# facebookresearch/DLRM-FlexFlow

Measured on AMD Instinct MI355X. Metric: dlrm_training_samples_per_sec, higher is better.
Workload: dtype f32; 1 GPU; criteo-terabyte-shape: 26 tables (rows 39884406-39043-17289-7420-20263-3-7120-1543-63-38532951-2953546-403346-10-2208-11938-155-4-976-14-39979771-25641295-39664984-585935-12972-108-36), emb_dim 128, bag 1, bot 13-512-256-128, top 3456-1024-1024-512-256-1, cat interaction, SGD lr 0.01, MSE loss; global_batch=32768, per_gpu_batch=32768, parallelism=single GPU, hipGraph-replayed step, step_graph=True

## Files before the change

dlrm_flexflow_amd/capi.py:

```python
from __future__ import annotations

import ctypes as C
import os
import re

_HERE = os.path.dirname(os.path.abspath(__file__))
REPO_ROOT = os.path.dirname(_HERE)
HIP_LIB_PATH = os.path.join(_HERE, "csrc", "libffhip.so")
HEADER_PATH = os.path.join(REPO_ROOT, "include", "ff_hip.h")

FFH_OK = 0
FFH_ERR_BAD_ARG, FFH_ERR_HIP, FFH_ERR_UNSUPPORTED, FFH_ERR_WORKSPACE, FFH_ERR_NOMEM = -1, -2, -3, -4, -5
AC_MODE_NONE, AC_MODE_RELU, AC_MODE_SIGMOID, AC_MODE_TANH, AC_MODE_GELU = 10, 11, 12, 13, 14
AGGR_MODE_NONE, AGGR_MODE_SUM, AGGR_MODE_AVG = 20, 21, 22
MAX_TABLES = 64
EMB_CHUNK, EMB_CHUNK1 = 32, 1024
OPT_ZERO_GRAD = 1
CONCAT_BWD_OVERWRITE = 1
LINEAR_DX_OVERWRITE, LINEAR_ONLY_DW, LINEAR_ONLY_DX, LINEAR_DY_PREMASKED, LINEAR_DX_MASK_BY_X = 1, 2, 4, 8, 16
METRIC_ACCURACY, METRIC_MSE, METRIC_RMSE, METRIC_MAE = 1, 2, 4, 8

P = C.c_void_p
I = C.c_int
L = C.c_int64
# ... 618 lines not shown

DIGEST_HEADER_PATH = os.path.join(REPO_ROOT, "include", "ff_hip_digest.h")

_SIGS_DIGEST = {
    "ffh_digest_abi_version": (I, []),
    "ffh_state_digest": (I, [P, P, L, L, L, C.c_uint64, C.c_uint64, P, P]),
}


def digest_header_symbols(header_path: str = DIGEST_HEADER_PATH) -> list[str]:
    text = open(header_path).read()
    m = re.search(r"#define FFH_DIGEST_API_LIST\(X\)(.*?)\n\n", text, re.S)
    if not m:
        raise RuntimeError("FFH_DIGEST_API_LIST not found in " + header_path)
    return re.findall(r"X\((ffh_[a-z0-9_]+)\)", m.group(1))


def digest_header_abi_version(header_path: str = DIGEST_HEADER_PATH) -> int:
    m = re.search(r"#define\s+FFH_DIGEST_ABI_VERSION\s+(\d+)", open(header_path).read())
    if not m:
        raise RuntimeError("FFH_DIGEST_ABI_VERSION not found in " + header_path)
    return int(m.group(1))


class DigestApi:

    def __init__(self, lib: FFHLib):
        self.base = lib
        for name, (res, args) in _SIGS_DIGEST.items():
            fn = getattr(lib.lib, name, None)
            if fn is None:
                raise FFHError(f"{lib.path}: no digest extension ({name} missing; include/ff_hip_digest.h)")
            fn.restype = res
            fn.argtypes = args
        got = lib.lib.ffh_digest_abi_version()
        if got != digest_header_abi_version():
            raise FFHError(f"{lib.path}: digest ABI version {got}, include/ff_hip_digest.h says {digest_header_abi_version()} (rebuild)")
        self.lib = lib.lib
        self.ctx = lib.ctx

    def state_digest_rc(self, base, rows, row_bytes, ld_bytes, seed, index_base, acc, stream=None) -> int:
        m64 = 2 ** 64 - 1
        return self.lib.ffh_state_digest(self.ctx, ptr(base), int(rows), int(row_bytes), int(ld_bytes), int(seed) & m64, int(index_base) & m64, ptr(acc),
                                         ptr(stream))

    def state_digest(self, base, rows, row_bytes, ld_bytes, seed, index_base, acc, stream=None):
        self.base.check(self.state_digest_rc(base, rows, row_bytes, ld_bytes, seed, index_base, acc, stream), "ffh_state_digest")


def digest_api(lib: FFHLib) -> DigestApi:
    return DigestApi(lib)


class CrossApi:

    def __init__(self, lib: FFHLib):
        self.base = lib
        for name, (res, args) in _SIGS_CROSS.items():
            fn = getattr(lib.lib, name, None)
            if fn is None:
                raise FFHError(f"{lib.path}: no cross extension ({name} missing; include/ff_hip_cross.h)")
            fn.restype = res
            fn.argtypes = args
        got = lib.lib.ffh_cross_abi_version()
        if got != cross_header_abi_version():
            raise FFHError(f"{lib.path}: cross ABI version {got}, include/ff_hip_cross.h says {cross_header_abi_version()} (rebuild)")
        self.lib = lib.lib
        self.ctx = lib.ctx

    def rc(self, name: str, *args) -> int:
        sig = _SIGS_CROSS[name][1][1:]
        if len(args) != len(sig):
            raise TypeError(f"{name}: expected {len(sig)} args, got {len(args)}")
        conv = [ptr(a) if t is P else a for a, t in zip(args, sig)]
        return getattr(self.lib, name)(self.ctx, *conv)

    def call(self, name: str, *args):
        self.base.check(self.rc(name, *args), name)


def cross_api(lib: FFHLib) -> CrossApi:
    return CrossApi(lib)


class AdagradApi:

    def __init__(self, lib: FFHLib):
        self.base = lib
        for name, (res, args) in _SIGS_ADAGRAD.items():
            fn = getattr(lib.lib, name, None)
            if fn is None:
                raise FFHError(f"{lib.path}: no Adagrad extension ({name} missing; include/ff_hip_adagrad.h)")
            fn.restype = res
            fn.argtypes = args
        got = lib.lib.ffh_adagrad_abi_version()
        if got != adagrad_header_abi_version():
            raise FFHError(f"{lib.path}: Adagrad ABI version {got}, include/ff_hip_adagrad.h says {adagrad_header_abi_version()} (rebuild)")
        self.lib = lib.lib
        self.ctx = lib.ctx

    def rc(self, name: str, *args) -> int:
        sig = _SIGS_ADAGRAD[name][1][1:]
        if len(args) != len(sig):
            raise TypeError(f"{name}: expected {len(sig)} args, got {len(args)}")
        conv = [ptr(a) if t is P else a for a, t in zip(args, sig)]
        return getattr(self.lib, name)(self.ctx, *conv)

    def call(self, name: str, *args):
        self.base.check(self.rc(name, *args), name)


def adagrad_api(lib: FFHLib) -> AdagradApi:
    return AdagradApi(lib)


class RowwiseApi:

    def __init__(self, lib: FFHLib):
        self.base = lib
        for name, (res, args) in _SIGS_ROWWISE.items():
            fn = getattr(lib.lib, name, None)
            if fn is None:
                raise FFHError(f"{lib.path}: no row-wise Adagrad extension ({name} missing; include/ff_hip_rowwise.h)")
            fn.restype = res
            fn.argtypes = args
        got = lib.lib.ffh_rowwise_abi_version()
        if got != rowwise_header_abi_version():
            raise FFHError(f"{lib.path}: row-wise Adagrad ABI version {got}, include/ff_hip_rowwise.h says {rowwise_header_abi_version()} (rebuild)")
        self.lib = lib.lib
        self.ctx = lib.ctx


def rowwise_api(lib: FFHLib) -> RowwiseApi:
    return RowwiseApi(lib)


FOLD_HEADER_PATH = os.path.join(REPO_ROOT, "include", "ff_hip_fold.h")


class FoldGroup(C.Structure):
    _fields_ = [("e", P), ("lde", L), ("col0", L), ("p", P), ("rows", L)]


class FoldSeg(C.Structure):
    _fields_ = [("k0", C.c_int32), ("len", C.c_int32)]


_SIGS_FOLD = {
    "ffh_fold_abi_version": (I, []),
    "ffh_fold_product": (I, [P, C.POINTER(FoldGroup), I, P, L, I, I, P]),
    "ffh_fold_gather_add": (I, [P, C.POINTER(EmbTable), I, I, I, L, I, P, L, P]),
    "ffh_fold_linear_fwd": (I, [P, P, L, P, L, P, P, I, I, L, I, C.POINTER(FoldSeg), I, P, L, P]),
    "ffh_fold_linear_fwd_plan": (I, [P, P, L, P, L, P, P, I, I, L, C.POINTER(FoldSeg), I, P, L]),
}


def fold_header_symbols(header_path: str = FOLD_HEADER_PATH) -> list[str]:
    m = re.search(r"#define FFH_FOLD_API_LIST\(X\)(.*?)\n\n", open(header_path).read(), re.S)
    if not m:
        raise RuntimeError("FFH_FOLD_API_LIST not found in " + header_path)
    return re.findall(r"X\((\w+)\)", m.group(1))


def fold_header_abi_version(header_path: str = FOLD_HEADER_PATH) -> int:
    m = re.search(r"#define\s+FFH_FOLD_ABI_VERSION\s+(\d+)", open(header_path).read())
    if not m:
        raise RuntimeError("FFH_FOLD_ABI_VERSION not found in " + header_path)
    return int(m.group(1))


class FoldApi:

    def __init__(self, lib: "FFHLib"):
        self.base = lib
        for name, (res, args) in _SIGS_FOLD.items():
            fn = getattr(lib.lib, name, None)
            if fn is None:
                raise FFHError(f"{lib.path}: no fold extension ({name} missing; include/ff_hip_fold.h)")
            fn.restype = res
            fn.argtypes = args
        got = lib.lib.ffh_fold_abi_version()
        if got != fold_header_abi_version():
            raise FFHError(f"{lib.path}: fold ABI version {got}, include/ff_hip_fold.h says {fold_header_abi_version()} (rebuild)")
        self.lib = lib.lib
        self.ctx = lib.ctx

    @staticmethod
    def groups(entries) -> "C.Array":
        entries = list(entries)
        arr = (FoldGroup * len(entries))()
        for k, (e, lde, col0, p, rows) in enumerate(entries):
            arr[k] = FoldGroup(ptr(e), int(lde), int(col0), ptr(p), int(rows))
        return arr

    @staticmethod
    def segs(entries) -> "C.Array":
        entries = list(entries)
        arr = (FoldSeg * max(1, len(entries)))()
        for k, (k0, n) in enumerate(entries):
            arr[k] = FoldSeg(int(k0), int(n))
        return arr

    def rc(self, name: str, *args) -> int:
        sig = _SIGS_FOLD[name][1][1:]
        if len(args) != len(sig):
            raise TypeError(f"{name}: expected {len(sig)} args, got {len(args)}")
        conv = [ptr(a) if t is P else a for a, t in zip(args, sig)]
        return getattr(self.lib, name)(self.ctx, *conv)

    def call(self, name: str, *args):
        self.base.check(self.rc(name, *args), name)


def fold_api(lib: "FFHLib") -> FoldApi:
    return FoldApi(lib)


_hip_singleton: FFHLib | None = None


def load_hip(device: int = 0) -> FFHLib:
    global _hip_singleton
    if _hip_singleton is None:
        import torch
        _hip_singleton = FFHLib(HIP_LIB_PATH, device)
        if not _hip_singleton.backend.startswith("hip"):
            raise FFHError(f"{HIP_LIB_PATH} is not the HIP backend ({_hip_singleton.backend})")
    return _hip_singleton
```

dlrm_flexflow_amd/csrc/fold.hip:

```cpp
#include "linear_gemm.h"

#include "../../include/ff_hip_fold.h"

using namespace ffh_gemm;

namespace {

typedef float f32x4 __attribute__((ext_vector_type(4)));

struct FoldGemmGroup { const float* a; int64_t lda; int64_t wcol0; float* c; int64_t ldc; int rows; int tile0; };
struct FoldGemmArgs {
  FoldGemmGroup grp[FFH_FOLD_MAX_GROUPS];
  ffh_fold_seg  seg[FFH_FOLD_MAX_SEGS];
  const float*  w; int64_t ldw;
  const float*  bias;
  const float*  addend; int64_t ldadd;
  int ngroups, nseg, N, act, ntiles;
};
static_assert(sizeof(FoldGemmArgs) <= 4096, "kernel arguments");

template <bool EPI>
__global__ __launch_bounds__(256) void fold_gemm_kernel(const FoldGemmArgs g) {
  ffh_kernel_prio();
  const int lane = threadIdx.x & 63;
  const int wave = __builtin_amdgcn_readfirstlane((int)(threadIdx.x >> 6));
  const int c = lane & 15, q = lane >> 4;
  const int wt = (int)blockIdx.x * 4 + wave;
  if (wt >= g.ntiles) return;
  int gi = 0;
  while (gi + 1 < g.ngroups && g.grp[gi + 1].tile0 <= wt) gi++;
  const FoldGemmGroup G = g.grp[gi];
  const int ct = g.N / 64, local = wt - G.tile0;
  const int r0 = (local / ct) * 32, n0 = (local % ct) * 64;
  const float* ap[2];
  const float* wp[4];
#pragma unroll
  for (int mt = 0; mt < 2; mt++) {
    int r = r0 + 16 * mt + c;
    if (r > G.rows - 1) r = G.rows - 1;
    ap[mt] = G.a + (int64_t)r * G.lda + 4 * q;
  }
#pragma unroll
  for (int nt = 0; nt < 4; nt++) wp[nt] = g.w + (int64_t)(n0 + 16 * nt + c) * g.ldw + G.wcol0 + 4 * q;
  f32x4 acc[4][2];
#pragma unroll
  for (int nt = 0; nt < 4; nt++)
#pragma unroll
    for (int mt = 0; mt < 2; mt++) acc[nt][mt] = f32x4{0.f, 0.f, 0.f, 0.f};
  for (int si = 0; si < g.nseg; si++) {
    const int k0 = g.seg[si].k0, k1 = k0 + g.seg[si].len;
    for (int k = k0; k < k1; k += 16) {
      f32x4 a[2], b[4];
#pragma unroll
      for (int mt = 0; mt < 2; mt++) a[mt] = *reinterpret_cast<const f32x4*>(ap[mt] + k);
#pragma unroll
      for (int nt = 0; nt < 4; nt++) b[nt] = *reinterpret_cast<const f32x4*>(wp[nt] + k);
#pragma unroll
      for (int e = 0; e < 4; e++)
#pragma unroll
        for (int nt = 0; nt < 4; nt++)
#pragma unroll
          for (int mt = 0; mt < 2; mt++) acc[nt][mt] = __builtin_amdgcn_mfma_f32_16x16x4f32(b[nt][e], a[mt][e], acc[nt][mt], 0, 0, 0);
    }
  }
#pragma unroll
  for (int mt = 0; mt < 2; mt++) {
    const int r = r0 + 16 * mt + c;
    if (r >= G.rows) continue;
#pragma unroll
    for (int nt = 0; nt < 4; nt++) {
      const int n = n0 + 16 * nt + 4 * q;
      f32x4 v = acc[nt][mt];
      if constexpr (EPI) {
        if (g.addend) v += *reinterpret_cast<const f32x4*>(g.addend + (int64_t)r * g.ldadd + n);
        if (g.bias) v += f32x4{g.bias[n], g.bias[n + 1], g.bias[n + 2], g.bias[n + 3]};
        if (g.act != FFH_AC_MODE_NONE) { v.x = act_apply(v.x, g.act); v.y = act_apply(v.y, g.act); v.z = act_apply(v.z, g.act); v.w = act_apply(v.w, g.act); }
      }
      *reinterpret_cast<f32x4*>(G.c + (int64_t)r * G.ldc + n) = v;
    }
  }
}

struct FoldGatherTable { const int64_t* idx; const float* p; };
struct FoldGatherArgs {
  FoldGatherTable t[FFH_MAX_TABLES];
  float* S; int64_t ldS;
  int64_t batch;
  int ntables, L, out;
};

__global__ __launch_bounds__(256) void fold_gather_add_kernel(const FoldGatherArgs g) {
  ffh_kernel_prio();
  const int nvec = g.out / 4;
  const int64_t total = g.batch * nvec;
  const int n = g.ntables * g.L;
  for (int64_t i = (int64_t)blockIdx.x * 256 + threadIdx.x; i < total; i += (int64_t)gridDim.x * 256) {
    const int64_t b = i / nvec;
    const int cv = (int)(i - b * nvec) * 4;
    f32x4 acc = f32x4{0.f, 0.f, 0.f, 0.f};
    for (int j0 = 0; j0 < n; j0 += 4) {
      f32x4 v[4];
#pragma unroll
      for (int u = 0; u < 4; u++) {
        const int j = j0 + u;
        if (j < n) {
          const int t = j / g.L, l = j - t * g.L;
          const int64_t id = g.t[t].idx[b * g.L + l];
          v[u] = *reinterpret_cast<const f32x4*>(g.t[t].p + id * g.out + cv);
        }
      }
#pragma unroll
      for (int u = 0; u < 4; u++)
        if (j0 + u < n) acc = (j0 + u == 0) ? v[u] : acc + v[u];
    }
    *reinterpret_cast<f32x4*>(g.S + b * g.ldS + cv) = acc;
  }
}

inline bool al16(const void* p) { return ((uintptr_t)p & 15) == 0; }

int fold_fwd_check(ffh_ctx* c, const float* x, int64_t ldx, const float* y, int64_t ldy, const float* w, int in, int out, int64_t batch,
                   const ffh_fold_seg* keep, int nkeep, const float* addend, int64_t ldadd) {
  FFH_REQUIRE(c, in > 0 && out > 0 && batch >= 0 && ldx >= in && ldy >= out, "fold_linear_fwd: bad dims");
  FFH_REQUIRE(c, batch == 0 || (x && y && w), "fold_linear_fwd: null pointer");
  FFH_REQUIRE(c, batch < (1LL << 31), "fold_linear_fwd: batch too large");
  FFH_REQUIRE(c, nkeep >= 0 && (nkeep == 0 || keep), "fold_linear_fwd: bad segment list");
  FFH_REQUIRE(c, !addend || ldadd >= out, "fold_linear_fwd: bad addend");
  int prev = 0;
  for (int i = 0; i < nkeep; i++) {
    FFH_REQUIRE(c, keep[i].k0 >= prev && keep[i].len > 0 && (int64_t)keep[i].k0 + keep[i].len <= in, "fold_linear_fwd: segments must ascend inside [0, in_dim)");
    prev = keep[i].k0 + keep[i].len;
  }
  return FFH_OK;
}
bool fold_fwd_served(const ffh_ctx* c, const float* x, int64_t ldx, const float* y, int64_t ldy, const float* w, int in, int out,
                     const ffh_fold_seg* keep, int nkeep, const float* addend, int64_t ldadd) {
  if (c->math_mode != FFH_MATH_DEFAULT) return false;
  if (in % FFH_FOLD_KTILE || out % FFH_FOLD_NTILE || nkeep > FFH_FOLD_MAX_SEGS) return false;
  if (!al16(x) || !al16(y) || !al16(w) || ldx % 4 || ldy % 4 || (addend && (!al16(addend) || ldadd % 4))) return false;
  for (int i = 0; i < nkeep; i++)
    if (keep[i].k0 % FFH_FOLD_KTILE || keep[i].len % FFH_FOLD_KTILE) return false;
  return true;
}
bool fold_keep_mask(int in, const ffh_fold_seg* keep, int nkeep, unsigned long long mask[2], int* nk_kept) {
  mask[0] = mask[1] = 0;
  *nk_kept = 0;
  if (in % 64 || in > 128 * 64) return false;
  const ffh_fold_seg all{0, in};
  if (nkeep == 0) { keep = &all; nkeep = 1; }
  for (int i = 0; i < nkeep; i++) {
    if (keep[i].k0 % 64 || keep[i].len % 64) return false;
    for (int kt = keep[i].k0 / 64; kt < (keep[i].k0 + keep[i].len) / 64; kt++) { mask[kt >> 6] |= 1ull << (kt & 63); (*nk_kept)++; }
  }
  return *nk_kept > 0;
}
GemmArgs fold_fwd_gemm(const float* x, int64_t ldx, float* y, int64_t ldy, const float* w, const float* bias, int in, int out, int64_t batch, int act) {
  GemmArgs g{};
  g.A = x; g.sAm = ldx; g.sAk = 1;
  g.B = w; g.sBn = in; g.sBk = 1;
  g.C = y; g.ldc = ldy; g.bias = bias;
  g.M = (int)batch; g.N = out; g.K = in;
  g.epi = EPI_STORE; g.act = act;
  return g;
}

}

extern "C" {

int ffh_fold_abi_version(void) { return FFH_FOLD_ABI_VERSION; }

int ffh_fold_product(ffh_ctx* c, const ffh_fold_group* groups, int ngroups, const float* w, int64_t ldw, int d, int out, ffh_stream s) {
  FFH_REQUIRE(c, groups && w && ngroups >= 1 && d > 0 && out > 0 && ldw >= d, "fold_product: bad arguments");
  if (ngroups > FFH_FOLD_MAX_GROUPS || d % FFH_FOLD_KTILE || out % FFH_FOLD_NTILE || !al16(w) || ldw % 4)
    return ffh_fail(c, FFH_ERR_UNSUPPORTED, "fold_product: d a multiple of 16, out_dim a multiple of 64, at most 64 tables, aligned weight");
  FoldGemmArgs a{};
  int64_t tiles = 0;
  for (int i = 0; i < ngroups; i++) {
    const ffh_fold_group& gr = groups[i];
    FFH_REQUIRE(c, gr.e && gr.p && gr.rows >= 1 && gr.rows < (1LL << 31) && gr.lde >= d && gr.col0 >= 0 && gr.col0 + d <= ldw, "fold_product: bad group");
    if (!al16(gr.e) || !al16(gr.p) || gr.lde % 4 || gr.col0 % FFH_FOLD_KTILE) return ffh_fail(c, FFH_ERR_UNSUPPORTED, "fold_product: group not aligned");
    a.grp[i] = FoldGemmGroup{gr.e, gr.lde, gr.col0, gr.p, (int64_t)out, (int)gr.rows, (int)tiles};
    tiles += ((gr.rows + 31) / 32) * (out / 64);
    FFH_REQUIRE(c, tiles < (1LL << 30), "fold_product: too many rows");
  }
  a.seg[0] = ffh_fold_seg{0, d};
  a.w = w; a.ldw = ldw; a.ngroups = ngroups; a.nseg = 1; a.N = out; a.act = FFH_AC_MODE_NONE; a.ntiles = (int)tiles;
  hipLaunchKernelGGL(fold_gemm_kernel<false>, dim3((unsigned)((tiles + 3) / 4)), dim3(256), 0, as_stream(s), a);
  FFH_LAUNCH_CHECK(c, "fold_gemm_kernel (products)");
  return FFH_OK;
}

int ffh_fold_gather_add(ffh_ctx* c, const ffh_emb_table* tables, int ntables, int in_dim, int out, int64_t batch, int aggr, float* S, int64_t ldS,
                        ffh_stream s) {
  FFH_REQUIRE(c, tables && ntables >= 1 && in_dim >= 1 && out > 0 && batch >= 0 && S && ldS >= out, "fold_gather_add: bad arguments");
  if (aggr != FFH_AGGR_MODE_SUM) return ffh_fail(c, FFH_ERR_UNSUPPORTED, "fold_gather_add: sum aggregation only");
  if (ntables > FFH_MAX_TABLES || out % 4 || ldS % 4 || !al16(S)) return ffh_fail(c, FFH_ERR_UNSUPPORTED, "fold_gather_add: out_dim and ldS multiples of 4, aligned S, at most 64 tables");
  FoldGatherArgs a{};
  for (int t = 0; t < ntables; t++) {
    FFH_REQUIRE(c, tables[t].idx && tables[t].weight && tables[t].num_entries >= 1, "fold_gather_add: bad table");
    if (!al16(tables[t].weight)) return ffh_fail(c, FFH_ERR_UNSUPPORTED, "fold_gather_add: product not aligned");
    a.t[t] = FoldGatherTable{tables[t].idx, tables[t].weight};
  }
  if (batch == 0) return FFH_OK;
  a.S = S; a.ldS = ldS; a.batch = batch; a.ntables = ntables; a.L = in_dim; a.out = out;
  hipLaunchKernelGGL(fold_gather_add_kernel, dim3(ffh_grid(batch * (out / 4), 256, 4096)), dim3(256), 0, as_stream(s), a);
  FFH_LAUNCH_CHECK(c, "fold_gather_add_kernel");
  return FFH_OK;
}

int ffh_fold_linear_fwd_plan(ffh_ctx* c, const float* x, int64_t ldx, const float* y, int64_t ldy, const float* w, const float* bias, int in, int out,
                             int64_t batch, const ffh_fold_seg* keep, int nkeep, const float* addend, int64_t ldadd) {
  const int rc = fold_fwd_check(c, x, ldx, y, ldy, w, in, out, batch, keep, nkeep, addend, ldadd);
  if (rc != FFH_OK) return rc;
  if (!fold_fwd_served(c, x, ldx, y, ldy, w, in, out, keep, nkeep, addend, ldadd)) return ffh_fail(c, FFH_ERR_UNSUPPORTED, "fold_linear_fwd: shape / alignment / math mode not served");
  const GemmArgs g = fold_fwd_gemm(x, ldx, const_cast<float*>(y), ldy, w, bias, in, out, batch, FFH_AC_MODE_NONE);
  unsigned long long mask[2]; int nk = 0;
  if (batch > 0 && fold_keep_mask(in, keep, nkeep, mask, &nk) && launch_gemm_sk_fold(c, g, mask, nk, addend, ldadd, true, nullptr, "") == 1) return 2;
  return (batch > 0 && gemm_sk_serves(c, g, SK_FORM_FWD)) ? 0 : 1;
}

int ffh_fold_linear_fwd(ffh_ctx* c, const float* x, int64_t ldx, float* y, int64_t ldy, const float* w, const float* bias, int in, int out, int64_t batch,
                        int act, const ffh_fold_seg* keep, int nkeep, const float* addend, int64_t ldadd, ffh_stream s) {
  if (nkeep == 0 && !addend) return ffh_linear_fwd(c, x, ldx, y, ldy, w, bias, in, out, batch, act, s);
  const int rc = fold_fwd_check(c, x, ldx, y, ldy, w, in, out, batch, keep, nkeep, addend, ldadd);
  if (rc != FFH_OK) return rc;
  if (act != FFH_AC_MODE_NONE && act != FFH_AC_MODE_RELU && act != FFH_AC_MODE_SIGMOID && act != FFH_AC_MODE_GELU)
    return ffh_fail(c, FFH_ERR_UNSUPPORTED, "fold_linear_fwd: activation not supported (NONE, RELU, SIGMOID, GELU)");
  if (!fold_fwd_served(c, x, ldx, y, ldy, w, in, out, keep, nkeep, addend, ldadd)) return ffh_fail(c, FFH_ERR_UNSUPPORTED, "fold_linear_fwd: shape / alignment / math mode not served");
  ffh_route_clear(c);
  if (batch == 0) return FFH_OK;
  const GemmArgs g = fold_fwd_gemm(x, ldx, y, ldy, w, bias, in, out, batch, act);
  unsigned long long mask[2]; int nk = 0;
  if (fold_keep_mask(in, keep, nkeep, mask, &nk) && (!bias || al16(bias))) {
    const int r = launch_gemm_sk_fold(c, g, mask, nk, addend, ldadd, false, s, "fold_linear_fwd gemm");
    if (r != 0) return r < 0 ? r : FFH_OK;
  }
  FoldGemmArgs a{};
  a.grp[0] = FoldGemmGroup{x, ldx, 0, y, ldy, (int)batch, 0};
  if (nkeep == 0) { a.seg[0] = ffh_fold_seg{0, in}; a.nseg = 1; }
  else { for (int i = 0; i < nkeep; i++) a.seg[i] = keep[i]; a.nseg = nkeep; }
  const int64_t tiles = ((batch + 31) / 32) * (out / 64);
  FFH_REQUIRE(c, tiles < (1LL << 30), "fold_linear_fwd: too many tiles");
  a.w = w; a.ldw = in; a.bias = bias; a.addend = addend; a.ldadd = ldadd; a.ngroups = 1; a.N = out; a.act = act; a.ntiles = (int)tiles;
  hipLaunchKernelGGL(fold_gemm_kernel<true>, dim3((unsigned)((tiles + 3) / 4)), dim3(256), 0, as_stream(s), a);
  FFH_LAUNCH_CHECK(c, "fold_gemm_kernel (forward)");
  ffh_route_add(c, "fold_linear_fwd gemm|mfma_32x64x16");
  return FFH_OK;
}

}
```

dlrm_flexflow_amd/csrc/linear_gemm.h:

```cpp
#pragma once
#include "ffh_common.h"

#include <hip/hip_runtime.h>

namespace ffh_gemm {

typedef float f32x16 __attribute__((ext_vector_type(16)));

enum { EPI_STORE = 0, EPI_ADD = 1, EPI_ATOMIC = 2 };

struct GemmArgs {
  const float* A;
  const float* B;
  float*       C;
  const float* bias;
  int64_t sAm, sAk, sBn, sBk, ldc;
  int64_t bsA, bsB, bsC;
  int M, N, K;
  int k_per_split;
  int splitk;
  int epi;
  int act;
  const float* act_y;
  int64_t      ld_act_y;
  float*       db;
  int          fuse;
  const float* mask;
  int64_t      ldmask;
  const ffh_col_dest* colmap;
  float* colsum;
  const unsigned short* A16;
  const unsigned short* B16;
  unsigned short*       C16;
  int                   a_not_twinned;
  int                   db_done;
};

constexpr int kSplitGran = 32;

__device__ __forceinline__ float act_apply(float v, int act) {
  if (act == FFH_AC_MODE_RELU) return v > 0.0f ? v : 0.0f;
  if (act == FFH_AC_MODE_SIGMOID) return 1.0f / (1.0f + expf(-v));
  if (act == FFH_AC_MODE_GELU) {
    constexpr float B = 0.7978845608028654f, C = 0.035677408136300125f;
    return v * (0.5f + 0.5f * tanhf(v * (C * v * v + B)));
  }
  return v;
}

__device__ __forceinline__ float4 load4_guard(const float* p, bool row_ok, int c0, int climit, bool vec_ok) {
  float4 v = make_float4(0.f, 0.f, 0.f, 0.f);
  if (!row_ok) return v;
  if (vec_ok && c0 + 3 < climit) return ld4u(p);
  if (c0 + 0 < climit) v.x = p[0];
  if (c0 + 1 < climit) v.y = p[1];
  if (c0 + 2 < climit) v.z = p[2];
  if (c0 + 3 < climit) v.w = p[3];
  return v;
}

template <typename K>
bool glds_set_lds(K kern, int bytes) {
  if (hipFuncSetAttribute((const void*)kern, hipFuncAttributeMaxDynamicSharedMemorySize, bytes) != hipSuccess) { (void)hipGetLastError(); return false; }
  return true;
}

inline bool use_bf16(const ffh_ctx* c, int in, int out, int64_t batch) {
  if (in < FFH_BF16_MIN_DIM || out < FFH_BF16_MIN_DIM) return false;
  if (c->math_mode == FFH_MATH_TENSOR_OP_BF16) return true;
  return c->math_mode == FFH_MATH_FP32_SPLIT_BF16X3_ALL || (c->math_mode == FFH_MATH_FP32_SPLIT_BF16X3 && 2.0 * (double)batch * (double)in * (double)out >= FFH_BF16X3_MIN_FLOP);
}

enum { BF16_FORM_FWD = 0,
       BF16_FORM_DW = 1,
       BF16_FORM_DX = 2,
       BF16_FORM_DX_MASK = 3 };
int launch_gemm_bf16_form(ffh_ctx* c, GemmArgs& g, int form, ffh_stream s, const char* name);
int launch_gemm_bf16_dma(ffh_ctx* c, const GemmArgs& g, int form, ffh_stream s, const char* name);
int launch_gemm_x3_dma(ffh_ctx* c, const GemmArgs& g, int form, ffh_stream s, const char* name);
float* dw_tile_slots(const ffh_ctx* c, ffh_stream s, int64_t tiles, int splitk, int64_t ldc);
void launch_dw_tile_reduce(const float* slots, float* C, int64_t ldc, int M, int N, int64_t tiles, int splitk, ffh_stream s);

enum { SK_FORM_FWD = 0, SK_FORM_DX = 1, SK_FORM_DW = 2 };
bool gemm_sk_serves(const ffh_ctx* c, const GemmArgs& g, int form);
int launch_gemm_sk(ffh_ctx* c, const GemmArgs& g, int form, ffh_stream s, const char* name);
int launch_gemm_sk_fold(ffh_ctx* c, const GemmArgs& g, const unsigned long long keep[2], int nk_kept, const float* addend, int64_t ldadd, bool dry,
                        ffh_stream s, const char* name);

}
```

dlrm_flexflow_amd/csrc/linear_sk.hip:

```cpp
#include "linear_gemm.h"

#include <stdlib.h>
#include <atomic>
#include <type_traits>
#include <utility>

using namespace ffh_gemm;

namespace {

typedef float f32x4 __attribute__((ext_vector_type(4)));
typedef unsigned u32x4 __attribute__((ext_vector_type(4)));

constexpr int SK_BM = 128, SK_BN = 128, SK_BK = 64;
constexpr int SK_LDS_KC = 128 * 256 + 32 * 32;
constexpr int SK_LDS_KR = 64 * 512;
constexpr int sk_lds_kc_a(int TMW) { return 32 * TMW * 256 + 32 * 32; }

enum { SK_EPI_FWD = 0, SK_EPI_DX_STORE = 1, SK_EPI_DX_ADD = 2, SK_EPI_DW_ATOMIC = 3, SK_EPI_DX_CMAP = 4 };

struct SkArgs {
  const float* A; const float* B; float* C;
  const float* bias;
  float*       db;
  const float* mask;
  const ffh_col_dest* colmap;
  float*       colsum;
  int64_t lda, ldb, ldc, ldmask;
  int M, N, K;
  int act;
  unsigned a_bytes, b_bytes, bias_bytes, mask_bytes;
  float*    sk_slots;
  unsigned* sk_cnt;
};

struct SkArgsFold : SkArgs {
  unsigned long long keep[2];
  unsigned           nk_kept;
  const float*       addend;
  int64_t            ldadd;
};

template <int... I, class F>
__device__ __forceinline__ void sk_static_for_impl(std::integer_sequence<int, I...>, F&& f) { (f(std::integral_constant<int, I>{}), ...); }
template <int N_, class F>
__device__ __forceinline__ void sk_static_for(F&& f) { sk_static_for_impl(std::make_integer_sequence<int, N_>{}, static_cast<F&&>(f)); }

#define SK_PIN() __builtin_amdgcn_sched_barrier(0)

constexpr int SK_EP_LD = 68;
constexpr int SK_EP_ROWS = 16;
constexpr int SK_EP_WAVE = SK_EP_ROWS * SK_EP_LD * 4;

template <bool AKR, bool BKR, int EPI, bool DB = false, bool SPLIT = false, int TMW = 4, bool FOLD = false>
__global__ __launch_bounds__(256, 1) void gemm_sk_kernel(const std::conditional_t<FOLD, SkArgsFold, SkArgs> g) {
  static_assert(!FOLD || (EPI == SK_EPI_FWD && !SPLIT && !DB && TMW == 4), "kept k-tiles + addend: the whole-tile forward form");
  static_assert(!DB || (EPI == SK_EPI_DW_ATOMIC && AKR), "the bias gradient rides on the weight-gradient form");
  static_assert(!SPLIT || EPI != SK_EPI_DW_ATOMIC, "the weight gradient meets by atomics");
  static_assert(TMW == 4 || (TMW == 2 && !AKR && EPI != SK_EPI_DW_ATOMIC), "64-row tiles: forward and data gradient (A k-contiguous)");
  extern __shared__ __attribute__((aligned(16))) char sk_lds[];
  constexpr bool ATOMIC = EPI == SK_EPI_DW_ATOMIC;
  constexpr bool STREAMK = ATOMIC || SPLIT;
  constexpr int BM = 32 * TMW;
  constexpr int NM = 64 * TMW;
  constexpr int NPA = 2 * TMW, NP = NPA + 8;
  constexpr int LDS_A = AKR ? SK_LDS_KR : sk_lds_kc_a(TMW);
  char* const ldsA = sk_lds;
  char* const ldsB = sk_lds + LDS_A;
  const int tid = threadIdx.x, lane = tid & 63;
  const int wave = __builtin_amdgcn_readfirstlane(tid >> 6);
  const int wy = wave >> 1, wx = wave & 1;
  const int c16 = lane & 15, q = lane >> 4;

  const int fra = AKR ? (q * 2048 + wy * 256 + c16 * 16) : ((16 * TMW * wy + TMW * c16) * 256 + (16 * wy + c16) * 32 + q * 16);
  const int frb = BKR ? (q * 2048 + wx * 256 + c16 * 16) : ((64 * wx + 4 * c16) * 256 + (16 * wx + c16) * 32 + q * 16);
  const int srowA = AKR ? (tid >> 5) : (tid >> 4), schA = AKR ? (tid & 31) : (tid & 15);
  const int srowB = BKR ? (tid >> 5) : (tid >> 4), schB = BKR ? (tid & 31) : (tid & 15);
  const unsigned voffA = (unsigned)((srowA * g.lda + schA * 4) * 4);
  const unsigned voffB = (unsigned)((srowB * g.ldb + schB * 4) * 4);
  const int swA = AKR ? (srowA * 512 + schA * 16) : (srowA * 256 + (srowA / TMW) * 32 + schA * 16);
  const int swB = BKR ? (srowB * 512 + schB * 16) : (srowB * 256 + (srowB >> 2) * 32 + schB * 16);
  constexpr int SW_STEP_A = AKR ? 4096 : (4096 + (16 / TMW) * 32), SW_STEP_B = BKR ? 4096 : 4224;
  const unsigned ioffA = (unsigned)((AKR ? 8 : 16) * g.lda * 4), ioffB = (unsigned)((BKR ? 8 : 16) * g.ldb * 4);
  const unsigned kadvA = AKR ? (unsigned)(SK_BK * g.lda * 4) : (unsigned)(SK_BK * 4), kadvB = BKR ? (unsigned)(SK_BK * g.ldb * 4) : (unsigned)(SK_BK * 4);

  const __amdgpu_buffer_rsrc_t rsA = __builtin_amdgcn_make_buffer_rsrc(const_cast<float*>(g.A), 0, g.a_bytes, 0x00020000);
  const __amdgpu_buffer_rsrc_t rsB = __builtin_amdgcn_make_buffer_rsrc(const_cast<float*>(g.B), 0, g.b_bytes, 0x00020000);

  const unsigned nbx = (unsigned)(g.N / SK_BN), nby = (unsigned)(g.M / BM), ntiles = nbx * nby;
  unsigned nk = (unsigned)(g.K / SK_BK);
  if constexpr (FOLD) nk = g.nk_kept;
  auto first_kept = [&]() -> unsigned {
    if constexpr (FOLD) return g.keep[0] ? (unsigned)__builtin_ctzll(g.keep[0]) : 64u + (unsigned)__builtin_ctzll(g.keep[1]);
    else return 0u;
  };
  auto next_kept = [&](unsigned p) -> unsigned {
    if constexpr (FOLD) {
      p++;
      if (p < 64u) {
        const unsigned long long m = g.keep[0] >> p;
        if (m) return p + (unsigned)__builtin_ctzll(m);
        p = 64u;
      }
      const unsigned long long m = p < 128u ? g.keep[1] >> (p - 64u) : 0ull;
      return m ? p + (unsigned)__builtin_ctzll(m) : p;
    } else return p + 1u;
  };
  const unsigned G = gridDim.x, w = blockIdx.x;
  const unsigned total_it = ntiles * nk;
  const unsigned wperm = (w & 7u) * (G >> 3) + (w >> 3);
  unsigned it_b, it_e;
  const unsigned ipw = (total_it + G - 1) / G;
  const unsigned rng = SPLIT ? wperm : w;
  if (STREAMK) {
    it_b = rng * ipw; it_e = it_b + ipw < total_it ? it_b + ipw : total_it;
    if (it_b > total_it) it_b = total_it;
  } else {
    const unsigned mine = ntiles / G + (wperm < ntiles % G ? 1u : 0u);
    it_b = 0; it_e = mine * nk;
  }
  const unsigned n_it = it_e - it_b;
  if (n_it == 0) return;

  struct Cursor { unsigned seq, kt, m0, n0, offA, offB, kp; };
  auto place = [&](Cursor& c) {
    unsigned lin;
    if (STREAMK) lin = it_b / nk + c.seq;
    else lin = c.seq * G + wperm;
    if (lin >= ntiles) lin = ntiles - 1;
    const unsigned by = lin / nbx, bx = lin - by * nbx;
    c.m0 = by * BM; c.n0 = bx * SK_BN;
    c.kp = FOLD ? first_kept() : c.kt;
    c.offA = (AKR ? c.m0 * 4u : (unsigned)(c.m0 * g.lda * 4)) + c.kp * kadvA;
    c.offB = (BKR ? c.n0 * 4u : (unsigned)(c.n0 * g.ldb * 4)) + c.kp * kadvB;
  };
  auto advance = [&](Cursor& c) {
    c.kt++;
    if (c.kt == nk) { c.kt = 0; c.seq++; place(c); }
    else if constexpr (FOLD) { const unsigned np = next_kept(c.kp), d = np - c.kp; c.offA += d * kadvA; c.offB += d * kadvB; c.kp = np; }
    else { c.offA += kadvA; c.offB += kadvB; }
  };
  Cursor ld{0, STREAMK ? it_b % nk : 0u, 0, 0, 0, 0, 0}, cp = ld;
  place(ld); place(cp);

  u32x4 P[NP];
  auto gload_one = [&](int i, const Cursor& c) {
    if (i < NPA) P[i] = __builtin_amdgcn_raw_buffer_load_b128(rsA, voffA, c.offA + (unsigned)i * ioffA, 0);
    else P[i] = __builtin_amdgcn_raw_buffer_load_b128(rsB, voffB, c.offB + (unsigned)(i - NPA) * ioffB, 0);
  };
  auto lwrite_one = [&](int i) {
    if (i < NPA) *reinterpret_cast<u32x4*>(ldsA + swA + i * SW_STEP_A) = P[i];
    else *reinterpret_cast<u32x4*>(ldsB + swB + (i - NPA) * SW_STEP_B) = P[i];
  };
  f32x4 fa[4][4], fb[4][4];
  auto fread = [&](int j, int r, bool isB) {
    if (!isB) fa[j][r] = *reinterpret_cast<const f32x4*>(ldsA + fra + (AKR ? (j * 8192 + r * 512) : (r * 256 + j * 64)));
    else fb[j][r] = *reinterpret_cast<const f32x4*>(ldsB + frb + (BKR ? (j * 8192 + r * 512) : (r * 256 + j * 64)));
  };
  f32x4 acc[TMW][4];
  f32x4 bsum = f32x4{0.f, 0.f, 0.f, 0.f};

#pragma unroll
  for (int i = 0; i < NP; i++) gload_one(i, ld);
  advance(ld);
#pragma unroll
  for (int i = 0; i < NP; i++) lwrite_one(i);
#pragma unroll
  for (int i = 0; i < NP; i++) gload_one(i, ld);
  advance(ld);
  __builtin_amdgcn_s_waitcnt(0xC07F);
  __builtin_amdgcn_s_barrier();
  SK_PIN();
#pragma unroll
  for (int r = 0; r < 4; r++) { if (r < TMW) fread(0, r, false); fread(0, r, true); }
  SK_PIN();

  for (unsigned it = 0; it < n_it;) {
    const unsigned seg = (nk - cp.kt) < (n_it - it) ? (nk - cp.kt) : (n_it - it);
#pragma unroll
    for (int i = 0; i < TMW; i++)
#pragma unroll
      for (int j = 0; j < 4; j++) acc[i][j] = f32x4{0.f, 0.f, 0.f, 0.f};
    asm volatile("s_nop 7" ::: "memory");
    for (unsigned kk = 0; kk < seg; kk++) {
      sk_static_for<NM>([&](auto sc) {
        constexpr int s = decltype(sc)::value;
        constexpr int tn = s & 3, tm = (s >> 2) % TMW, e = (s / (4 * TMW)) & 3, j = s / (16 * TMW);
        const float av = AKR ? fa[j][e][tm] : fa[j][tm][e];
        const float bv = BKR ? fb[j][e][tn] : fb[j][tn][e];
        asm volatile("v_mfma_f32_16x16x4_f32 %0, %1, %2, %0" : "+a"(acc[tm][tn]) : "v"(av), "v"(bv));
        if constexpr (DB && (s & 15) == 1) {
          asm volatile("v_add_f32 %0, %4, %0\n\tv_add_f32 %1, %5, %1\n\tv_add_f32 %2, %6, %2\n\tv_add_f32 %3, %7, %3"
                       : "+v"(bsum.x), "+v"(bsum.y), "+v"(bsum.z), "+v"(bsum.w)
                       : "v"(fa[j][e].x), "v"(fa[j][e].y), "v"(fa[j][e].z), "v"(fa[j][e].w));
        }
        constexpr int RPG = TMW + 4;
        constexpr int NRD = 3 * RPG;
        constexpr int BAR1 = TMW == 4 ? 53 : 30;
        constexpr int PSTEP = TMW == 4 ? 11 : 7;
        constexpr int BAR2 = NM - 13;
        if constexpr (s < NRD) {
          constexpr int jj = 1 + s / RPG, gi = s % RPG;
          if constexpr (gi < 2 * TMW) fread(jj, gi >> 1, (gi & 1) != 0);
          else fread(jj, gi - TMW, true);
        }
        if constexpr (s == BAR1) {
          __builtin_amdgcn_s_waitcnt(0xC07F);
          __builtin_amdgcn_s_barrier();
        }
        if constexpr (s > BAR1 && s <= BAR1 + 1 + (NP - 1) * PSTEP && (s - BAR1 - 1) % PSTEP == 0) {
          constexpr int i = (s - BAR1 - 1) / PSTEP;
          lwrite_one(i);
          gload_one(i, ld);
        }
        if constexpr (s == BAR2) {
          __builtin_amdgcn_s_waitcnt(0xC07F);
          __builtin_amdgcn_s_barrier();
        }
        if constexpr (s > BAR2 && s <= BAR2 + RPG) {
          constexpr int o = s - BAR2 - 1;
          if constexpr (o == 0) fread(0, 0, false);
          else if constexpr (o <= 4) fread(0, o - 1, true);
          else fread(0, o - 4, false);
        }
        SK_PIN();
      });
      advance(ld);
    }
    it += seg;
    asm volatile("s_nop 15\n\ts_nop 15" ::: "memory");
    bool store_tile = true;
    if constexpr (SPLIT) {
      const bool head = cp.kt == 0;
      if (!(head && seg == nk)) {
        typedef unsigned long long u64;
        const unsigned it0 = (it_b / nk + cp.seq) * nk;
        const unsigned r0 = it0 / ipw, r1 = (it0 + nk - 1) / ipw;
        const unsigned nparts = r1 - r0 + 1;
        u64* slot = reinterpret_cast<u64*>(g.sk_slots + (size_t)(head ? 2u * rng + 1u : 2u * rng) * (SK_BM * SK_BN));
#pragma unroll
        for (int tm = 0; tm < TMW; tm++)
#pragma unroll
          for (int tn = 0; tn < 4; tn++) {
            const f32x4 v = acc[tm][tn];
            u64* q2 = slot + ((tm * 4 + tn) * 256 + tid) * 2;
            __hip_atomic_store(q2, ((u64)__float_as_uint(v.y) << 32) | __float_as_uint(v.x), __ATOMIC_RELAXED, __HIP_MEMORY_SCOPE_AGENT);
            __hip_atomic_store(q2 + 1, ((u64)__float_as_uint(v.w) << 32) | __float_as_uint(v.z), __ATOMIC_RELAXED, __HIP_MEMORY_SCOPE_AGENT);
          }
        asm volatile("s_waitcnt vmcnt(0)" ::: "memory");
        __syncthreads();
        unsigned* const bc = reinterpret_cast<unsigned*>(sk_lds + LDS_A + (BKR ? SK_LDS_KR : SK_LDS_KC));
        if (tid == 0) *bc = __hip_atomic_fetch_add(g.sk_cnt + r0, 1u, __ATOMIC_RELAXED, __HIP_MEMORY_SCOPE_AGENT);
        __syncthreads();
        const bool last = *bc == nparts - 1;
        __syncthreads();
        if (!last) {
          store_tile = false;
        } else {
          if (tid == 0) __hip_atomic_store(g.sk_cnt + r0, 0u, __ATOMIC_RELAXED, __HIP_MEMORY_SCOPE_AGENT);
          for (unsigned p = head ? 1u : 0u; p < nparts; p++) {
            const u64* sl = reinterpret_cast<const u64*>(g.sk_slots + (size_t)(p == 0 ? 2u * r0 + 1u : 2u * (r0 + p)) * (SK_BM * SK_BN));
#pragma unroll
            for (int tm = 0; tm < TMW; tm++)
#pragma unroll
              for (int tn = 0; tn < 4; tn++) {
                const u64* q2 = sl + ((tm * 4 + tn) * 256 + tid) * 2;
                const u64 lo = __hip_atomic_load(q2, __ATOMIC_RELAXED, __HIP_MEMORY_SCOPE_AGENT);
                const u64 hi = __hip_atomic_load(q2 + 1, __ATOMIC_RELAXED, __HIP_MEMORY_SCOPE_AGENT);
                const f32x4 v = f32x4{__uint_as_float((unsigned)lo), __uint_as_float((unsigned)(lo >> 32)), __uint_as_float((unsigned)hi), __uint_as_float((unsigned)(hi >> 32))};
                if (p == 0) acc[tm][tn] = v; else acc[tm][tn] += v;
              }
          }
        }
      }
    }
    if (store_tile) {
      const int nn = (int)cp.n0 + 64 * wx + 4 * c16;
      const bool relu_fast = g.act == FFH_AC_MODE_RELU, none_fast = g.act == FFH_AC_MODE_NONE;
      (void)relu_fast; (void)none_fast;
      f32x4 bv = f32x4{0.f, 0.f, 0.f, 0.f};
      if constexpr (EPI == SK_EPI_FWD) {
        const __amdgpu_buffer_rsrc_t rsBias = __builtin_amdgcn_make_buffer_rsrc(const_cast<float*>(g.bias), 0, g.bias_bytes, 0x00020000);
        const u32x4 t = __builtin_amdgcn_raw_buffer_load_b128(rsBias, (unsigned)nn * 4u, 0, 0);
        bv = __builtin_bit_cast(f32x4, t);
// ... 121 lines not shown

namespace ffh_gemm {

namespace {
struct SkPlan { int64_t lda, ldb, a_bytes, b_bytes; int G; bool split; int tmw; };
bool sk_plan(const ffh_ctx* c, const GemmArgs& g, int form, SkPlan& p) {
  static const int off = FFH_LAB_INT("FFH_GEMM_NO_SK", 0);
  if (off) return false;
  {
    static const int64_t min_w = FFH_LAB_I64("FFH_SK_MIN_WEIGHTS", 0);
    static const int64_t min_wb = FFH_LAB_I64("FFH_SK_MIN_WEIGHTS_BWD", 65536);
    const int64_t nw = form == SK_FORM_DW ? (int64_t)g.M * g.N : (int64_t)g.N * g.K;
    if (nw < min_w || (form != SK_FORM_FWD && nw < min_wb)) return false;
  }
  if (g.M % SK_BM || g.N % SK_BN || g.K % SK_BK || g.M <= 0 || g.N <= 0 || g.K <= 0) return false;
  const bool akr = form == SK_FORM_DW, bkr = form != SK_FORM_FWD;
  p.lda = akr ? g.sAk : g.sAm; p.ldb = bkr ? g.sBk : g.sBn;
  if ((akr ? g.sAm : g.sAk) != 1 || (bkr ? g.sBn : g.sBk) != 1) return false;
  if (!sk_aligned(g.A, p.lda) || !sk_aligned(g.B, p.ldb) || (!g.colmap && !sk_aligned(g.C, g.ldc))) return false;
  if (g.mask && !sk_aligned(g.mask, g.ldmask)) return false;
  if (g.bias && ((uintptr_t)g.bias & 15)) return false;
  if (g.act_y || g.fuse || g.splitk > 1) return false;
  if (g.colmap && (form != SK_FORM_DX || g.epi != EPI_STORE || g.mask)) return false;
  p.a_bytes = ((akr ? (int64_t)(g.K - 1) : (int64_t)(g.M - 1)) * p.lda + (akr ? g.M : g.K)) * 4;
  p.b_bytes = ((bkr ? (int64_t)(g.K - 1) : (int64_t)(g.N - 1)) * p.ldb + (bkr ? g.N : g.K)) * 4;
  if (p.a_bytes >= (1LL << 32) || p.b_bytes >= (1LL << 32)) return false;
  p.G = c->num_cus & ~7;
  if (form == SK_FORM_DW && c->dw_cu_reserve > 0 && p.G - c->dw_cu_reserve >= 64) p.G -= c->dw_cu_reserve;
  if (p.G < 8) return false;
  const int64_t ntiles = (int64_t)(g.M / SK_BM) * (g.N / SK_BN), nk = g.K / SK_BK;
  if (ntiles * nk >= (1LL << 31)) return false;
  p.tmw = 4;
  if (form == SK_FORM_DW) {
    if (c->deterministic || g.epi != EPI_ATOMIC) return false;
    static const int dw_min_it = FFH_LAB_INT("FFH_SK_DW_MIN_IT", 8);
    if (ntiles * nk < (int64_t)dw_min_it * p.G) return false;
  } else {
    if (g.epi != EPI_STORE && g.epi != EPI_ADD) return false;
    static const int no_split = FFH_LAB_INT("FFH_SK_NO_SPLIT", 0);
    const int64_t rounds = (ntiles + p.G - 1) / p.G;
    const int64_t idle_it = (rounds * p.G - ntiles) * nk / p.G;
    static const int no_t64 = FFH_LAB_INT("FFH_SK_NO_T64", 0);
    p.tmw = 4;
    if (!no_t64 && ntiles < p.G && g.M % 64 == 0 && (g.epi == EPI_STORE || g.epi == EPI_ADD) && nk >= 8) {
      const int64_t nt64 = (int64_t)(g.M / 64) * (g.N / SK_BN);
      if (nt64 <= p.G && nt64 * 100 >= (int64_t)p.G * 80) { p.tmw = 2; p.split = false; return true; }
    }
    p.split = !no_split && idle_it >= 2 && ntiles * nk >= 8LL * p.G && g.epi == EPI_STORE;
    if (!p.split) {
      if (ntiles < p.G) return false;
      if (ntiles * 100 < rounds * p.G * 80) return false;
    }
  }
  return true;
}

bool sk_slots_for(ffh_ctx* c, hipStream_t s, float** slots, unsigned** cnt) {
  for (int i = 0; i < c->nscratch; i++)
    if (c->scratch[i].stream == (void*)s && c->scratch[i].sk_slots) { *slots = c->scratch[i].sk_slots; *cnt = c->scratch[i].sk_cnt; return true; }
  return false;
}
}

bool gemm_sk_serves(const ffh_ctx* c, const GemmArgs& g, int form) { SkPlan p; return sk_plan(c, g, form, p); }

int launch_gemm_sk(ffh_ctx* c, const GemmArgs& g, int form, ffh_stream s, const char* name) {
  SkPlan p{};
  if (!sk_plan(c, g, form, p)) return 0;
  float* slots = nullptr; unsigned* flags = nullptr;
  if (p.split && !sk_slots_for(c, as_stream(s), &slots, &flags)) {
    p.split = false;
    { char tok[96]; snprintf(tok, sizeof tok, "%s|no_scratch_on_this_stream", name); ffh_route_add(c, tok); }
    const int64_t ntiles = (int64_t)(g.M / SK_BM) * (g.N / SK_BN), rounds = (ntiles + p.G - 1) / p.G;
    if (ntiles < p.G || ntiles * 100 < rounds * p.G * 80) return 0;
  }
  const int64_t lda = p.lda, ldb = p.ldb, a_bytes = p.a_bytes, b_bytes = p.b_bytes;
  const int G = p.G;
  SkArgs a{};
  a.A = g.A; a.B = g.B; a.C = g.C; a.bias = g.bias; a.mask = g.mask; a.db = g.db; a.colmap = g.colmap; a.colsum = (form == SK_FORM_DX && g.epi == EPI_STORE && !g.colmap) ? g.colsum : nullptr;
  a.lda = lda; a.ldb = ldb; a.ldc = g.ldc; a.ldmask = g.ldmask;
  a.M = g.M; a.N = g.N; a.K = g.K; a.act = g.act;
  a.a_bytes = (unsigned)a_bytes; a.b_bytes = (unsigned)b_bytes;
  a.bias_bytes = g.bias ? (unsigned)g.N * 4u : 0u;
  a.mask_bytes = g.mask ? 1u : 0u;
  if (p.split) { a.sk_slots = slots; a.sk_cnt = flags; }
#define FFH_SK_LAUNCH(AKR, BKR, EPI, LDSB, ...)                                                                  \
  {                                                                                                              \
    auto kern = gemm_sk_kernel<AKR, BKR, EPI, ##__VA_ARGS__>;                                                    \
    static std::atomic<signed char> ok[64];                \
    const int dev = c->device & 63;                                                                              \
    if (ok[dev].load(std::memory_order_acquire) == 0) ok[dev].store(sk_set_lds(kern, LDSB) ? 1 : -1, std::memory_order_release); \
    if (ok[dev].load(std::memory_order_acquire) < 0) return 0;                                                   \
    hipLaunchKernelGGL(kern, dim3((unsigned)G), dim3(256), LDSB, as_stream(s), a);                               \
  }
  constexpr int BCW = 64;
  constexpr int KC64 = sk_lds_kc_a(2);
  if (form == SK_FORM_FWD && p.tmw == 2) FFH_SK_LAUNCH(false, false, SK_EPI_FWD, KC64 + SK_LDS_KC, false, false, 2)
  else if (form == SK_FORM_DX && p.tmw == 2 && g.colmap) FFH_SK_LAUNCH(false, true, SK_EPI_DX_CMAP, KC64 + SK_LDS_KR, false, false, 2)
  else if (form == SK_FORM_DX && p.tmw == 2 && g.epi == EPI_STORE) FFH_SK_LAUNCH(false, true, SK_EPI_DX_STORE, KC64 + SK_LDS_KR, false, false, 2)
  else if (form == SK_FORM_DX && p.tmw == 2) FFH_SK_LAUNCH(false, true, SK_EPI_DX_ADD, KC64 + SK_LDS_KR, false, false, 2)
  else if (form == SK_FORM_FWD && p.split) FFH_SK_LAUNCH(false, false, SK_EPI_FWD, 2 * SK_LDS_KC + BCW, false, true)
  else if (form == SK_FORM_DX && p.split && g.colmap) FFH_SK_LAUNCH(false, true, SK_EPI_DX_CMAP, SK_LDS_KC + SK_LDS_KR + BCW, false, true)
  else if (form == SK_FORM_DX && p.split) FFH_SK_LAUNCH(false, true, SK_EPI_DX_STORE, SK_LDS_KC + SK_LDS_KR + BCW, false, true)
  else if (form == SK_FORM_FWD) FFH_SK_LAUNCH(false, false, SK_EPI_FWD, 2 * SK_LDS_KC)
  else if (form == SK_FORM_DW && g.db) FFH_SK_LAUNCH(true, true, SK_EPI_DW_ATOMIC, 2 * SK_LDS_KR + 4 * SK_EP_WAVE, true)
  else if (form == SK_FORM_DW) FFH_SK_LAUNCH(true, true, SK_EPI_DW_ATOMIC, 2 * SK_LDS_KR + 4 * SK_EP_WAVE)
  else if (g.colmap) FFH_SK_LAUNCH(false, true, SK_EPI_DX_CMAP, SK_LDS_KC + SK_LDS_KR)
  else if (g.epi == EPI_STORE) FFH_SK_LAUNCH(false, true, SK_EPI_DX_STORE, SK_LDS_KC + SK_LDS_KR)
  else FFH_SK_LAUNCH(false, true, SK_EPI_DX_ADD, SK_LDS_KC + SK_LDS_KR)
#undef FFH_SK_LAUNCH
  {
    const hipError_t e = hipGetLastError();
    if (e == hipErrorInvalidValue || e == hipErrorInvalidConfiguration || e == hipErrorLaunchOutOfResources || e == hipErrorSharedObjectInitFailed) return 0;
    if (e != hipSuccess) return ffh_fail_hip(c, e, name);
  }
  { char tok[96]; snprintf(tok, sizeof tok, "%s|sk_%dx128x64%s%s%s|wgs=%d", name, 32 * p.tmw, g.colmap ? "|colmap" : "", p.split ? "|streamk" : "", a.colsum ? "|colsum" : "", G); ffh_route_add(c, tok); }
  return 1;
}

int launch_gemm_sk_fold(ffh_ctx* c, const GemmArgs& g, const unsigned long long keep[2], int nk_kept, const float* addend, int64_t ldadd, bool dry,
                        ffh_stream s, const char* name) {
  if (g.K % SK_BK || g.K > 128 * SK_BK || nk_kept < 1 || nk_kept > g.K / SK_BK) return 0;
  if (addend && !sk_aligned(addend, ldadd)) return 0;
  GemmArgs gk = g;
  gk.K = nk_kept * SK_BK;
  SkPlan p{};
  if (!sk_plan(c, gk, SK_FORM_FWD, p) || p.split || p.tmw != 4) return 0;
  const int64_t a_bytes = ((int64_t)(g.M - 1) * p.lda + g.K) * 4, b_bytes = ((int64_t)(g.N - 1) * p.ldb + g.K) * 4;
  if (a_bytes >= (1LL << 32) || b_bytes >= (1LL << 32)) return 0;
  if (dry) return 1;
  SkArgsFold a{};
  a.A = g.A; a.B = g.B; a.C = g.C; a.bias = g.bias;
  a.lda = p.lda; a.ldb = p.ldb; a.ldc = g.ldc;
  a.M = g.M; a.N = g.N; a.K = g.K; a.act = g.act;
  a.a_bytes = (unsigned)a_bytes; a.b_bytes = (unsigned)b_bytes;
  a.bias_bytes = g.bias ? (unsigned)g.N * 4u : 0u;
  a.keep[0] = keep[0]; a.keep[1] = keep[1]; a.nk_kept = (unsigned)nk_kept; a.addend = addend; a.ldadd = ldadd;
  {
    auto kern = gemm_sk_kernel<false, false, SK_EPI_FWD, false, false, 4, true>;
    constexpr int LDSB = 2 * SK_LDS_KC;
    static std::atomic<signed char> ok[64];
    const int dev = c->device & 63;
    if (ok[dev].load(std::memory_order_acquire) == 0) ok[dev].store(sk_set_lds(kern, LDSB) ? 1 : -1, std::memory_order_release);
    if (ok[dev].load(std::memory_order_acquire) < 0) return 0;
    hipLaunchKernelGGL(kern, dim3((unsigned)p.G), dim3(256), LDSB, as_stream(s), a);
    const hipError_t e = hipGetLastError();
    if (e == hipErrorInvalidValue || e == hipErrorInvalidConfiguration || e == hipErrorLaunchOutOfResources || e == hipErrorSharedObjectInitFailed) return 0;
    if (e != hipSuccess) return ffh_fail_hip(c, e, name);
  }
  { char tok[96]; snprintf(tok, sizeof tok, "%s|sk_128x128x64|kept=%d/%d%s|wgs=%d", name, nk_kept, g.K / SK_BK, addend ? "|addend" : "", p.G); ffh_route_add(c, tok); }
  return 1;
}

}
```

dlrm_flexflow_amd/host/ffmodel.h:

```cpp
#pragma once

#include <cstddef>
#include <cstdint>
#include <condition_variable>
#include <deque>
#include <functional>
#include <map>
#include <mutex>
#include <thread>
#include <string>
#include <vector>

#include "../../include/ff_hip.h"
#include "../../include/ff_hip_bf16.h"
#include "../../include/ff_hip_ctr.h"
#include "../../include/ff_hip_lr.h"
#include "../../include/ff_hip_cross.h"
#include "../../include/ff_hip_adagrad.h"
#include "../../include/ff_hip_rowwise.h"
#include "../../include/ff_hip_fold.h"
#include "ffcomm.h"

enum ActiMode { AC_MODE_NONE = 10, AC_MODE_RELU = 11, AC_MODE_SIGMOID = 12, AC_MODE_TANH = 13, AC_MODE_GELU = 14 };
enum AggrMode { AGGR_MODE_NONE = 20, AGGR_MODE_SUM = 21, AGGR_MODE_AVG = 22 };
enum DataType { DT_FLOAT = 40, DT_DOUBLE = 41, DT_INT32 = 42, DT_INT64 = 43, DT_BOOLEAN = 44, DT_NONE = 49,
                DT_BF16 = 140 };
enum LossType {
  LOSS_CATEGORICAL_CROSSENTROPY = 50,
  LOSS_SPARSE_CATEGORICAL_CROSSENTROPY = 51,
  LOSS_MEAN_SQUARED_ERROR_AVG_REDUCE = 52,
  LOSS_MEAN_SQUARED_ERROR_SUM_REDUCE = 53,
  LOSS_BINARY_CROSSENTROPY = 150,
};
enum CompMode { COMP_MODE_TRAINING = 70, COMP_MODE_INFERENCE = 71 };
enum ParameterSyncType { NONE = 80, PS = 81, NCCL = 82 };
enum MetricsType {
  METRICS_ACCURACY = 1001,
  METRICS_CATEGORICAL_CROSSENTROPY = 1002,
  METRICS_SPARSE_CATEGORICAL_CROSSENTROPY = 1004,
  METRICS_MEAN_SQUARED_ERROR = 1008,
  METRICS_ROOT_MEAN_SQUARED_ERROR = 1016,
  METRICS_MEAN_ABSOLUTE_ERROR = 1032,
  METRICS_BINARY_CROSSENTROPY = 2001,
  METRICS_AUC = 2002,
};
enum OperatorType { OP_INPUT, OP_LINEAR, OP_EMBEDDING, OP_CONCAT, OP_BATCHMATMUL, OP_TRANSPOSE, OP_RESHAPE, OP_FLAT, OP_TRIL, OP_DOT_INTERACTION, OP_CROSS_COMBINE };

#define MAX_TENSOR_DIM 4
#define MAX_NUM_INPUTS 256
#define MAX_OPNAME 64

class FFModel;
class Op;
struct KernelApi;

struct ParallelConfig {
  enum DeviceType { GPU = 0, CPU = 1 };
  ParallelConfig() : device_type(GPU), nDims(0) { for (int& d : dim) d = 1; }
  int num_parts() const { int n = 1; for (int i = 0; i < nDims; i++) n *= dim[i]; return n; }
  bool is_data_parallel() const;
  bool operator==(const ParallelConfig& rhs) const;
  DeviceType device_type;
  int nDims, dim[MAX_TENSOR_DIM];
  std::vector<int> device_ids;
};
typedef size_t MappingTagID;
bool load_strategies_from_file(const std::string& filename, std::map<MappingTagID, ParallelConfig>& strategies);
bool save_strategies_to_file(const std::string& filename, const std::map<std::string, ParallelConfig>& strategies);

class FFConfig {
 public:
  FFConfig();
  void parse_args(char** argv, int argc);
  int epochs, batchSize, printFreq;
  int numNodes, cpusPerNode, workersPerNode;
  float learningRate, weightDecay;
  size_t workSpaceSize;
  bool syntheticInput, profiling, perform_fusion;
  CompMode computationMode;
  std::string dataset_path;
  std::string import_strategy_file, export_strategy_file;
  std::map<MappingTagID, ParallelConfig> strategies;
  static MappingTagID get_hash_id(const std::string& pcname);
  bool find_parallel_config(int ndims, const std::string& pcname, ParallelConfig& config) const;
  std::string save_checkpoint_dir, load_checkpoint_dir;
  int checkpoint_every_epochs;
  std::string backend_lib;
  int device;
  uint64_t seed;
  bool enable_graph;
  bool overlap_embedding;
  bool dense_embedding_update;
  int64_t column_shard_rows;
  bool deterministic;
  bool fp32_split_bf16x3;
  bool allow_tensor_op_math_conversion;
  bool bf16_convert_twins;
  bool bf16_exact_small_backward;
  bool bf16_twins, force_async_launch;
  bool capture_exchange;
  bool pad_linear_k;
  bool sparse_embedding_optimizer;
  int early_sort;
  bool dx_colsum;
  bool dx_scatter;
  bool fuse_pair;
  int  bucket_allreduce;
  bool direct_allreduce;
  int64_t allreduce_bucket_floats;
  int64_t big_dw_min_weights;
  int  big_dw_chunks;
  int  trace_mode;
  bool fold_small_tables;
  int64_t fold_max_rows;
  bool mlp_chain;
  int64_t mlp_chain_max_batch;
  int64_t mlp_chain_fwd_max_batch;
  int64_t mlp_chain_fwd_min_batch;
  int64_t mlp_chain_max_weights;
  bool attach_events;
  bool timing_events;
  int driver_loss;
  int eval_batches;
  int synthetic_labels;
  bool eval_only;
  int data_randomize;
  bool fuse_loss;
  int64_t replicate_embedding_rows;
  int64_t row_shard_rows;
  bool async_launch;
  bool parallel_dw;
  bool force_exchange;
  DataType embedding_dtype;
  int embedding_rounding;
  int64_t lr_warmup_steps, lr_decay_start_step, lr_num_decay_steps;
  bool device_lr;
  bool host_lr_schedule;
  double adagrad_eps;
  double adagrad_initial_accumulator;
  bool adagrad_rowwise;
  ffcomm comm;
};

struct TensorPiece {
  float*  ptr;
  float*  grad;
  int64_t ld;
  int     cols;
};

struct TensorImpl {
  void*   ptr = nullptr;
  int64_t ld = 0;
  float*  grad = nullptr;
  int64_t grad_ld = 0;
  bool    alias = false;
  bool    grad_alias = false;
  bool    is_input = false;
  size_t  bytes = 0;
  int64_t rows_local = 0;
  int     guid = -1;
  std::vector<TensorPiece> pieces;
};

struct Tensor {
  Tensor(void);
  size_t get_volume() const;
  int64_t rows() const;
  int64_t cols() const { return adim[0]; }
  template <typename T> bool set_tensor(const FFModel* model, const std::vector<int>& dims, const T* data);
  template <typename T> bool get_tensor(const FFModel* model, T* data) const;
  template <typename T> bool get_grad(const FFModel* model, T* data) const;
  int numDim, adim[MAX_TENSOR_DIM];
  DataType data_type;
  ParameterSyncType sync_type;
  Op* owner_op;
  int owner_idx;
  TensorImpl* impl;
};

struct Parameter : Tensor {
  template <typename T> bool set_weights(const FFModel* model, const std::vector<int>& dims, const T* data);
  template <typename T> bool get_weights(const FFModel* model, T* data) const;
};

class Initializer {
 public:
  virtual ~Initializer() {}
  virtual void init(const FFModel* ff, const Parameter* p) = 0;
};
class ZeroInitializer : public Initializer {
 public:
  void init(const FFModel* ff, const Parameter* p) override;
};
class ConstantInitializer : public Initializer {
 public:
  explicit ConstantInitializer(float v) : value(v) {}
  void init(const FFModel* ff, const Parameter* p) override;
  float value;
};
class UniformInitializer : public Initializer {
 public:
  UniformInitializer(int _seed, float _min, float _max) : seed(_seed), min_val(_min), max_val(_max) {}
  void init(const FFModel* ff, const Parameter* p) override;
  int seed;
  float min_val, max_val;
};
class NormInitializer : public Initializer {
 public:
  NormInitializer(int _seed, float _mean, float _stddev) : seed(_seed), mean(_mean), stddev(_stddev) {}
  void init(const FFModel* ff, const Parameter* p) override;
  int seed;
  float mean, stddev;
};
class GlorotUniform : public Initializer {
 public:
  explicit GlorotUniform(int _seed) : seed(_seed) {}
  void init(const FFModel* ff, const Parameter* p) override;
  int seed;
};

class Optimizer {
 public:
  explicit Optimizer(const FFModel* _model) : model(_model) {}
  virtual ~Optimizer() {}
  virtual void init(void) = 0;
  virtual void next(void) = 0;
  virtual void update(const Parameter* p) = 0;
  const FFModel* model;
};
class SGDOptimizer : public Optimizer {
 public:
  SGDOptimizer(const FFModel* _model, double lr = 0.01f, double momentum = 0.0f, bool nesterov = false,
               double weight_decay = 0.0f);
  void init(void) override;
  void next(void) override;
  void update(const Parameter* p) override;
  void set_weight_decay(double wd) { weight_decay = wd; }
  double lr, momentum;
  bool nesterov;
  double weight_decay;
  std::map<const void*, float*> v_values;
};

class AdamOptimizer : public Optimizer {
 public:
  AdamOptimizer(const FFModel* _model, double _alpha = 0.001f, double _beta1 = 0.9f, double _beta2 = 0.999f,
                double _weight_decay = 0.0f, double _epsilon = 1e-8);
  void init(void) override;
  void next(void) override;
  void update(const Parameter* p) override;
  void set_weight_decay(double wd) { weight_decay = wd; }
  double alpha, beta1, beta2, weight_decay, epsilon;
  double alpha_t, beta1_t, beta2_t;
  float *mlp_m, *mlp_v;
  std::map<const void*, std::pair<float*, float*>> mv_values;
};

class AdagradOptimizer : public Optimizer {
 public:
  AdagradOptimizer(const FFModel* _model, double _lr = 0.01f, double _weight_decay = 0.0f, double _epsilon = 1e-10, double _initial_accumulator = 0.0);
  void init(void) override;
  void next(void) override;
  void update(const Parameter* p) override;
  void set_weight_decay(double wd) { weight_decay = wd; }
  double lr, weight_decay, epsilon, initial_accumulator;
  bool rowwise;
// ... 215 lines not shown
                          bool create_grad = true);

  void compile(LossType loss_type, const std::vector<MetricsType>& metrics, CompMode comp_mode = COMP_MODE_TRAINING);
  void compile(Optimizer* optimizer, LossType loss_type, const std::vector<MetricsType>& metrics,
               CompMode comp_mode = COMP_MODE_TRAINING);
  void init_layers();
  void reset_metrics();
  void forward(int seq_length = -1);
  void zero_gradients();
  void compute_metrics();
  void backward(int seq_length = -1);
  void update();
  void begin_trace(int trace_id);
  void end_trace(int trace_id);
  void sync();
  PerfMetrics get_perf_metrics();
  void eval_batch();
  void reset_eval_metrics();
  EvalMetrics get_eval_metrics(bool with_histograms = false);
  Initializer* own(Initializer* init) { owned_initializers.push_back(init); return init; }
  int next_seed();
  uint64_t seed_counter;
  void print_layers(int id);
  std::string get_operator_type_name(OperatorType type) const;

  int op_global_guid;
  FFConfig config;
  Optimizer* optimizer;
  LossType loss_type;
  int metrics_flags;
  Tensor label_tensor;
  std::vector<Op*> layers;
  std::vector<Parameter> parameters;
  int seq_length;

  const KernelApi* api;
  ffh_ctx* ctx;
  ffh_stream stream;
  ffh_stream side_stream;
  ffh_stream dw_stream;
  ffh_event ev_dw_done;
  int big_dw_layer;
  bool need_zero_gsend;
  bool need_zero_act_grads;
  mutable bool dw_forked;
  mutable bool dw1_used = false;
  mutable bool dw_stream_used_directly = false;
  struct GradBucket {
    size_t off, count;
    int lowest_layer;
    bool issued;
    ffh_event ready, ready_dw, done;
    int chunk_layer, chunk_index;
    bool inline_issued;
  };
  std::vector<GradBucket> grad_buckets;
  std::vector<std::pair<size_t, size_t>> grad_rest;
  ffh_stream ar_stream = nullptr;
  bool bucketed_now() const;
  int  allreduce_grads(float* buf, int64_t count, ffh_stream s, bool bucket) const;
  float* ar_scratch = nullptr;
  size_t ar_scratch_floats = 0;
  mutable int64_t n_direct_allreduces = 0;
  mutable std::map<int64_t, std::vector<int64_t>> direct_plans;
  bool buckets_held() const;
  void issue_grad_buckets(int next_layer);
  void issue_one_bucket(size_t k, bool wait_main);
  int  big_dw_chunks_now() const;
  mutable int64_t n_bucket_allreduces = 0;
  int64_t n_fused_loss_calls = 0;
  mutable int64_t n_chain_fwd_calls = 0, n_chain_bwd_calls = 0;
  bool mlp_chain_usable(int64_t rows, bool fwd) const;
  int run_chain_fwd(const Linear* lowest) const;
  int run_chain_bwd(Linear* top);
  mutable bool mlp_grads_clean;
  LaunchWorker *dw_worker, *side_worker;
  std::vector<ffh_event> layer_events;
  bool use_workers() const { return dw_worker != nullptr && capturing_trace < 0; }
  ffh_event ev_fork, ev_join, ev_grad_ready, ev_update_done;
  int rank, world_size;
  bool exchange;
  int64_t local_batch;
  bool compiled;

  void* dmalloc(size_t bytes) const;
  void check(int rc, const char* what) const;

  std::vector<Embedding*> embeddings;
  void embedding_group_forward(ffh_stream s, ffh_ctx* on_ctx = nullptr) const;
  void replicated_embedding_grads() const;
  void embedding_group_update(ffh_stream s, ffh_ctx* on_ctx = nullptr) const;
  void embedding_kernels_only(bool fwd, ffh_stream s, const std::vector<const int64_t*>* idx_override = nullptr) const;
  mutable bool probe_events_on = false;
  static constexpr int kProbeEvents = 30;
  mutable ffh_event probe_ev[kProbeEvents] = {};
  void probe_record(int which, ffh_stream s, ffh_ctx* cx) const;
  uint64_t* bf16_counter = nullptr;
  ffh_bf16_rounding bf16_rounding() const;
  uint64_t read_bf16_counter() const;
  void advance_bf16_counter(ffh_stream s, ffh_ctx* cx) const;
  size_t bf16_tables_per_launch() const;
  enum LrRoute { kLrOff = 0, kLrHost = 1, kLrDevice = 2 };
  int lr_route = kLrOff;
  std::string lr_route_why;
  double lr_base = 0.0;
  int64_t lr_host_steps = 0;
  ffh_lr_state* lr_block[2] = {nullptr, nullptr};
  void lr_choose_route();
  void lr_allocate();
  void lr_host_set(int64_t k);
  void advance_lr(int which, ffh_stream s, ffh_ctx* cx) const;
  double current_lr();
  int64_t lr_steps();
  std::string lr_schedule_line() const;
  struct CheckpointInfo { int64_t epochs_done = 0, steps = 0; uint64_t digest = 0; size_t bytes = 0; };
  CheckpointInfo save_checkpoint(const std::string& dir, int64_t epochs_done);
  CheckpointInfo load_checkpoint(const std::string& dir);
  uint64_t state_digest();
  int64_t n_update_calls = 0;
  uint64_t* digest_acc = nullptr;
  mutable int64_t n_graph_replays = 0;
  mutable int64_t n_early_sorts = 0;
  bool fused_embedding_update() const;
  bool sparse_rule(ffh_sparse_opt& rule) const;
  mutable bool opt_next_done = false;
  void embedding_dense_update() const;
  void issue_embedding_forward_on_side_stream() const;
  void join_embedding_forward() const;
  void issue_embedding_update_on_side_stream() const;
  void order_input_writes_behind_update() const;
  void profiled(const Op* op, bool fwd, const std::function<void()>& fn) const;
  mutable bool emb_forward_issued, emb_forward_joined, emb_update_pending;
  static constexpr int early_sort_big_batch_mode = 0;
  bool early_sort_possible(int where) const;
  mutable bool emb_sorted_early;
  int scatter_attach_layer;
  std::vector<Initializer*> owned_initializers;
  int grad_attach_layer;
  void* w_twin = nullptr; void* act_twin = nullptr; void* grad_twin = nullptr;
  mutable bool w_twin_dirty = false;
  void refresh_weight_twin() const;
  int64_t weight_mirror_stale_bytes();
  void note_weight_write(const void* p) const;
  mutable bool bwd_alltoall_issued = false;
  int n_twin_regions = 0;
  struct FoldRoute {
    Linear* layer = nullptr;
    std::vector<Embedding*> tables;
    std::vector<ffh_fold_group> groups;
    std::vector<ffh_emb_table> gather;
    std::vector<ffh_fold_seg> keep;
    float* P = nullptr;
    float* S = nullptr;
  } fold;
  ffh_event ev_fold_w = nullptr;
  ffh_event ev_fold_done = nullptr;
  mutable bool fold_w_recorded = false, fold_on_side = false;
  void plan_fold();
  void fold_products_and_sum(ffh_stream s, ffh_ctx* cx) const;
  void fold_linear_forward(const Linear* li) const;
  int z_reader_layer;
  ffh_event ev_z_free;
  mutable bool z_free_recorded;
  mutable bool grad_ready_attached;

  float *mlp_weights, *mlp_grads;  size_t mlp_count;
  char* act_slab;
  char* act_grad_slab;  size_t act_grad_bytes;
  void* workspace;  size_t workspace_bytes;
  void* repl_workspace;  size_t repl_workspace_bytes;
  ffh_perf_metrics* d_perf;
  float* d_bce_sum;
  ffh_ctr_eval* d_eval;
  bool want_eval;
  bool evaluating;
  struct EmbShard { Embedding* e; int owner; int col0; int cols; int64_t off; };
  std::vector<EmbShard> shards;
  std::vector<int64_t> rank_width;
  float *xsend, *xrecv, *gsend, *grecv;
  std::vector<int64_t> fwd_send_counts, fwd_recv_counts;
  std::vector<int> owned_tables;
  int tables_of_rank(int r) const;

  std::map<int, ffh_graph> graphs;
  int capturing_trace, replaying_trace;
  struct TraceTune { int calls = 0; int decided = 0; ffh_event ev[4] = {nullptr, nullptr, nullptr, nullptr}; float eager_ms = 0.f, graph_ms = 0.f; };
  std::map<int, TraceTune> trace_tune;
  bool trace_adaptive() const { return config.trace_mode == 0 && !exchange; }
  bool trace_replays(int trace_id) const;
  mutable bool inputs_dirty;
  mutable bool fork_recorded;

  std::vector<TensorImpl*> tensor_impls;
  std::vector<Tensor*> input_tensors;
 private:
  void allocate();
  void apply_strategies();
};
```

dlrm_flexflow_amd/host/ffmodel_c.cc:

```cpp
#include <cstring>
#include "ffmodel_c.h"
#include <string>

#include <chrono>

#include <cstdio>
#include <cstdlib>
#include <vector>

#include "backend.h"
#include "dlrm.h"
#include "ffmodel.h"

namespace {
FFConfig* C(flexflow_config_t h) { return (FFConfig*)h.impl; }
FFModel* M(flexflow_model_t h) { return (FFModel*)h.impl; }
Tensor* T(flexflow_tensor_t h) { return (Tensor*)h.impl; }
Initializer* I(flexflow_initializer_t h) { return (Initializer*)h.impl; }
DLRMApp* A(flexflow_dlrm_t h) { return (DLRMApp*)h.impl; }
flexflow_tensor_t wrap(const Tensor& t) { flexflow_tensor_t h; h.impl = new Tensor(t); return h; }
std::vector<int> dims_vec(const int* dims, int n) { return std::vector<int>(dims, dims + n); }
}

extern "C" {

flexflow_config_t flexflow_config_create(void) { flexflow_config_t h; h.impl = new FFConfig(); return h; }
void flexflow_config_destroy(flexflow_config_t h) { delete C(h); }
void flexflow_config_parse_args(flexflow_config_t h, char** argv, int argc) { C(h)->parse_args(argv, argc); }
void flexflow_config_set_comm(flexflow_config_t h, const ffcomm* comm) { if (comm) C(h)->comm = *comm; }
void flexflow_config_set_batch_size(flexflow_config_t h, int b) { C(h)->batchSize = b; }
int  flexflow_config_get_batch_size(flexflow_config_t h) { return C(h)->batchSize; }
void flexflow_config_set_backend(flexflow_config_t h, const char* p) { C(h)->backend_lib = p ? p : ""; }
void flexflow_config_set_seed(flexflow_config_t h, uint64_t s) { C(h)->seed = s; }
void flexflow_config_set_device(flexflow_config_t h, int d) { C(h)->device = d; }
void flexflow_config_set_enable_graph(flexflow_config_t h, bool v) { C(h)->enable_graph = v; }
void flexflow_config_set_overlap_embedding(flexflow_config_t h, bool v) { C(h)->overlap_embedding = v; }
void flexflow_config_set_dense_embedding_update(flexflow_config_t h, bool v) { C(h)->dense_embedding_update = v; }
void flexflow_config_set_embedding_dtype(flexflow_config_t h, int dt) {
  if (dt != DT_FLOAT && dt != DT_BF16) { fprintf(stderr, "FATAL: embedding data type %d: %d (fp32) or %d (bf16)\n", dt, (int)DT_FLOAT, (int)DT_BF16); abort(); }
  C(h)->embedding_dtype = (DataType)dt;
}
void flexflow_config_set_embedding_rounding(flexflow_config_t h, int mode) {
  if (mode != 0 && mode != 1) { fprintf(stderr, "FATAL: embedding rounding %d: 0 (stochastic) or 1 (nearest)\n", mode); abort(); }
  C(h)->embedding_rounding = mode;
}
void flexflow_config_set_lr_schedule(flexflow_config_t h, int64_t warmup_steps, int64_t decay_start_step, int64_t num_decay_steps, int device_lr) {
  C(h)->lr_warmup_steps = warmup_steps; C(h)->lr_decay_start_step = decay_start_step; C(h)->lr_num_decay_steps = num_decay_steps;
  C(h)->device_lr = device_lr == 1;
  C(h)->host_lr_schedule = device_lr == -1;
}
double flexflow_lr_schedule_value(int64_t k, double base, int64_t W, int64_t S, int64_t N) { return (double)(float)ffh_lr_schedule_value(k, base, W, S, N); }
uint64_t flexflow_shuffle_index(uint64_t seed, uint64_t epoch, uint64_t i, uint64_t n) { return ffh_perm_index(seed, epoch, i, n); }
void flexflow_shuffle_indices(uint64_t seed, uint64_t epoch, uint64_t first, uint64_t count, uint64_t n, uint64_t* out) {
  for (uint64_t j = 0; j < count; j++) out[j] = ffh_perm_index(seed, epoch, first + j, n);
}

flexflow_model_t flexflow_model_create(flexflow_config_t c) { flexflow_model_t h; h.impl = new FFModel(*C(c)); return h; }
void flexflow_model_destroy(flexflow_model_t h) { delete M(h); }

flexflow_tensor_t flexflow_tensor_create(flexflow_model_t m, int nd, const int* dims, int dt, bool cg) {
  switch (nd) {
    case 1: return wrap(M(m)->create_tensor<1>(dims, (DataType)dt, NULL, cg));
    case 2: return wrap(M(m)->create_tensor<2>(dims, (DataType)dt, NULL, cg));
    case 3: return wrap(M(m)->create_tensor<3>(dims, (DataType)dt, NULL, cg));
    case 4: return wrap(M(m)->create_tensor<4>(dims, (DataType)dt, NULL, cg));
    default: fprintf(stderr, "FATAL: tensors have 1..4 dimensions\n"); abort();
  }
}
flexflow_tensor_t flexflow_model_add_dense(flexflow_model_t m, flexflow_tensor_t in, int out_dim, int act, bool use_bias,
                                           flexflow_initializer_t ki, flexflow_initializer_t bi, const char* name) {
  return wrap(M(m)->dense(*T(in), out_dim, (ActiMode)act, use_bias, NULL, I(ki), I(bi), name));
}
flexflow_tensor_t flexflow_model_add_embedding(flexflow_model_t m, flexflow_tensor_t in, int num_entries, int out_dim, int aggr,
                                               flexflow_initializer_t ki, const char* name) {
  return wrap(M(m)->embedding(*T(in), num_entries, out_dim, (AggrMode)aggr, NULL, I(ki), name));
}
flexflow_tensor_t flexflow_model_add_concat(flexflow_model_t m, int n, const flexflow_tensor_t* ins, int axis, const char* name) {
  std::vector<Tensor> v;
  for (int i = 0; i < n; i++) v.push_back(*T(ins[i]));
  return wrap(M(m)->concat(n, v.data(), axis, name));
}
flexflow_tensor_t flexflow_model_add_flat(flexflow_model_t m, flexflow_tensor_t in, const char* name) { return wrap(M(m)->flat(*T(in), name)); }
flexflow_tensor_t flexflow_model_add_dot_interaction(flexflow_model_t m, flexflow_tensor_t in, int d, const char* name) { return wrap(M(m)->dot_interaction(*T(in), d, name)); }
flexflow_tensor_t flexflow_model_add_cross_combine(flexflow_model_t m, flexflow_tensor_t x0, flexflow_tensor_t v, flexflow_tensor_t xl, const char* name) {
  return wrap(M(m)->cross_combine(*T(x0), *T(v), *T(xl), name));
}
flexflow_tensor_t flexflow_model_add_cross_net(flexflow_model_t m, flexflow_tensor_t x0, int num_layers, int low_rank, const char* name) {
  return wrap(M(m)->cross_net(*T(x0), num_layers, low_rank, name));
}
flexflow_tensor_t flexflow_model_add_tril(flexflow_model_t m, flexflow_tensor_t in, const char* name) { return wrap(M(m)->tril(*T(in), name)); }
flexflow_tensor_t flexflow_model_add_transpose(flexflow_model_t m, flexflow_tensor_t in, int n, const int* perm, const char* name) {
  return wrap(M(m)->transpose(*T(in), dims_vec(perm, n), name));
}
flexflow_tensor_t flexflow_model_add_reshape(flexflow_model_t m, flexflow_tensor_t in, int n, const int* shape, const char* name) {
  return wrap(M(m)->reshape(*T(in), dims_vec(shape, n), name));
}
flexflow_tensor_t flexflow_model_add_batch_matmul(flexflow_model_t m, flexflow_tensor_t a, flexflow_tensor_t b, int asd, int bsd) {
  return wrap(M(m)->batch_matmul(*T(a), *T(b), asd, bsd));
}
flexflow_initializer_t flexflow_zero_initializer_create(void) { flexflow_initializer_t h; h.impl = new ZeroInitializer(); return h; }
flexflow_initializer_t flexflow_uniform_initializer_create(int seed, float lo, float hi) { flexflow_initializer_t h; h.impl = new UniformInitializer(seed, lo, hi); return h; }
flexflow_initializer_t flexflow_norm_initializer_create(int seed, float mean, float sd) { flexflow_initializer_t h; h.impl = new NormInitializer(seed, mean, sd); return h; }
flexflow_initializer_t flexflow_glorot_uniform_initializer_create(int seed) { flexflow_initializer_t h; h.impl = new GlorotUniform(seed); return h; }
flexflow_sgd_optimizer_t flexflow_sgd_optimizer_create(flexflow_model_t m, double lr, double mom, bool nest, double wd) {
  flexflow_sgd_optimizer_t h; h.impl = new SGDOptimizer(M(m), lr, mom, nest, wd); return h;
}
void flexflow_model_set_sgd_optimizer(flexflow_model_t m, flexflow_sgd_optimizer_t o) { M(m)->optimizer = (SGDOptimizer*)o.impl; }
flexflow_adam_optimizer_t flexflow_adam_optimizer_create(flexflow_model_t m, double alpha, double b1, double b2, double wd, double eps) {
  flexflow_adam_optimizer_t h; h.impl = new AdamOptimizer(M(m), alpha, b1, b2, wd, eps); return h;
}
void flexflow_adam_optimizer_set_lr(flexflow_adam_optimizer_t o, double lr) { ((AdamOptimizer*)o.impl)->alpha = lr; }
void flexflow_model_set_adam_optimizer(flexflow_model_t m, flexflow_adam_optimizer_t o) { M(m)->optimizer = (AdamOptimizer*)o.impl; }
int64_t flexflow_model_weight_mirror_stale_bytes(flexflow_model_t m) { return M(m)->weight_mirror_stale_bytes(); }
void flexflow_config_set_adagrad(flexflow_config_t h, double eps, double acc) { C(h)->adagrad_eps = eps; C(h)->adagrad_initial_accumulator = acc; }
flexflow_adagrad_optimizer_t flexflow_adagrad_optimizer_create(flexflow_model_t m, double lr, double wd, double eps, double acc) {
  flexflow_adagrad_optimizer_t h;
  h.impl = new AdagradOptimizer(M(m), lr, wd, eps != eps ? M(m)->config.adagrad_eps : eps, acc != acc ? M(m)->config.adagrad_initial_accumulator : acc);
  return h;
}
void flexflow_model_set_adagrad_optimizer(flexflow_model_t m, flexflow_adagrad_optimizer_t o) { M(m)->optimizer = (AdagradOptimizer*)o.impl; }
void flexflow_config_set_adagrad_rowwise(flexflow_config_t h, int on) { C(h)->adagrad_rowwise = on != 0; }
void flexflow_adagrad_optimizer_set_rowwise(flexflow_adagrad_optimizer_t o, int on) { ((AdagradOptimizer*)o.impl)->rowwise = on != 0; }
void flexflow_model_compile(flexflow_model_t m, int loss, const int* metrics, int nb, int comp_mode) {
  std::vector<MetricsType> v;
  for (int i = 0; i < nb; i++) v.push_back((MetricsType)metrics[i]);
  M(m)->compile((LossType)loss, v, (CompMode)comp_mode);
}
void flexflow_model_init_layers(flexflow_model_t m) { M(m)->init_layers(); }
void flexflow_model_reset_metrics(flexflow_model_t m) { M(m)->reset_metrics(); }
void flexflow_model_forward(flexflow_model_t m, int sl) { M(m)->forward(sl); }
void flexflow_model_zero_gradients(flexflow_model_t m) { M(m)->zero_gradients(); }
void flexflow_model_backward(flexflow_model_t m, int sl) { M(m)->backward(sl); }
void flexflow_model_update(flexflow_model_t m) { M(m)->update(); }
void flexflow_model_begin_trace(flexflow_model_t m, int id) { M(m)->begin_trace(id); }
void flexflow_model_end_trace(flexflow_model_t m, int id) { M(m)->end_trace(id); }
void flexflow_model_sync(flexflow_model_t m) { M(m)->sync(); }
const char* flexflow_model_get_backend_name(flexflow_model_t m) { return M(m)->api->ffh_backend_name(); }
const char* flexflow_model_get_backend_path(flexflow_model_t m) { return M(m)->api->path.c_str(); }
void flexflow_model_get_perf_metrics(flexflow_model_t m, flexflow_perf_metrics_t* out) {
  PerfMetrics p = M(m)->get_perf_metrics();
  out->train_all = p.train_all; out->train_correct = p.train_correct; out->cce_loss = p.cce_loss;
  out->sparse_cce_loss = p.sparse_cce_loss; out->mse_loss = p.mse_loss; out->rmse_loss = p.rmse_loss; out->mae_loss = p.mae_loss;
}
flexflow_tensor_t flexflow_model_get_label_tensor(flexflow_model_t m) { return wrap(M(m)->label_tensor); }
int flexflow_model_get_num_layers(flexflow_model_t m) { return (int)M(m)->layers.size(); }
const char* flexflow_model_get_layer_name(flexflow_model_t m, int l) { return M(m)->layers.at(l)->name; }
int flexflow_model_get_layer_num_weights(flexflow_model_t m, int l) { return M(m)->layers.at(l)->numWeights; }
flexflow_tensor_t flexflow_model_get_parameter(flexflow_model_t m, int l, int i) {
  Op* op = M(m)->layers.at(l);
  if (i < 0 || i >= op->numWeights) { fprintf(stderr, "FATAL: %s has %d weights\n", op->name, op->numWeights); abort(); }
  return wrap(op->weights[i]);
}
flexflow_tensor_t flexflow_model_get_layer_output(flexflow_model_t m, int l) { return wrap(M(m)->layers.at(l)->outputs[0]); }
void* flexflow_model_get_stream(flexflow_model_t m) { return M(m)->stream; }
double flexflow_model_get_current_lr(flexflow_model_t m) { return M(m)->current_lr(); }
int flexflow_model_uses_graph(flexflow_model_t m) { return M(m)->config.enable_graph ? 1 : 0; }
void flexflow_model_set_trace_mode(flexflow_model_t m, int mode) { M(m)->config.trace_mode = mode; }
int flexflow_model_trace_replays(flexflow_model_t m, int trace_id) { return M(m)->trace_replays(trace_id) ? 1 : 0; }
int64_t flexflow_model_get_counter(flexflow_model_t m, const char* name) {
  const std::string n(name ? name : "");
  if (n == "mlp_chain_fwd_calls") return M(m)->n_chain_fwd_calls;
  if (n == "mlp_chain_bwd_calls") return M(m)->n_chain_bwd_calls;
  if (n == "fused_loss_calls") return M(m)->n_fused_loss_calls;
  if (n == "allreduce_bucket_calls") return M(m)->n_bucket_allreduces;
  if (n == "allreduce_buckets") return (int64_t)M(m)->grad_buckets.size();
  if (n.rfind("allreduce_bucket_floats_", 0) == 0) {
    const size_t k = (size_t)atoi(n.c_str() + 24);
    return k < M(m)->grad_buckets.size() ? (int64_t)M(m)->grad_buckets[k].count : -1;
  }
  if (n == "allreduce_bucket_channel_own") return M(m)->config.comm.bucket_channel_own;
  if (n == "direct_allreduces") return M(m)->n_direct_allreduces;
  if (n == "bf16_updates") return (int64_t)M(m)->read_bf16_counter();
  if (n == "early_sorts") return M(m)->n_early_sorts;
  if (n == "lr_steps") return M(m)->lr_steps();
  if (n == "lr_route") return M(m)->lr_route;
  if (n == "graph_replays") return M(m)->n_graph_replays;
  if (n == "folded_tables") return (int64_t)M(m)->fold.tables.size();
  if (n == "tensor_op_exact_backward_layers") {
    int64_t k = 0;
    for (Op* op : M(m)->layers) if (op->op_type == OP_LINEAR && static_cast<Linear*>(op)->bwd_exact) k++;
    return k;
  }
  return -1;
}

int flexflow_model_save_checkpoint(flexflow_model_t m, const char* dir, int64_t epochs_done) { M(m)->save_checkpoint(dir ? dir : "", epochs_done); return 0; }
int flexflow_model_load_checkpoint(flexflow_model_t m, const char* dir, int64_t* epochs_done) {
  const FFModel::CheckpointInfo info = M(m)->load_checkpoint(dir ? dir : "");
  if (epochs_done) *epochs_done = info.epochs_done;
  return 0;
}
uint64_t flexflow_model_state_digest(flexflow_model_t m) { return M(m)->state_digest(); }
uint64_t flexflow_state_digest_host(const void* base, int64_t rows, int64_t row_bytes, int64_t ld_bytes, uint64_t seed, uint64_t index_base) {
  return ffh_state_digest_host(base, rows, row_bytes, ld_bytes, seed, index_base);
}
uint64_t flexflow_digest_record_seed(uint64_t ordinal) { return ffh_digest_record_seed(ordinal); }

int flexflow_tensor_get_num_dims(flexflow_tensor_t t) { return T(t)->numDim; }
void flexflow_tensor_get_dims(flexflow_tensor_t t, int* dims) { for (int i = 0; i < T(t)->numDim; i++) dims[i] = T(t)->adim[T(t)->numDim - 1 - i]; }
int64_t flexflow_tensor_get_local_rows(flexflow_tensor_t t) { return T(t)->impl ? T(t)->impl->rows_local : 0; }
bool flexflow_tensor_is_local(flexflow_tensor_t t) { return T(t)->impl && T(t)->impl->ptr != nullptr; }
void* flexflow_tensor_get_device_ptr(flexflow_tensor_t t) { return T(t)->impl ? T(t)->impl->ptr : nullptr; }
int64_t flexflow_tensor_get_ld(flexflow_tensor_t t) { return T(t)->impl ? T(t)->impl->ld : 0; }
void flexflow_tensor_set_float(flexflow_tensor_t t, flexflow_model_t m, const int* dims, int nd, const float* d) { T(t)->set_tensor<float>(M(m), dims_vec(dims, nd), d); }
void flexflow_tensor_set_int64(flexflow_tensor_t t, flexflow_model_t m, const int* dims, int nd, const int64_t* d) { T(t)->set_tensor<int64_t>(M(m), dims_vec(dims, nd), d); }
void flexflow_tensor_get_float(flexflow_tensor_t t, flexflow_model_t m, float* d) { T(t)->get_tensor<float>(M(m), d); }
void flexflow_tensor_get_int64(flexflow_tensor_t t, flexflow_model_t m, int64_t* d) { T(t)->get_tensor<int64_t>(M(m), d); }
void flexflow_tensor_get_grad_float(flexflow_tensor_t t, flexflow_model_t m, float* d) { T(t)->get_grad<float>(M(m), d); }
int flexflow_tensor_get_data_type(flexflow_tensor_t t) { return (int)T(t)->data_type; }
void flexflow_tensor_set_bf16(flexflow_tensor_t t, flexflow_model_t m, const int* dims, int nd, const uint16_t* d) {
  if (T(t)->data_type != DT_BF16) { fprintf(stderr, "FATAL: flexflow_tensor_set_bf16: not a bf16 tensor\n"); abort(); }
  T(t)->set_tensor<uint16_t>(M(m), dims_vec(dims, nd), d);
}
void flexflow_tensor_get_bf16(flexflow_tensor_t t, flexflow_model_t m, uint16_t* d) {
  if (T(t)->data_type != DT_BF16) { fprintf(stderr, "FATAL: flexflow_tensor_get_bf16: not a bf16 tensor\n"); abort(); }
  T(t)->get_tensor<uint16_t>(M(m), d);
}

flexflow_dlrm_t flexflow_dlrm_create(int argc, char** argv, const ffcomm* comm) { flexflow_dlrm_t h; h.impl = new DLRMApp(argc, argv, comm); return h; }
void flexflow_dlrm_destroy(flexflow_dlrm_t h) { delete A(h); }
int flexflow_dlrm_get_start_epoch(flexflow_dlrm_t h) { return A(h)->start_epoch; }
flexflow_model_t flexflow_dlrm_get_model(flexflow_dlrm_t h) { flexflow_model_t m; m.impl = A(h)->ff; return m; }
int flexflow_dlrm_get_num_samples(flexflow_dlrm_t h) { return A(h)->loader->num_samples; }
int flexflow_dlrm_get_num_tables(flexflow_dlrm_t h) { return (int)A(h)->sparse_inputs.size(); }
flexflow_tensor_t flexflow_dlrm_get_sparse_input(flexflow_dlrm_t h, int t) { return wrap(A(h)->sparse_inputs.at(t)); }
flexflow_tensor_t flexflow_dlrm_get_dense_input(flexflow_dlrm_t h) { return wrap(A(h)->dense_input); }
void flexflow_dlrm_warmup(flexflow_dlrm_t h) { A(h)->warmup(); }
static void to_c(const EvalMetrics& m, flexflow_eval_metrics_t* out) {
  out->samples = m.samples; out->positives = m.positives; out->correct = m.correct; out->nan_predictions = m.nan_predictions;
  out->logloss_sum = m.logloss_sum; out->auc = m.auc;
}
double flexflow_dlrm_evaluate(flexflow_dlrm_t h, int epoch, flexflow_eval_metrics_t* out) {
  EvalMetrics m;
  const double secs = A(h)->evaluate(epoch, &m);
  if (out) to_c(m, out);
  return secs;
}
float flexflow_perf_metrics_get_bce_loss(flexflow_model_t m) { return M(m)->get_perf_metrics().bce_loss; }
void flexflow_model_eval_batch(flexflow_model_t m) { M(m)->eval_batch(); }
void flexflow_model_reset_eval_metrics(flexflow_model_t m) { M(m)->reset_eval_metrics(); }
void flexflow_model_get_eval_metrics(flexflow_model_t m, flexflow_eval_metrics_t* out, uint64_t* hist_pos, uint64_t* hist_neg) {
  const EvalMetrics e = M(m)->get_eval_metrics(hist_pos || hist_neg);
  to_c(e, out);
  if (hist_pos) memcpy(hist_pos, e.hist_pos.data(), sizeof(uint64_t) * FFH_AUC_BINS);
  if (hist_neg) memcpy(hist_neg, e.hist_neg.data(), sizeof(uint64_t) * FFH_AUC_BINS);
}
int flexflow_auc_bins(void) { return FFH_AUC_BINS; }
double flexflow_auc_from_histograms(const uint64_t* hist_pos, const uint64_t* hist_neg, int bins) { return ffh_auc_from_histograms(hist_pos, hist_neg, bins); }
void flexflow_dlrm_train_steps(flexflow_dlrm_t h, int n, bool trace) { A(h)->train_steps(n, trace); }
double flexflow_dlrm_run_epochs(flexflow_dlrm_t h) { return A(h)->run_epochs(); }

void flexflow_dlrm_probe_step(flexflow_dlrm_t h, int iters, float* out, int nout) {
  DLRMApp* app = A(h);
  FFModel* ff = app->ff;
  for (int k = 0; k < nout; k++) out[k] = 0.0f;
  if (!app->warmed_up) app->warmup();
  ff->sync();
  ff->probe_events_on = true;
  const int npairs = FFModel::kProbeEvents / 2;
  std::vector<double> sum(npairs, 0.0);
  std::vector<int> cnt(npairs, 0);
  for (int i = 0; i < iters + 1; i++) {
    app->train_steps(1, false);
    ff->sync();
    if (i == 0) continue;
    for (int k = 0; k < npairs; k++) {
      if (!ff->probe_ev[2 * k] || !ff->probe_ev[2 * k + 1]) continue;
      float ms = 0.f;
      if (ff->api->ffh_event_elapsed_ms(ff->ctx, ff->probe_ev[2 * k], ff->probe_ev[2 * k + 1], &ms) == 0) { sum[k] += ms; cnt[k]++; }
    }
  }
  ff->probe_events_on = false;
  for (int k = 0; k < npairs && k < nout; k++) out[k] = cnt[k] ? (float)(sum[k] / cnt[k]) : 0.0f;
}

float flexflow_dlrm_time_kernel(flexflow_dlrm_t h, int which, int iters) {
  DLRMApp* app = A(h);
  FFModel* ff = app->ff;
  if (!app->warmed_up) app->warmup();
  ff->sync();
  if (which == 10 || which == 11) {
    if (ff->embeddings.empty() || !ff->config.overlap_embedding) return 0.0f;
    ff->probe_events_on = true;
    double sum = 0.0; int n = 0;
    for (int i = 0; i < iters + 1; i++) {
      app->train_steps(1, false);
      ff->sync();
      const int a = which == 10 ? 0 : 2;
      if (i == 0 || !ff->probe_ev[a] || !ff->probe_ev[a + 1]) continue;
      float ms = 0.f;
      if (ff->api->ffh_event_elapsed_ms(ff->ctx, ff->probe_ev[a], ff->probe_ev[a + 1], &ms) == 0) { sum += ms; n++; }
    }
    ff->probe_events_on = false;
    return n ? (float)(sum / n) : 0.0f;
  }
  constexpr int kProbeSets = 4;
  std::vector<std::vector<const int64_t*>> probe_ids;
  std::vector<void*> probe_bufs;
  if (which == 8 || which == 9) {
    const int L = ff->embeddings.empty() ? 1 : ff->embeddings[0]->inputs[0].adim[0];
    for (int set = 0; set < kProbeSets; set++) {
      std::vector<const int64_t*> ptrs;
      for (const FFModel::EmbShard& sh : ff->shards) {
        if (sh.owner != ff->rank) continue;
        const int64_t n = (int64_t)ff->config.batchSize * L;
        void* buf = nullptr;
        ff->check(ff->api->ffh_malloc(ff->ctx, &buf, (size_t)n * sizeof(int64_t)), "probe ids");
        ff->check(ff->api->ffh_gen_indices(ff->ctx, (int64_t*)buf, n, 0x9e3779b97f4a7c15ull * (uint64_t)(set + 1) + (uint64_t)ptrs.size(), 0, sh.e->num_entries, ff->stream), "probe ids");
        probe_bufs.push_back(buf);
        ptrs.push_back((const int64_t*)buf);
      }
      probe_ids.push_back(ptrs);
    }
  }
  int probe_turn = 0;
  ffh_event e0, e1;
  ff->check(ff->api->ffh_event_create(ff->ctx, &e0), "event");
  ff->check(ff->api->ffh_event_create(ff->ctx, &e1), "event");
  auto body = [&](int n) {
    for (int i = 0; i < n; i++) {
      if (which == 6 || which == 7) {
        Linear* big = nullptr;
        for (Op* op : ff->layers)
          if (Linear* li = dynamic_cast<Linear*>(op))
            if (!big || (double)li->in_channels * li->out_channels > (double)big->in_channels * big->out_channels) big = li;
        if (!big) continue;
        if (which == 6) big->forward(*ff); else big->backward(*ff);
        continue;
      }
      if (which == 8) ff->embedding_kernels_only(true, ff->stream, &probe_ids[probe_turn++ % kProbeSets]);
// ... 45 lines not shown
```

dlrm_flexflow_amd/host/model.cc:

```cpp
#include "ffmodel.h"
#include "model_internal.h"


LaunchWorker::LaunchWorker(const KernelApi* _api, int _device) : api(_api), device(_device), wctx(nullptr), stop(false), busy(false) {
  th = std::thread([this] { run(); });
  drain();
}
LaunchWorker::~LaunchWorker() {
  {
    std::lock_guard<std::mutex> lk(mu);
    stop = true;
  }
  cv.notify_all();
  if (th.joinable()) th.join();
  if (wctx) api->ffh_ctx_destroy(wctx);
}
void LaunchWorker::run() {
  {
    ffh_ctx* c = nullptr;
    if (api->ffh_ctx_create(&c, device) != FFH_OK) die("launch worker: ffh_ctx_create(device %d) failed", device);
    std::lock_guard<std::mutex> lk(mu);
    wctx = c;
  }
  cv_idle.notify_all();
// ... 192 lines not shown
  ff->check(ff->api->ffh_stream_sync(ff->ctx, ff->stream), "NormInitializer sync");
  ff->note_weight_write(p->impl->ptr);
}
void GlorotUniform::init(const FFModel* ff, const Parameter* p) {
  const float fan = (float)(p->adim[0] + (p->numDim > 1 ? p->adim[1] : 0));
  const float scale = std::sqrt(6.0f / fan);
  init_uniform(ff, p, ff->config.seed * 0x9E3779B1ULL + (uint64_t)(uint32_t)seed, -scale, scale, "GlorotUniform");
  ff->note_weight_write(p->impl->ptr);
}

PerfMetrics::PerfMetrics()
    : train_all(0), train_correct(0), cce_loss(0), sparse_cce_loss(0), mse_loss(0), rmse_loss(0), mae_loss(0), bce_loss(0) {
  start_time = now_us();
}
void PerfMetrics::update(const PerfMetrics& o) {
  train_all += o.train_all; train_correct += o.train_correct; cce_loss += o.cce_loss;
  sparse_cce_loss += o.sparse_cce_loss; mse_loss += o.mse_loss; rmse_loss += o.rmse_loss; mae_loss += o.mae_loss; bce_loss += o.bce_loss;
}
void PerfMetrics::print(int flags) const {
  std::string out = "[Metrics]";
  if (flags & 1) {
    const float acc = train_all ? train_correct * 100.0f / train_all : 0.0f;
    out += " accuracy: " + std::to_string(acc) + "% (" + std::to_string(train_correct) + " / " + std::to_string(train_all) + ")";
  }
  if (flags & 2) out += " mean_squared_error: " + std::to_string(train_all ? mse_loss / train_all : 0.0f);
  if (flags & 4) out += " root_mean_squared_error: " + std::to_string(train_all ? rmse_loss / train_all : 0.0f);
  if (flags & 8) out += " mean_absolute_error: " + std::to_string(train_all ? mae_loss / train_all : 0.0f);
  if (flags & 16) out += " binary_crossentropy: " + std::to_string(train_all ? bce_loss / (train_all / ((flags & 1) ? 2 : 1)) : 0.0f);
  fprintf(stderr, "%s\n", out.c_str());
}

std::string FFModel::get_operator_type_name(OperatorType type) const {
  switch (type) {
    case OP_LINEAR: return "Dense";
    case OP_EMBEDDING: return "Embedding";
    case OP_CONCAT: return "Concat";
    case OP_BATCHMATMUL: return "BatchMatmul";
    case OP_TRANSPOSE: return "Transpose";
    case OP_RESHAPE: return "Reshape";
    case OP_FLAT: return "Flat";
    case OP_TRIL: return "Tril";
    case OP_DOT_INTERACTION: return "DotInteraction";
    case OP_CROSS_COMBINE: return "CrossCombine";
    default: return "Unknown";
  }
}

Op::Op(FFModel& model, OperatorType type, const char* _name, int num_inputs, const Tensor* _inputs)
    : op_type(type), numInputs(num_inputs), numWeights(0), numOutputs(1), layer_index(-1), profiling(model.config.profiling) {
  std::string pc = (_name == nullptr ? model.get_operator_type_name(type) : std::string(_name)) + "_" +
                   std::to_string(model.op_global_guid++);
  if (pc.length() >= MAX_OPNAME) die("operator name too long: %s", pc.c_str());
  strcpy(name, pc.c_str());
  if (num_inputs > MAX_NUM_INPUTS) die("%s: more than %d inputs", name, MAX_NUM_INPUTS);
  for (int i = 0; i < num_inputs; i++) inputs[i] = _inputs[i];
  outputs[0].owner_op = this;
  outputs[0].owner_idx = 0;
  outputs[0].data_type = DT_FLOAT;
  outputs[0].impl = new TensorImpl();
  model.tensor_impls.push_back(outputs[0].impl);
  outputs[0].impl->guid = (int)model.tensor_impls.size() - 1;
}

void Op::print_layer(const FFModel&) const {
  printf("%s: inputs %d ->", name, numInputs);
  for (int d = outputs[0].numDim - 1; d >= 0; d--) printf(" %d", outputs[0].adim[d]);
  printf("\n");
}

static FFConfig& profiling_schedule(FFConfig& c) {
  if (c.profiling) {
    c.overlap_embedding = false; c.enable_graph = false; c.parallel_dw = false; c.async_launch = false;
    c.fuse_pair = false; c.mlp_chain = false; c.attach_events = false; c.dx_scatter = false; c.timing_events = true;
  }
  return c;
}

FFModel::FFModel(FFConfig& _config)
    : op_global_guid(100), config(profiling_schedule(_config)), optimizer(nullptr), loss_type(LOSS_MEAN_SQUARED_ERROR_AVG_REDUCE),
      metrics_flags(0), seq_length(-1), api(nullptr), ctx(nullptr), stream(nullptr), side_stream(nullptr),
      ev_fork(nullptr), ev_join(nullptr), ev_grad_ready(nullptr), ev_update_done(nullptr), compiled(false),
      emb_forward_issued(false), emb_forward_joined(false), emb_update_pending(false), emb_sorted_early(false), mlp_weights(nullptr), mlp_grads(nullptr), mlp_count(0),
      act_slab(nullptr), act_grad_slab(nullptr), act_grad_bytes(0), workspace(nullptr), workspace_bytes(0), repl_workspace(nullptr), repl_workspace_bytes(0), d_perf(nullptr), d_bce_sum(nullptr), d_eval(nullptr), want_eval(false), evaluating(false),
      xsend(nullptr), xrecv(nullptr), gsend(nullptr), grecv(nullptr), capturing_trace(-1), replaying_trace(-1), inputs_dirty(true), fork_recorded(false) {
  seed_counter = 0;
  dw_stream = nullptr; ev_dw_done = nullptr; big_dw_layer = -1; need_zero_act_grads = true; need_zero_gsend = true; dw_forked = false; mlp_grads_clean = false; dw_worker = side_worker = nullptr;
  rank = config.comm.world_size > 1 ? config.comm.rank : 0;
  world_size = config.comm.world_size > 1 ? config.comm.world_size : 1;
  if (world_size == 1 && config.workersPerNode > 1)
    die("-ll:gpu %d: one process per GPU and no communicator was supplied; use the `dlrm` binary (it starts its own %d ranks),\n"
        "       python dlrm_flexflow_amd/run_dlrm.py <flags>, or bench.py --gpus %d",
        config.workersPerNode, config.workersPerNode, config.workersPerNode);
  if (world_size > 1 && (!config.comm.alltoall_f32 || !config.comm.allreduce_sum_f32))
    die("world_size %d needs the ffcomm callbacks", world_size);
  if (config.batchSize % world_size != 0) die("batch size %d is not divisible by %d ranks", config.batchSize, world_size);
  local_batch = config.batchSize / world_size;
  exchange = world_size > 1 || (config.force_exchange && config.comm.alltoall_f32 && config.comm.allreduce_sum_f32);
  api = load_kernel_api(config.backend_lib);
  int rc = api->ffh_ctx_create(&ctx, config.device);
  if (rc != FFH_OK || !ctx) die("ffh_ctx_create(device %d) failed with %d on %s -- no usable GPU?", config.device, rc, api->path.c_str());
  if (config.allow_tensor_op_math_conversion) check(api->ffh_ctx_set_math_mode(ctx, FFH_MATH_TENSOR_OP_BF16), "tensor-op math mode");
  else if (config.fp32_split_bf16x3) check(api->ffh_ctx_set_math_mode(ctx, FFH_MATH_FP32_SPLIT_BF16X3), "split-bf16x3 math mode");
  if (config.deterministic) { check(api->ffh_ctx_set_deterministic(ctx, 1), "deterministic mode"); config.async_launch = false; }
  check(api->ffh_stream_create(ctx, &stream), "stream create");
  check(api->ffh_ctx_reserve_scratch(ctx, stream), "reserve scratch");
  check(api->ffh_stream_create(ctx, &side_stream), "stream create");
  check(api->ffh_stream_create(ctx, &dw_stream), "stream create");
  check(api->ffh_ctx_reserve_scratch(ctx, dw_stream), "reserve scratch");
  check(api->ffh_stream_create(ctx, &ar_stream), "stream create");
  check((config.timing_events ? api->ffh_event_create : api->ffh_event_create_sync)(ctx, &ev_dw_done), "event create");
  check((config.timing_events ? api->ffh_event_create : api->ffh_event_create_sync)(ctx, &ev_z_free), "event create");
  z_reader_layer = -1; z_free_recorded = false;
  dw_worker = side_worker = nullptr;
  if (config.async_launch && (std::string(api->ffh_backend_name()).rfind("hip", 0) == 0 || config.force_async_launch)) {
    dw_worker = new LaunchWorker(api, config.device);
    side_worker = new LaunchWorker(api, config.device);
    const int mm = config.allow_tensor_op_math_conversion ? FFH_MATH_TENSOR_OP_BF16 : (config.fp32_split_bf16x3 ? FFH_MATH_FP32_SPLIT_BF16X3 : FFH_MATH_DEFAULT);
    if (mm != FFH_MATH_DEFAULT) {
      check(api->ffh_ctx_set_math_mode(dw_worker->ctx(), mm), "math mode");
      check(api->ffh_ctx_set_math_mode(side_worker->ctx(), mm), "math mode");
    }
  }
  check((config.timing_events ? api->ffh_event_create : api->ffh_event_create_sync)(ctx, &ev_fork), "event create");
  check((config.timing_events ? api->ffh_event_create : api->ffh_event_create_sync)(ctx, &ev_join), "event create");
  check((config.timing_events ? api->ffh_event_create : api->ffh_event_create_sync)(ctx, &ev_grad_ready), "event create");
  check((config.timing_events ? api->ffh_event_create : api->ffh_event_create_sync)(ctx, &ev_update_done), "event create");
}

FFModel::~FFModel() {
  if (!ctx) return;
  delete dw_worker; delete side_worker;
  api->ffh_device_sync(ctx);
  for (ffh_event e : layer_events) api->ffh_event_destroy(ctx, e);
  for (auto& kv : graphs) api->ffh_graph_destroy(ctx, kv.second);
  for (TensorImpl* t : tensor_impls) {
    if (t->ptr && !t->alias && t->bytes) api->ffh_free(ctx, t->ptr);
    delete t;
  }
  for (void* p : {w_twin, act_twin, grad_twin, (void*)ar_scratch}) if (p) api->ffh_free(ctx, p);
  for (void* p : {(void*)mlp_weights, (void*)mlp_grads, (void*)act_slab, (void*)act_grad_slab, workspace, repl_workspace, (void*)d_perf, (void*)d_bce_sum, (void*)d_eval, (void*)digest_acc, (void*)xsend,
                  (void*)xrecv, (void*)gsend, (void*)grecv})
    if (p) api->ffh_free(ctx, p);
  for (Embedding* e : embeddings)
    for (void* p : {(void*)e->local_idx, (void*)e->partial, (void*)e->gfull, (void*)e->opt_state[0], (void*)e->opt_state[1]})
      if (p) api->ffh_free(ctx, p);
  for (Op* op : layers)
    if (op->op_type == OP_LINEAR && static_cast<Linear*>(op)->dx_map) api->ffh_free(ctx, static_cast<Linear*>(op)->dx_map);
  api->ffh_event_destroy(ctx, ev_fork); api->ffh_event_destroy(ctx, ev_join);
  api->ffh_event_destroy(ctx, ev_grad_ready); api->ffh_event_destroy(ctx, ev_update_done);
  api->ffh_event_destroy(ctx, ev_dw_done);
  api->ffh_event_destroy(ctx, ev_z_free);
  if (ev_fold_w) api->ffh_event_destroy(ctx, ev_fold_w);
  if (ev_fold_done) api->ffh_event_destroy(ctx, ev_fold_done);
  for (void* p : {(void*)fold.P, (void*)fold.S}) if (p) api->ffh_free(ctx, p);
  for (auto& kv : trace_tune) for (ffh_event& e : kv.second.ev) if (e) { api->ffh_event_destroy(ctx, e); e = nullptr; }
  for (ffh_event& e : probe_ev) if (e) { api->ffh_event_destroy(ctx, e); e = nullptr; }
  api->ffh_stream_destroy(ctx, stream); api->ffh_stream_destroy(ctx, side_stream); api->ffh_stream_destroy(ctx, dw_stream); api->ffh_stream_destroy(ctx, ar_stream);
  for (GradBucket& b : grad_buckets) { api->ffh_event_destroy(ctx, b.ready); api->ffh_event_destroy(ctx, b.ready_dw); api->ffh_event_destroy(ctx, b.done); }
  api->ffh_ctx_destroy(ctx);
  for (Op* op : layers) delete op;
  for (Initializer* i : owned_initializers) delete i;
  for (Tensor* t : input_tensors) delete t;
}

void FFModel::check(int rc, const char* what) const {
  if (rc != FFH_OK) die("%s failed (%d): %s", what, rc, api->ffh_last_error_string(ctx));
}

void* FFModel::dmalloc(size_t bytes) const {
  void* p = nullptr;
  int rc = api->ffh_malloc(ctx, &p, bytes);
  if (rc != FFH_OK || !p) die("device allocation of %zu bytes failed: %s", bytes, api->ffh_last_error_string(ctx));
  return p;
}

template <int NDIM>
Tensor FFModel::create_tensor(const int dims[], DataType data_type, const Op* owner_op, bool create_grad) {
  (void)create_grad;
  Tensor t;
  t.numDim = NDIM;
  t.data_type = data_type;
  t.owner_op = const_cast<Op*>(owner_op);
  for (int i = 0; i < NDIM; i++) t.adim[i] = dims[NDIM - 1 - i];
  t.impl = new TensorImpl();
  tensor_impls.push_back(t.impl);
  t.impl->guid = (int)tensor_impls.size() - 1;
  t.impl->is_input = owner_op == nullptr;
  if (owner_op == nullptr) {
    Tensor* keep = new Tensor(t);
    input_tensors.push_back(keep);
  }
  return t;
}
template Tensor FFModel::create_tensor<1>(const int[], DataType, const Op*, bool);
template Tensor FFModel::create_tensor<2>(const int[], DataType, const Op*, bool);
template Tensor FFModel::create_tensor<3>(const int[], DataType, const Op*, bool);
template Tensor FFModel::create_tensor<4>(const int[], DataType, const Op*, bool);

template <int NDIM>
Parameter FFModel::create_weight(const int dims[], const Op* op, DataType data_type, Initializer* initializer, bool) {
  Parameter p;
  p.numDim = NDIM;
  p.data_type = data_type;
  p.owner_op = const_cast<Op*>(op);
  p.sync_type = world_size > 1 ? NCCL : PS;
  for (int i = 0; i < NDIM; i++) p.adim[i] = dims[NDIM - 1 - i];
  p.impl = new TensorImpl();
  tensor_impls.push_back(p.impl);
  p.impl->guid = (int)tensor_impls.size() - 1;
  (void)initializer;
  return p;
}
template Parameter FFModel::create_weight<1>(const int[], const Op*, DataType, Initializer*, bool);
template Parameter FFModel::create_weight<2>(const int[], const Op*, DataType, Initializer*, bool);

Tensor FFModel::dense(const Tensor& input, int outDim, ActiMode activation, bool use_bias, const Op* shared_op,
                      Initializer* kernel_initializer, Initializer* bias_initializer, const char* name) {
  if (kernel_initializer == nullptr) kernel_initializer = new GlorotUniform(next_seed());
  if (bias_initializer == nullptr) bias_initializer = new ZeroInitializer();
  Linear* li = new Linear(*this, input, outDim, activation, use_bias, shared_op, kernel_initializer, bias_initializer, name);
  li->layer_index = (int)layers.size();
  layers.push_back(li);
  return li->outputs[0];
}

Tensor FFModel::embedding(const Tensor& input, int num_entries, int outDim, AggrMode aggr, const Op* shared_op,
                          Initializer* kernel_initializer, const char* name) {
  if (kernel_initializer == nullptr) kernel_initializer = new GlorotUniform(next_seed());
  Embedding* e = new Embedding(*this, input, num_entries, outDim, aggr, shared_op, kernel_initializer, name);
  e->layer_index = (int)layers.size();
  layers.push_back(e);
  return e->outputs[0];
}

Tensor FFModel::concat(int n, const Tensor* tensors, int axis, const char* name) {
  Concat* c = new Concat(*this, n, tensors, axis, name);
  c->layer_index = (int)layers.size();
  layers.push_back(c);
  return c->outputs[0];
}

Tensor FFModel::batch_matmul(const Tensor& A, const Tensor& B, int a_seq_length_dim, int b_seq_length_dim) {
  BatchMatmul* b = new BatchMatmul(*this, A, B, a_seq_length_dim, b_seq_length_dim);
  b->layer_index = (int)layers.size();
  layers.push_back(b);
  return b->outputs[0];
}

Linear::Linear(FFModel& model, const Tensor& input, int out_dim, ActiMode _activation, bool _use_bias, const Op* shared_op,
               Initializer* ki, Initializer* bi, const char* name)
    : Op(model, OP_LINEAR, name, 1, &input), in_channels(input.adim[0]), out_channels(out_dim), in_padded(input.adim[0]), activation(_activation),
      use_bias(_use_bias), discard_input_grad(input.owner_op == nullptr), dx_overwrite(false), dx_map(nullptr), dx_map_concat(nullptr), pair_upper(nullptr), fwd_done_by_pair(false), pair_lower(nullptr), dx_mask_by_x(false), dy_premasked(false), colsum_lower(nullptr), db_from_upper(false), fwd_done_by_chain(false),
      kernel_initializer(ki), bias_initializer(bi) {
  if (shared_op) die("%s: weight sharing is not supported on this path", this->name);
  if (input.data_type != DT_FLOAT) die("%s: input must be DT_FLOAT", this->name);
  if (activation != AC_MODE_NONE && activation != AC_MODE_RELU && activation != AC_MODE_SIGMOID && activation != AC_MODE_GELU)
    die("%s: activation %d not supported (NONE, RELU, SIGMOID, GELU)", this->name, (int)activation);
  outputs[0].numDim = input.numDim;
  for (int i = 1; i < input.numDim; i++) outputs[0].adim[i] = input.adim[i];
  outputs[0].adim[0] = out_dim;
  numWeights = use_bias ? 2 : 1;
}
void Linear::create_output_and_partition(FFModel&) {}
void Linear::create_weights(FFModel& model) {
  const int kdims[2] = {out_channels, in_channels};
  weights[0] = model.create_weight<2>(kdims, this, DT_FLOAT, kernel_initializer);
  if (use_bias) {
    const int bdims[1] = {out_channels};
    weights[1] = model.create_weight<1>(bdims, this, DT_FLOAT, bias_initializer);
  }
}
void Linear::forward(const FFModel& ff) {
  const Tensor& x = inputs[0];
  const Tensor& y = outputs[0];
  const int64_t b = local_rows(y, &ff);
  if (fwd_done_by_pair) { fwd_done_by_pair = false; return; }
  if (fwd_done_by_chain) { fwd_done_by_chain = false; return; }
  if (!chain_fwd.empty() && ff.mlp_chain_usable(b, true)) {
    const int rc = ff.run_chain_fwd(this);
    if (rc == FFH_OK) { for (size_t i = 1; i < chain_fwd.size(); i++) chain_fwd[i]->fwd_done_by_chain = true; return; }
    if (rc != FFH_ERR_UNSUPPORTED) ff.check(rc, name);
    chain_fwd.clear();
  }
  if (pair_upper) {
    Linear* up = pair_upper;
    const Tensor& yu = up->outputs[0];
    const int rc = ff.api->ffh_linear_pair_fwd(ff.ctx, (const float*)x.impl->ptr, x.impl->ld, (const float*)weights[0].impl->ptr,
                                               use_bias ? (const float*)weights[1].impl->ptr : nullptr, in_channels, (int)activation, (float*)y.impl->ptr,
                                               y.impl->ld, out_channels, (const float*)up->weights[0].impl->ptr,
                                               up->use_bias ? (const float*)up->weights[1].impl->ptr : nullptr, up->out_channels, (int)up->activation,
                                               (float*)yu.impl->ptr, yu.impl->ld, b, ff.stream);
    if (rc == FFH_OK) { up->fwd_done_by_pair = true; return; }
    if (rc != FFH_ERR_UNSUPPORTED) ff.check(rc, name);
    pair_upper = nullptr;
  }
  if (ff.fold.layer == this) { ff.fold_linear_forward(this); return; }
  ff.check(ff.api->ffh_linear_fwd(ff.ctx, (const float*)x.impl->ptr, x.impl->ld, (float*)y.impl->ptr, y.impl->ld,
                                  (const float*)weights[0].impl->ptr, use_bias ? (const float*)weights[1].impl->ptr : nullptr,
                                  in_padded, out_channels, b, (int)activation, ff.stream), name);
  if (out_twin && out_twin_x3) ff.check(ff.api->ffh_convert_f32_to_bf16x3(ff.ctx, (const float*)y.impl->ptr, b, out_channels, y.impl->ld, ff.stream), name);
  else if (out_twin) ff.check(ff.api->ffh_convert_f32_to_bf16(ff.ctx, out_twin, (const float*)y.impl->ptr, b * (int64_t)y.impl->ld, ff.stream), name);
}
int Linear::backward_pair(const FFModel& ff) {
  Linear* lo = pair_lower;
  const Tensor &xu = inputs[0], &yu = outputs[0], &xl = lo->inputs[0];
  const int64_t b = local_rows(yu, &ff);
  const int flags_u = dy_premasked ? FFH_LINEAR_DY_PREMASKED : 0;
  const int flags_l = (lo->dx_overwrite ? FFH_LINEAR_DX_OVERWRITE : 0) | (lo->dx_mask_by_x ? FFH_LINEAR_DX_MASK_BY_X : 0);
  const int rc = ff.api->ffh_linear_pair_bwd(
      ff.ctx, (const float*)xu.impl->ptr, xu.impl->ld, (const float*)yu.impl->ptr, yu.impl->ld, yu.impl->grad, yu.impl->grad_ld,
      (const float*)weights[0].impl->ptr, weights[0].impl->grad, (use_bias && !db_from_upper) ? weights[1].impl->grad : nullptr, in_channels, out_channels,
      (int)activation, flags_u, (const float*)xl.impl->ptr, xl.impl->ld, xl.impl->grad, xl.impl->grad_ld, xu.impl->grad, xu.impl->grad_ld,
      (const float*)lo->weights[0].impl->ptr, lo->in_channels, (int)lo->activation, flags_l, b, ff.stream);
  if (rc != FFH_OK) return rc;
  db_from_upper = false;
  ff.check(ff.api->ffh_linear_bwd_ex(ff.ctx, (const float*)xl.impl->ptr, xl.impl->ld, nullptr, xl.impl->grad_ld, (const float*)xu.impl->ptr, xu.impl->ld,
                                     xu.impl->grad, xu.impl->grad_ld, (const float*)lo->weights[0].impl->ptr, lo->weights[0].impl->grad,
                                     lo->use_bias ? lo->weights[1].impl->grad : nullptr, lo->in_channels, lo->out_channels, b, (int)lo->activation,
                                     FFH_LINEAR_ONLY_DW | FFH_LINEAR_DY_PREMASKED, ff.stream, nullptr), lo->name);
  return FFH_OK;
}
void Linear::backward(const FFModel& ff) { backward_part(ff, 0); }

void Linear::backward_part(const FFModel& ff, int part) {
  if (activation == AC_MODE_GELU) die("%s: GELU has no backward (forward / inference only, as in the reference)", name);
  const Tensor& x = inputs[0];
  const Tensor& y = outputs[0];
  const int64_t b = local_rows(y, &ff);
  float* dx = discard_input_grad ? nullptr : x.impl->grad;
  const double macs = (double)in_channels * out_channels * (double)b;
  const bool fork = ff.config.parallel_dw && macs >= 1.0e8;
  const int flags = (dx_overwrite ? FFH_LINEAR_DX_OVERWRITE : 0) | (dx_mask_by_x ? FFH_LINEAR_DX_MASK_BY_X : 0) | (dy_premasked ? FFH_LINEAR_DY_PREMASKED : 0);
  const float *xp = (const float*)x.impl->ptr, *yp = (const float*)y.impl->ptr, *wp = (const float*)weights[0].impl->ptr;
  float *dyp = y.impl->grad, *dwp = weights[0].impl->grad, *dbp = (use_bias && !db_from_upper) ? weights[1].impl->grad : nullptr;
  const int64_t ldx = x.impl->ld, lddx = x.impl->grad_ld, ldy = y.impl->ld, lddy = y.impl->grad_ld;
  if (part != 1) db_from_upper = false;
  struct ColsumScope {
    const FFModel& ff; Linear* lo;
    ColsumScope(const FFModel& f, Linear* l, bool produces_dx) : ff(f), lo(produces_dx ? l : nullptr) {
      if (lo) ff.check(ff.api->ffh_linear_bwd_set_dx_colsum(ff.ctx, lo->weights[1].impl->grad, lo->out_channels), "dx colsum");
    }
    ~ColsumScope() { if (lo) lo->db_from_upper = ff.api->ffh_linear_dx_colsum_used(ff.ctx) != 0; }
  } colsum_scope(ff, colsum_lower, dx != nullptr && (part == 0 || part == 1) && !ff.use_workers() && !ff.config.profiling);
  auto image_dx = [&] {
    if (dx_image && dx) ff.check(ff.api->ffh_convert_f32_to_bf16x3(ff.ctx, dx, b, in_channels, lddx, ff.stream), name);
    if (bwd_exact && dx && dx_twin) ff.check(ff.api->ffh_convert_f32_to_bf16(ff.ctx, dx_twin, dx, b * (int64_t)in_channels, ff.stream), name);
  };
  struct ExactScope {
    const FFModel& ff; bool on;
    ExactScope(const FFModel& f, bool o) : ff(f), on(o) { if (on) ff.check(ff.api->ffh_ctx_set_math_mode(ff.ctx, FFH_MATH_DEFAULT), "math mode"); }
    ~ExactScope() { if (on) ff.check(ff.api->ffh_ctx_set_math_mode(ff.ctx, FFH_MATH_TENSOR_OP_BF16), "math mode"); }
  } exact_scope(ff, bwd_exact && !ff.use_workers());
  if (part == 1) {
    ff.check(ff.api->ffh_linear_bwd_ex(ff.ctx, xp, ldx, dx, lddx, yp, ldy, dyp, lddy, wp, dwp, dbp, in_padded, out_channels, b, (int)activation,
                                       flags | FFH_LINEAR_ONLY_DX, ff.stream, nullptr), name);
    image_dx();
    return;
  }
  if (fork && ff.use_workers()) {
    const KernelApi* api = ff.api;
    ffh_stream dws = ff.dw_stream;
    ffh_event ev = ff.layer_events[layer_index];
    const int in = in_padded, out = out_channels, act = (int)activation;
    const char* nm = name;
    auto dw_call = [=](ffh_ctx* wc) {
      int rc = api->ffh_stream_wait_event(wc, dws, ev);
      if (rc == FFH_OK) rc = api->ffh_linear_bwd_ex(wc, xp, ldx, nullptr, lddx, yp, ldy, dyp, lddy, wp, dwp, dbp, in, out, b, act, flags | FFH_LINEAR_ONLY_DW, dws, nullptr);
      if (rc != FFH_OK) die("%s (weight gradient) failed (%d): %s", nm, rc, api->ffh_last_error_string(wc));
    };
    const bool sig = activation == AC_MODE_SIGMOID;
    if (!sig) { ff.check(api->ffh_event_record(ff.ctx, ev, ff.stream), "event"); ff.dw_worker->post(dw_call); }
    ff.check(api->ffh_linear_bwd_ex(ff.ctx, xp, ldx, dx, lddx, yp, ldy, dyp, lddy, wp, dwp, dbp, in, out, b, act, flags | FFH_LINEAR_ONLY_DX, ff.stream, nullptr), name);
    if (sig) { ff.check(api->ffh_event_record(ff.ctx, ev, ff.stream), "event"); ff.dw_worker->post(dw_call); }
    ff.dw_forked = true;
    return;
  }
  ffh_stream dws = ff.dw_stream;
  ff.check(ff.api->ffh_linear_bwd_ex(ff.ctx, xp, ldx, dx, lddx, yp, ldy, dyp, lddy, wp, dwp, dbp, in_padded, out_channels, b, (int)activation,
                                     flags, ff.stream, fork ? dws : nullptr), name);
  image_dx();
  if (fork) { ff.dw_forked = true; ff.dw1_used = true; }
}

void Linear::backward_dw_rows(const FFModel& ff, int row0, int nrows) {
  const Tensor& x = inputs[0];
  const Tensor& y = outputs[0];
  const int64_t b = local_rows(y, &ff);
  const float *xp = (const float*)x.impl->ptr, *yp = (const float*)y.impl->ptr + row0;
  float *dyp = y.impl->grad + row0, *dwp = weights[0].impl->grad + (size_t)row0 * (size_t)weights[0].impl->ld;
  const float* wp = (const float*)weights[0].impl->ptr + (size_t)row0 * (size_t)weights[0].impl->ld;
  float* dbp = (use_bias && !db_from_upper) ? weights[1].impl->grad + row0 : nullptr;
  const int flags = FFH_LINEAR_ONLY_DW | FFH_LINEAR_DY_PREMASKED;
  ff.check(ff.api->ffh_linear_bwd_ex(ff.ctx, xp, x.impl->ld, nullptr, x.impl->grad_ld, yp, y.impl->ld, dyp, y.impl->grad_ld, wp, dwp, dbp, in_padded, nrows, b,
                                     (int)activation, flags, ff.dw_stream, nullptr), name);
  ff.dw_forked = true;
  ff.dw1_used = true;
  ff.dw_stream_used_directly = true;
}

bool FFModel::mlp_chain_usable(int64_t rows, bool fwd) const {
  return config.mlp_chain && !config.profiling && !use_workers() && !config.allow_tensor_op_math_conversion && rows <= config.mlp_chain_max_batch && (!fwd || (rows >= config.mlp_chain_fwd_min_batch && rows <= config.mlp_chain_fwd_max_batch));
}
static void fill_chain(const std::vector<Linear*>& ch, ffh_chain_layer* out) {
  for (size_t i = 0; i < ch.size(); i++) {
    const Linear* li = ch[i];
    ffh_chain_layer& d = out[i];
    d.w = (const float*)li->weights[0].impl->ptr;
    d.bias = li->use_bias ? (const float*)li->weights[1].impl->ptr : nullptr;
    d.y = (float*)li->outputs[0].impl->ptr; d.ldy = li->outputs[0].impl->ld;
    d.dy = li->outputs[0].impl->grad; d.lddy = li->outputs[0].impl->grad_ld;
    d.dw = li->weights[0].impl->grad;
    d.db = (li->use_bias && !li->db_from_upper) ? li->weights[1].impl->grad : nullptr;
    d.ldw = (int)li->weights[0].impl->ld; d.in_dim = li->in_padded; d.out_dim = li->out_channels; d.activation = (int)li->activation;
  }
}
int FFModel::run_chain_fwd(const Linear* lowest) const {
  const std::vector<Linear*>& ch = lowest->chain_fwd;
  ffh_chain_layer ls[FFH_CHAIN_MAX_LAYERS];
  fill_chain(ch, ls);
  const Tensor& x = lowest->inputs[0];
  const int rc = api->ffh_mlp_chain_fwd(ctx, (const float*)x.impl->ptr, x.impl->ld, ls, (int)ch.size(), local_rows(lowest->outputs[0], this), stream);
  if (rc == FFH_OK) n_chain_fwd_calls++;
  return rc;
}
int FFModel::run_chain_bwd(Linear* top) {
  const std::vector<Linear*>& ch = top->chain_bwd;
  ffh_chain_layer ls[FFH_CHAIN_MAX_LAYERS];
  fill_chain(ch, ls);
  Linear* lo = ch.front();
  const Tensor& x = lo->inputs[0];
  const int flags = (top->dy_premasked ? FFH_LINEAR_DY_PREMASKED : 0) | (lo->dx_overwrite ? FFH_LINEAR_DX_OVERWRITE : 0) |
                    (lo->dx_mask_by_x ? FFH_LINEAR_DX_MASK_BY_X : 0);
  const int rc = api->ffh_mlp_chain_bwd(ctx, (const float*)x.impl->ptr, x.impl->ld, lo->discard_input_grad ? nullptr : x.impl->grad, x.impl->grad_ld, ls,
                                        (int)ch.size(), local_rows(top->outputs[0], this), flags, stream);
  if (rc == FFH_OK) { n_chain_bwd_calls++; for (Linear* li : ch) li->db_from_upper = false; }
  return rc;
}

Embedding::Embedding(FFModel& model, const Tensor& input, int _num_entries, int outDim, AggrMode _aggr, const Op* shared_op,
                     Initializer* ki, const char* name)
    : Op(model, OP_EMBEDDING, name, 1, &input), num_entries(_num_entries), out_channels(outDim), aggr(_aggr),
      kernel_initializer(ki) {
  if (shared_op) die("%s: weight sharing is not supported on this path", this->name);
  if (input.data_type != DT_INT64) die("%s: input must be DT_INT64", this->name);
  if (input.numDim != 2) die("%s: input must be [batch][bag]", this->name);
  if (input.owner_op != nullptr) die("%s: input must be a model input tensor", this->name);
  if (aggr != AGGR_MODE_SUM && aggr != AGGR_MODE_AVG) die("%s: aggr must be SUM or AVG", this->name);
  outputs[0].numDim = 2;
  outputs[0].adim[0] = outDim;
  outputs[0].adim[1] = input.adim[1];
  numWeights = 1;
  table_index = (int)model.embeddings.size();
  owner_rank = table_index % model.world_size;
  column_sharded = model.world_size > 1 && model.config.column_shard_rows > 0 && num_entries >= model.config.column_shard_rows;
  if (column_sharded && outDim % model.world_size != 0) die("%s: out_dim %d is not divisible by %d ranks", this->name, outDim, model.world_size);
  local_cols = column_sharded ? outDim / model.world_size : outDim;
  local_idx = nullptr; partial = gfull = nullptr;
  row_sharded = false; row_begin = 0; rows_local = num_entries;
  set_row_sharding(model, model.exchange && model.config.row_shard_rows > 0 && num_entries >= model.config.row_shard_rows);
  replicated = false;
  set_replicated(model, model.exchange && model.world_size > 1 && !row_sharded && !column_sharded && model.config.replicate_embedding_rows > 0 &&
                            num_entries <= model.config.replicate_embedding_rows);
  model.embeddings.push_back(this);
}
void Embedding::set_replicated(const FFModel& model, bool on) {
  if (on && !model.config.comm.allreduce_sum_f32) die("%s: a data-parallel table needs the allreduce callback of ffcomm", this->name);
  replicated = on;
  if (on) {
    set_row_sharding(model, false);
    column_sharded = false;
    local_cols = out_channels;
    owner_rank = -1;
  } else if (owner_rank < 0 && !row_sharded) {
    owner_rank = table_index % model.world_size;
  }
}
void Embedding::set_row_sharding(const FFModel& model, bool on) {
  if (on && (!model.config.comm.reduce_scatter_sum_f32 || !model.config.comm.allgather_f32))
    die("%s: --row-shard-rows needs the reduce_scatter / allgather callbacks of ffcomm", this->name);
  if (on && num_entries < model.world_size) die("%s: %d rows cannot be split over %d ranks", this->name, num_entries, model.world_size);
  row_sharded = on;
  if (on) {
    column_sharded = false;
    local_cols = out_channels;
    owner_rank = -1;
    row_begin = (int64_t)num_entries * model.rank / model.world_size;
    rows_local = (int64_t)num_entries * (model.rank + 1) / model.world_size - row_begin;
  } else {
    row_begin = 0;
    rows_local = num_entries;
    if (owner_rank < 0) owner_rank = table_index % model.world_size;
  }
}
void Embedding::create_output_and_partition(FFModel&) {}
void Embedding::create_weights(FFModel& model) {
  const int dims[2] = {row_sharded ? (int)rows_local : num_entries, local_cols};
  const DataType dt = model.config.embedding_dtype == DT_BF16 && !replicated ? DT_BF16 : DT_FLOAT;
  weights[0] = model.create_weight<2>(dims, this, dt, kernel_initializer);
}
void Embedding::forward(const FFModel& ff) {
  if (ff.emb_forward_issued) return;
  if (ff.config.overlap_embedding) {
    ff.issue_embedding_forward_on_side_stream();
  } else {
    ff.embedding_group_forward(ff.stream);
    ff.emb_forward_issued = true;
    ff.emb_forward_joined = true;
  }
}
void Embedding::backward(const FFModel& ff) {
  if (table_index != (int)ff.embeddings.size() - 1) return;
  ff.replicated_embedding_grads();
  if (ff.fused_embedding_update()) {
    if (ff.config.overlap_embedding) {
      if (!ff.grad_ready_attached) ff.check(ff.api->ffh_event_record(ff.ctx, ff.ev_grad_ready, ff.stream), "event");
      if (ff.exchange && !ff.config.comm.nonblocking && !ff.use_workers()) {
        ff.emb_update_pending = true;
      } else {
        ff.issue_embedding_update_on_side_stream();
      }
    }
    return;
  }
  if (ff.exchange) return;
  for (Embedding* e : ff.embeddings) {
    if (e->owner_rank != ff.rank || e->replicated) continue;
    const Tensor& in = e->inputs[0];
    const Tensor& out = e->outputs[0];
    const float* g = out.impl->grad;
    int64_t gld = out.impl->grad_ld, batch = ff.local_batch;
// ... 413 lines not shown
```

dlrm_flexflow_amd/host/model_allocate.cc:

```cpp
#include "model_internal.h"

int FFModel::tables_of_rank(int r) const {
  int n = 0;
  for (const Embedding* e : embeddings) n += e->owner_rank == r;
  return n;
}

int FFModel::next_seed() {
  return (int)(ffh_hash(config.seed * 0x9E3779B97F4A7C15ULL + 0x5EED, seed_counter++) & 0x7fffffffULL);
}

bool FFModel::fused_embedding_update() const {
  if (config.dense_embedding_update) return false;
  const SGDOptimizer* sgd = dynamic_cast<const SGDOptimizer*>(optimizer);
  if (sgd && sgd->momentum == 0.0 && sgd->weight_decay == 0.0) return true;
  const AdagradOptimizer* adagrad = dynamic_cast<const AdagradOptimizer*>(optimizer);
  if (adagrad && adagrad->weight_decay == 0.0) return true;
  return config.sparse_embedding_optimizer && (sgd || adagrad || dynamic_cast<const AdamOptimizer*>(optimizer));
}

bool FFModel::sparse_rule(ffh_sparse_opt& o) const {
  memset(&o, 0, sizeof o);
  if (const SGDOptimizer* sgd = dynamic_cast<const SGDOptimizer*>(optimizer)) {
    o.lr = (float)sgd->lr;
// ... 749 lines not shown
    auto twin_linear = [&](const Op* op) {
      const Linear* l = op && op->op_type == OP_LINEAR ? static_cast<const Linear*>(op) : nullptr;
      return l && l->in_channels >= FFH_BF16_MIN_DIM && l->out_channels >= FFH_BF16_MIN_DIM &&
             (!x3_images || 2.0 * (double)local_rows(l->outputs[0], this) * (double)l->in_padded * (double)l->out_channels >= FFH_BF16X3_MIN_FLOP);
    };
    auto in_slab = [&](const void* q) { return (const char*)q >= act_slab && (const char*)q < act_slab + act_bytes; };
    for (Op* op : layers) {
      TensorImpl* im = op->outputs[0].impl;
      if (!im || !im->ptr || alias_of.count(im) || !in_slab(im->ptr) || !im->pieces.empty()) continue;
      bool act_ok = false;
      if (twin_linear(op)) {
        act_ok = true;
        if (x3_images) {
          act_ok = false;
          for (Op* q : layers)
            for (int i = 0; i < q->numInputs; i++)
              if (q->inputs[i].impl == im && twin_linear(q)) act_ok = true;
        }
      }
      else if (Concat* c = dynamic_cast<Concat*>(op)) {
        act_ok = !exchange && c->numInputs > 0 && (!x3_images || im->ld % 32 == 0);
        std::vector<int> x3_convert;
        c->image_inputs.clear();
        for (int i = 0; i < c->numInputs && act_ok; i++) {
          const Tensor& in = c->inputs[i];
          auto it = alias_of.find(in.impl);
          if (it == alias_of.end() || it->second.first != c || !in.owner_op) { act_ok = false; break; }
          if (in.owner_op->op_type == OP_EMBEDDING) act_ok = static_cast<const Embedding*>(in.owner_op)->out_channels % 4 == 0 && !static_cast<const Embedding*>(in.owner_op)->replicated;
          else if (x3_images && in.owner_op->op_type == OP_LINEAR && !twin_linear(in.owner_op) && !use_workers()) x3_convert.push_back(i);
          else act_ok = twin_linear(in.owner_op);
        }
        if (act_ok) c->image_inputs = x3_convert;
      }
      const Linear* only = nullptr; int ncons = 0;
      for (Op* q : layers)
        for (int i = 0; i < q->numInputs; i++)
          if (q->inputs[i].impl == im) { ncons++; only = q->op_type == OP_LINEAR ? static_cast<const Linear*>(q) : nullptr; }
      if (!act_ok && config.bf16_convert_twins && op->op_type == OP_LINEAR && ncons == 1 && only && twin_linear(only) && !use_workers() && im->ld % 8 == 0) {
        Linear* li = static_cast<Linear*>(op);
        if (!li->pair_upper && !li->pair_lower) {
          li->out_twin = twin_at(act_twin, (size_t)((const char*)im->ptr - act_slab));
          li->out_twin_x3 = x3_images;
          act_ok = li->out_twin != nullptr;
        }
      }
      if (act_ok && !reg(im->ptr, im->bytes, twin_at(act_twin, (size_t)((const char*)im->ptr - act_slab)))) {
        if (op->op_type == OP_LINEAR) { static_cast<Linear*>(op)->out_twin = nullptr; static_cast<Linear*>(op)->out_twin_x3 = false; }
        if (Concat* c = dynamic_cast<Concat*>(op)) c->image_inputs.clear();
      }
      auto skinny_twin = [&](const Linear* l) {
        return l && l->out_channels <= 4 && l->in_channels >= FFH_BF16_MIN_DIM && l->in_channels <= 1024 && l->in_channels % 4 == 0 && !config.deterministic;
      };
      const Linear* prod = op->op_type == OP_LINEAR ? static_cast<const Linear*>(op) : nullptr;
      const bool twin_read = prod && twin_linear(prod) && (prod->dy_premasked || prod->activation == AC_MODE_NONE);
      if (ncons == 1 && twin_read && only && (twin_linear(only) || skinny_twin(only)) && only->dx_overwrite && !only->discard_input_grad && im->grad && !exchange) {
        const bool registered = reg(im->grad, im->bytes, twin_at(grad_twin, (size_t)((const char*)im->grad - act_grad_slab)));
        if (!x3_images && registered) {
          Linear* o = const_cast<Linear*>(only);
          o->dx_twin_registered = true;
          if (im->grad_ld == op->outputs[0].adim[0]) o->dx_twin = twin_at(grad_twin, (size_t)((const char*)im->grad - act_grad_slab));
        }
      }
      else if (x3_images && ncons == 1 && twin_read && only && only->dx_overwrite && !only->discard_input_grad && im->grad && !exchange && !use_workers() &&
               !only->pair_upper && !only->pair_lower && twin_at(grad_twin, (size_t)((const char*)im->grad - act_grad_slab))) {
        if (reg(im->grad, im->bytes, twin_at(grad_twin, (size_t)((const char*)im->grad - act_grad_slab)))) const_cast<Linear*>(only)->dx_image = true;
      }
    }
  }
  if (config.allow_tensor_op_math_conversion && !x3_images && config.bf16_exact_small_backward && !use_workers())
    for (Op* op : layers) {
      if (op->op_type != OP_LINEAR) continue;
      Linear* li = static_cast<Linear*>(op);
      const double flop = 2.0 * (double)local_rows(li->outputs[0], this) * (double)li->in_padded * (double)li->out_channels;
      if (li->in_channels < FFH_BF16_MIN_DIM || li->out_channels < FFH_BF16_MIN_DIM || flop >= 4.0e9) continue;
      if (li->dy_premasked || (li->activation != AC_MODE_RELU && li->activation != AC_MODE_SIGMOID)) continue;
      if (li->pair_upper || li->pair_lower || (li->dx_twin_registered && !li->dx_twin)) continue;
      li->bwd_exact = true;
    }
  if (x3_images)
    for (Op* op : layers) {
      if (op->op_type != OP_LINEAR) continue;
      Linear* li = static_cast<Linear*>(op);
      auto converts = [](const std::vector<Linear*>& ch) { for (const Linear* m : ch) if (m->out_twin || m->dx_image) return true; return false; };
      if (converts(li->chain_fwd)) li->chain_fwd.clear();
      if (converts(li->chain_bwd)) li->chain_bwd.clear();
    }
  plan_fold();
  check(api->ffh_stream_sync(ctx, stream), "allocate sync");
}

void FFModel::plan_fold() {
  fold = FoldRoute();
  if (!config.fold_small_tables || !api->fold || exchange || world_size != 1 || embeddings.empty()) return;
  if (config.allow_tensor_op_math_conversion || config.fp32_split_bf16x3) return;
  for (Op* op : layers) {
    Linear* li = dynamic_cast<Linear*>(op);
    if (!li) continue;
    const Tensor& x = li->inputs[0];
    Concat* c = x.owner_op ? dynamic_cast<Concat*>(const_cast<Op*>(x.owner_op)) : nullptr;
    if (!c || c->axis != 0 || !x.impl->pieces.empty() || !x.impl->ptr) continue;
    if (li->in_padded != li->in_channels || li->pair_upper || li->out_channels % FFH_FOLD_NTILE || li->in_channels % FFH_FOLD_KTILE) continue;
    if (!li->chain_fwd.empty() && mlp_chain_usable(local_rows(li->outputs[0], this), true)) continue;
    FoldRoute r;
    int64_t off = 0, prows = 0;
    int32_t kept_from = 0;
    for (int i = 0; i < c->numInputs; i++) {
      const Tensor& in = c->inputs[i];
      const int64_t w = in.adim[0];
      Embedding* e = in.owner_op && in.owner_op->op_type == OP_EMBEDDING ? static_cast<Embedding*>(const_cast<Op*>(in.owner_op)) : nullptr;
      const bool in_place = in.impl->pieces.empty() && in.impl->ptr == (float*)x.impl->ptr + off && in.impl->ld == x.impl->ld;
      const bool ok = e && in_place && e->aggr == AGGR_MODE_SUM && !e->replicated && !e->row_sharded && !e->column_sharded && !e->bf16_weights() &&
                      e->held_here(rank) && e->out_channels == w && w % FFH_FOLD_KTILE == 0 && off % FFH_FOLD_KTILE == 0 &&
                      e->num_entries <= config.fold_max_rows && 4 * (int64_t)e->num_entries <= 3 * local_batch &&
                      (r.tables.empty() || (e->out_channels == r.tables[0]->out_channels && e->inputs[0].adim[0] == r.tables[0]->inputs[0].adim[0])) &&
                      (int)r.tables.size() < FFH_FOLD_MAX_GROUPS;
      if (ok) {
        if (off > kept_from) r.keep.push_back(ffh_fold_seg{kept_from, (int32_t)(off - kept_from)});
        kept_from = (int32_t)(off + w);
        r.tables.push_back(e);
        prows += e->num_entries;
      }
      off += w;
    }
    if (off != li->in_channels || r.tables.empty()) continue;
    if (off > kept_from) r.keep.push_back(ffh_fold_seg{kept_from, (int32_t)(off - kept_from)});
    if (r.keep.empty() || r.keep.size() > (size_t)FFH_FOLD_MAX_SEGS) continue;
    const int out = li->out_channels;
    r.P = (float*)dmalloc((size_t)prows * out * 4);
    r.S = (float*)dmalloc((size_t)local_batch * out * 4);
    const int plan = api->fold->ffh_fold_linear_fwd_plan(ctx, (const float*)x.impl->ptr, x.impl->ld, (const float*)li->outputs[0].impl->ptr, li->outputs[0].impl->ld,
                                                         (const float*)li->weights[0].impl->ptr, li->use_bias ? (const float*)li->weights[1].impl->ptr : nullptr,
                                                         li->in_padded, out, local_rows(li->outputs[0], this), r.keep.data(), (int)r.keep.size(), r.S, out);
    if (plan < 1) { api->ffh_free(ctx, r.P); api->ffh_free(ctx, r.S); continue; }
    int64_t prow = 0, col = 0;
    size_t k = 0;
    for (int i = 0; i < c->numInputs; i++) {
      const Tensor& in = c->inputs[i];
      if (k < r.tables.size() && in.owner_op == r.tables[k]) {
        Embedding* e = r.tables[k++];
        float* p = r.P + (size_t)prow * out;
        r.groups.push_back(ffh_fold_group{(const float*)e->weights[0].impl->ptr, (int64_t)e->out_channels, col, p, (int64_t)e->num_entries});
        ffh_emb_table t;
        t.idx = (const int64_t*)e->inputs[0].impl->ptr;
        t.weight = p;
        t.num_entries = e->num_entries;
        t.io = nullptr;
        t.ld = out;
        r.gather.push_back(t);
        prow += e->num_entries;
      }
      col += in.adim[0];
    }
    r.layer = li;
    fold = r;
    if (!ev_fold_w) check((config.timing_events ? api->ffh_event_create : api->ffh_event_create_sync)(ctx, &ev_fold_w), "event create");
    if (!ev_fold_done) check((config.timing_events ? api->ffh_event_create : api->ffh_event_create_sync)(ctx, &ev_fold_done), "event create");
    return;
  }
}

void FFModel::init_layers() {
  if (!compiled) die("init_layers() before compile()");
  for (Op* op : layers) op->init(*this);
}

void FFModel::print_layers(int id) {
  if (id == -1) for (Op* op : layers) op->print_layer(*this);
  else layers.at(id)->print_layer(*this);
}
```

dlrm_flexflow_amd/host/model_flags.cc:

```cpp
#include "model_internal.h"

FFConfig::FFConfig() {
  epochs = 1;
  batchSize = 64;
  printFreq = 10;
  numNodes = 1;
  cpusPerNode = 0;
  workersPerNode = 0;
  learningRate = 0.01f;
  weightDecay = 0.0001f;
  workSpaceSize = (size_t)1 << 30;
  syntheticInput = false;
  profiling = false;
  perform_fusion = false;
  computationMode = COMP_MODE_TRAINING;
  device = 0;
  seed = 0;
  enable_graph = true;
  overlap_embedding = true;
  dense_embedding_update = false;
  force_exchange = false;
  parallel_dw = true;
  async_launch = false;
  column_shard_rows = 0;
  row_shard_rows = 0;
  replicate_embedding_rows = 0;
  fuse_loss = true;
  driver_loss = LOSS_MEAN_SQUARED_ERROR_AVG_REDUCE;
  eval_batches = 0;
  eval_only = false;
  synthetic_labels = 0;
  data_randomize = 0;
  timing_events = false;
  attach_events = true;
  fuse_pair = true;
  mlp_chain = true;
  fold_small_tables = true;
  fold_max_rows = 7420;
  trace_mode = -1;
  bucket_allreduce = -1;
  allreduce_bucket_floats = 1 << 20;
  direct_allreduce = false;
  big_dw_chunks = 0;
  big_dw_min_weights = 2 << 20;
  mlp_chain_max_batch = 8192;
  mlp_chain_fwd_max_batch = 4096;
  mlp_chain_fwd_min_batch = 4096;
  mlp_chain_max_weights = 200000;
  dx_scatter = true;
  dx_colsum = true;
  early_sort = -1;
  pad_linear_k = true;
  capture_exchange = false;
  bf16_twins = true;
  bf16_convert_twins = true;
  bf16_exact_small_backward = true;
  force_async_launch = false;
  sparse_embedding_optimizer = false;
  allow_tensor_op_math_conversion = false;
  fp32_split_bf16x3 = false;
  deterministic = false;
  embedding_dtype = DT_FLOAT;
  embedding_rounding = FFH_BF16_ROUND_STOCHASTIC;
  lr_warmup_steps = lr_decay_start_step = lr_num_decay_steps = 0;
  device_lr = false;
  host_lr_schedule = false;
  checkpoint_every_epochs = 0;
  adagrad_eps = 1e-10;
  adagrad_initial_accumulator = 0.0;
  adagrad_rowwise = false;
  memset(&comm, 0, sizeof comm);
  comm.rank = 0;
  comm.world_size = 1;
}

void FFConfig::parse_args(char** argv, int argc) {
  for (int i = 1; i < argc; i++) {
    const char* eq = strncmp(argv[i], "--", 2) == 0 ? strchr(argv[i], '=') : nullptr;
    auto is = [&](const char* a) { return eq ? (strlen(a) == (size_t)(eq - argv[i]) && !strncmp(argv[i], a, (size_t)(eq - argv[i]))) : !strcmp(argv[i], a); };
    auto next = [&]() -> const char* {
      if (eq) return eq + 1;
      if (i + 1 >= argc) die("flag %s needs a value", argv[i]);
      return argv[++i];
    };
    if (is("-e") || is("--epochs")) { epochs = atoi(next()); continue; }
    if (is("-b") || is("--batch-size")) { batchSize = atoi(next()); continue; }
    if (is("--lr") || is("--learning-rate")) { learningRate = (float)atof(next()); continue; }
    if (is("--wd") || is("--weight-decay")) { weightDecay = (float)atof(next()); continue; }
    if (is("-p") || is("--print-freq")) { printFreq = atoi(next()); continue; }
    if (is("-d") || is("--dataset")) { dataset_path = next(); continue; }
    if (is("--import") || is("--import-strategy")) { import_strategy_file = next(); continue; }
    if (is("--export") || is("--export-strategy")) { export_strategy_file = next(); continue; }
    if (is("-ll:gpu")) { workersPerNode = atoi(next()); continue; }
    if (is("--nodes")) { numNodes = atoi(next()); continue; }
    if (is("-ll:cpu")) { cpusPerNode = atoi(next()); continue; }
    if (is("--profiling")) { profiling = true; continue; }
    if (is("--fusion")) { perform_fusion = true; continue; }
    if (is("-ll:fsize") || is("-ll:zsize") || is("-ll:util") || is("-ll:csize") || is("--budget") || is("--search-budget") ||
        is("--alpha") || is("--search-alpha") || is("--simulator-workspace-size") || is("--strategy") ||
        is("--machine-model-version") || is("--machine-model-file") || is("--simulator-segment-size") ||
        is("--simulator-max-num-segments") || is("--taskgraph")) { next(); continue; }
    if (is("--allow-tensor-op-math-conversion")) { allow_tensor_op_math_conversion = true; continue; }
    if (is("--fp32-split-bf16x3")) { fp32_split_bf16x3 = true; continue; }
    if (is("-dm:memoize") || is("-dm:memorize") || is("--overlap") || is("--enable-parameter-parallel") ||
        is("--enable-attribute-parallel") || is("--enable-propagation")) continue;
    if (is("--seed")) { seed = strtoull(next(), nullptr, 10); continue; }
    if (is("--deterministic")) { deterministic = true; continue; }
    if (is("--backend")) { backend_lib = next(); continue; }
    if (is("--device")) { device = atoi(next()); continue; }
    if (is("--no-trace")) { enable_graph = false; continue; }
    if (is("--no-overlap")) { overlap_embedding = false; continue; }
    if (is("--dense-embedding-update")) { dense_embedding_update = true; continue; }
    if (is("--force-exchange")) { force_exchange = true; continue; }
    if (is("--serial-dw")) { parallel_dw = false; continue; }
    if (is("--inline-launch")) { async_launch = false; continue; }
    if (is("--async-launch")) { async_launch = true; continue; }
    if (is("--column-shard-rows")) { column_shard_rows = atoll(next()); continue; }
    if (is("--row-shard-rows")) { row_shard_rows = atoll(next()); continue; }
    if (is("--replicate-embedding-rows")) { replicate_embedding_rows = atoll(next()); continue; }
    if (is("--no-fused-loss")) { fuse_loss = false; continue; }
    if (is("--loss")) {
      const char* v = next();
      if (!strcmp(v, "mse")) driver_loss = LOSS_MEAN_SQUARED_ERROR_AVG_REDUCE;
      else if (!strcmp(v, "bce")) driver_loss = LOSS_BINARY_CROSSENTROPY;
      else die("--loss %s: 'mse' or 'bce'", v);
      continue;
    }
    if (is("--eval-batches")) { eval_batches = atoi(next()); if (eval_batches < 0) die("--eval-batches %d: must be >= 0", eval_batches); continue; }
    if (is("--eval-only")) { eval_only = true; continue; }
    if (is("--synthetic-labels")) {
      const char* v = next();
      if (!strcmp(v, "bernoulli")) synthetic_labels = 0;
      else if (!strcmp(v, "logistic")) synthetic_labels = 1;
      else die("--synthetic-labels %s: 'bernoulli' or 'logistic'", v);
      continue;
    }
    if (is("--data-randomize")) {
      const char* v = next();
      if (!strcmp(v, "none")) data_randomize = 0;
      else if (!strcmp(v, "total")) data_randomize = 1;
      else die("--data-randomize %s: 'none' or 'total'", v);
      continue;
    }
    if (is("--timing-events")) { timing_events = true; continue; }
    if (is("--no-attach-event")) { attach_events = false; continue; }
    if (is("--no-fused-pair")) { fuse_pair = false; continue; }
    if (is("--no-mlp-chain")) { mlp_chain = false; continue; }
    if (is("--no-fold-small-tables")) { fold_small_tables = false; continue; }
    if (is("--fold-max-rows")) { fold_max_rows = atoll(next()); continue; }
    if (is("--always-replay")) { trace_mode = 1; continue; }
    if (is("--adaptive-replay")) { trace_mode = 0; continue; }
    if (is("--bucket-allreduce")) { bucket_allreduce = 1; continue; }
    if (is("--no-bucket-allreduce")) { bucket_allreduce = 0; continue; }
    if (is("--allreduce-bucket-floats")) { allreduce_bucket_floats = atoll(next()); continue; }
    if (is("--direct-allreduce")) { direct_allreduce = true; continue; }
    if (is("--big-dw-chunks")) { big_dw_chunks = atoi(next()); continue; }
    if (is("--big-dw-min-weights")) { big_dw_min_weights = atoll(next()); continue; }
    if (is("--mlp-chain-max-batch")) { mlp_chain_max_batch = atoll(next()); continue; }
    if (is("--mlp-chain-fwd-min-batch")) { mlp_chain_fwd_min_batch = atoll(next()); continue; }
    if (is("--mlp-chain-fwd-max-batch")) { mlp_chain_fwd_max_batch = atoll(next()); continue; }
    if (is("--mlp-chain-max-weights")) { mlp_chain_max_weights = atoll(next()); continue; }
    if (is("--no-dx-scatter")) { dx_scatter = false; continue; }
    if (is("--no-dx-colsum")) { dx_colsum = false; continue; }
    if (is("--no-early-sort")) { early_sort = 0; continue; }
    if (is("--early-sort")) { early_sort = 1; continue; }
    if (is("--no-pad-linear-k")) { pad_linear_k = false; continue; }
    if (is("--capture-exchange")) { capture_exchange = true; continue; }
    if (is("--no-bf16-exact-small-backward")) { bf16_exact_small_backward = false; continue; }
    if (is("--no-bf16-convert-twins")) { bf16_convert_twins = false; continue; }
    if (is("--no-bf16-twins")) { bf16_twins = false; continue; }
    if (is("--force-async-launch")) { force_async_launch = true; continue; }
    if (is("--sparse-embedding-optimizer")) { sparse_embedding_optimizer = true; continue; }
    if (is("--embedding-dtype")) {
      const char* v = next();
      if (!strcmp(v, "fp32")) embedding_dtype = DT_FLOAT;
      else if (!strcmp(v, "bf16")) embedding_dtype = DT_BF16;
      else die("--embedding-dtype %s: 'fp32' or 'bf16'", v);
      continue;
    }
    if (is("--lr-num-warmup-steps")) { lr_warmup_steps = atoll(next()); continue; }
    if (is("--lr-decay-start-step")) { lr_decay_start_step = atoll(next()); continue; }
    if (is("--lr-num-decay-steps")) { lr_num_decay_steps = atoll(next()); continue; }
    if (is("--save-checkpoint")) { save_checkpoint_dir = next(); if (save_checkpoint_dir.empty()) die("--save-checkpoint: needs a directory"); continue; }
    if (is("--load-checkpoint")) { load_checkpoint_dir = next(); if (load_checkpoint_dir.empty()) die("--load-checkpoint: needs a directory"); continue; }
    if (is("--checkpoint-every-epochs")) {
      checkpoint_every_epochs = atoi(next());
      if (checkpoint_every_epochs < 1) die("--checkpoint-every-epochs %d: must be >= 1", checkpoint_every_epochs);
      continue;
    }
    if (is("--adagrad-eps")) { adagrad_eps = atof(next()); continue; }
    if (is("--adagrad-initial-accumulator")) { adagrad_initial_accumulator = atof(next()); continue; }
    if (is("--adagrad-rowwise")) { adagrad_rowwise = eq ? atoi(eq + 1) != 0 : true; continue; }
    if (is("--device-lr")) { device_lr = true; continue; }
    if (is("--host-lr-schedule")) { host_lr_schedule = true; continue; }
    if (is("--embedding-rounding")) {
      const char* v = next();
      if (!strcmp(v, "stochastic")) embedding_rounding = FFH_BF16_ROUND_STOCHASTIC;
      else if (!strcmp(v, "nearest")) embedding_rounding = FFH_BF16_ROUND_NEAREST;
      else die("--embedding-rounding %s: 'stochastic' or 'nearest'", v);
      continue;
    }
  }
}
```

dlrm_flexflow_amd/host/model_step.cc:

```cpp
#include "model_internal.h"

void FFModel::reset_metrics() {
  if (replaying_trace >= 0) return;
  check(api->ffh_zero(ctx, d_perf, sizeof(ffh_perf_metrics), stream), "reset_metrics");
  if (d_bce_sum) check(api->ffh_zero(ctx, d_bce_sum, sizeof(float), stream), "reset_metrics");
}

void FFModel::refresh_weight_twin() const {
  if (!w_twin || !w_twin_dirty) return;
  if (config.fp32_split_bf16x3 && !config.allow_tensor_op_math_conversion) check(api->ffh_convert_f32_to_bf16x3(ctx, mlp_weights, 1, (int64_t)mlp_count, (int64_t)mlp_count, stream), "weight image");
  else check(api->ffh_convert_f32_to_bf16(ctx, w_twin, mlp_weights, (int64_t)mlp_count, stream), "weight twin");
  w_twin_dirty = false;
}
int64_t FFModel::weight_mirror_stale_bytes() {
  if (!w_twin) return -1;
  if (w_twin_dirty) return -2;
  sync();
  const bool x3 = config.fp32_split_bf16x3 && !config.allow_tensor_op_math_conversion;
  const size_t bytes = x3 ? FFH_BF16X3_IMAGE_BYTES((size_t)mlp_count * 4) : (size_t)mlp_count * 2;
  std::vector<char> kept(bytes), fresh(bytes);
  check(api->ffh_memcpy_d2h(ctx, kept.data(), w_twin, bytes, stream), "weight mirror d2h");
  w_twin_dirty = true;
  refresh_weight_twin();
  check(api->ffh_memcpy_d2h(ctx, fresh.data(), w_twin, bytes, stream), "weight mirror d2h");
  check(api->ffh_stream_sync(ctx, stream), "weight mirror sync");
  int64_t n = 0;
  for (size_t i = 0; i < bytes; i++) n += kept[i] != fresh[i];
  return n;
}
void FFModel::note_weight_write(const void* p) const {
  if (w_twin && (const char*)p >= (const char*)mlp_weights && (const char*)p < (const char*)(mlp_weights + mlp_count)) w_twin_dirty = true;
}

void FFModel::forward(int _seq_length) {
  if (replaying_trace >= 0) return;
  seq_length = _seq_length;
  if (capturing_trace < 0) refresh_weight_twin();
  emb_forward_issued = emb_forward_joined = false;
  fold_w_recorded = fold_on_side = false;
  if (config.overlap_embedding && !embeddings.empty()) {
    fork_recorded = inputs_dirty || capturing_trace >= 0 || use_workers() || repl_workspace != nullptr || !fused_embedding_update();
    if (fork_recorded) check(api->ffh_event_record(ctx, ev_fork, stream), "fork");
    inputs_dirty = false;
    if (fold.layer && !use_workers()) {
      check(api->ffh_event_record(ctx, ev_fold_w, stream), "fold: weights ready");
      fold_w_recorded = true;
    }
    if (!exchange || config.comm.nonblocking || use_workers()) issue_embedding_forward_on_side_stream();
  }
  for (Op* op : layers) {
    if (!config.profiling) { op->forward(*this); continue; }
    if (op->op_type == OP_EMBEDDING && emb_forward_issued) continue;
    profiled(op, true, [&] { op->forward(*this); });
  }
  if (emb_forward_issued && !emb_forward_joined) join_embedding_forward();
}

void FFModel::profiled(const Op* op, bool fwd, const std::function<void()>& fn) const {
  ffh_event e0, e1;
  check(api->ffh_event_create(ctx, &e0), "event");
  check(api->ffh_event_create(ctx, &e1), "event");
  check(api->ffh_event_record(ctx, e0, stream), "event");
  fn();
  check(api->ffh_event_record(ctx, e1, stream), "event");
  check(api->ffh_event_sync(ctx, e1), "event");
  float ms = 0.0f;
  check(api->ffh_event_elapsed_ms(ctx, e0, e1, &ms), "event");
  api->ffh_event_destroy(ctx, e0);
  api->ffh_event_destroy(ctx, e1);
  const char* dir = fwd ? "forward" : "backward";
  switch (op->op_type) {
    case OP_LINEAR:
      if (fwd) printf("%s [Linear] forward time = %.2lfms\n", op->name, (double)ms);
      else printf("Linear backward time = %.2lfms\n", (double)ms);
      break;
    case OP_BATCHMATMUL: printf("BatchMatmul %s time = %.2lfms\n", dir, (double)ms); break;
    case OP_EMBEDDING:
      printf("[Embedding x%zu] %s time = %.4f ms\n", embeddings.size(), dir, ms);
      break;
    default: printf("[%s] %s time = %.4f ms\n", op->name, dir, ms); break;
  }
}

void FFModel::issue_embedding_forward_on_side_stream() const {
  if (use_workers()) {
    const FFModel* self = this;
    side_worker->post([self](ffh_ctx* wc) {
      self->check(self->api->ffh_stream_wait_event(wc, self->side_stream, self->ev_fork), "fork");
      self->embedding_group_forward(self->side_stream, wc);
      self->check(self->api->ffh_event_record(wc, self->ev_join, self->side_stream), "join");
    });
  } else {
    if (fork_recorded) check(api->ffh_stream_wait_event(ctx, side_stream, ev_fork), "fork");
    probe_record(0, side_stream, ctx);
    embedding_group_forward(side_stream);
    probe_record(1, side_stream, ctx);
    check(api->ffh_event_record(ctx, ev_join, side_stream), "join");
    if (fold.layer && fold_w_recorded) {
      check(api->ffh_stream_wait_event(ctx, side_stream, ev_fold_w), "fold: weights ready");
      fold_products_and_sum(side_stream, ctx);
      check(api->ffh_event_record(ctx, ev_fold_done, side_stream), "fold: sum ready");
      fold_on_side = true;
    }
    if (early_sort_possible(1)) {
      launch_shard_groups(this, kSortOnly, side_stream, ctx);
      emb_sorted_early = true;
    }
  }
  emb_forward_issued = true;
  emb_forward_joined = false;
}

void FFModel::fold_products_and_sum(ffh_stream s, ffh_ctx* cx) const {
  const Linear* li = fold.layer;
  const Embedding* e0 = fold.tables[0];
  check(api->fold->ffh_fold_product(cx, fold.groups.data(), (int)fold.groups.size(), (const float*)li->weights[0].impl->ptr, li->in_padded, e0->out_channels,
                                    li->out_channels, s), "fold_product");
  check(api->fold->ffh_fold_gather_add(cx, fold.gather.data(), (int)fold.gather.size(), e0->inputs[0].adim[0], li->out_channels, local_batch, FFH_AGGR_MODE_SUM,
                                       fold.S, li->out_channels, s), "fold_gather_add");
}

void FFModel::fold_linear_forward(const Linear* li) const {
  if (fold_on_side) check(api->ffh_stream_wait_event(ctx, stream, ev_fold_done), "fold: sum ready");
  else fold_products_and_sum(stream, ctx);
  const Tensor& x = li->inputs[0];
  const Tensor& y = li->outputs[0];
  check(api->fold->ffh_fold_linear_fwd(ctx, (const float*)x.impl->ptr, x.impl->ld, (float*)y.impl->ptr, y.impl->ld, (const float*)li->weights[0].impl->ptr,
                                       li->use_bias ? (const float*)li->weights[1].impl->ptr : nullptr, li->in_padded, li->out_channels, local_rows(y, this),
                                       (int)li->activation, fold.keep.data(), (int)fold.keep.size(), fold.S, li->out_channels, stream), li->name);
}

void FFModel::join_embedding_forward() const {
  if (side_worker) side_worker->drain();
  probe_record(10, stream, ctx);
  check(api->ffh_stream_wait_event(ctx, stream, ev_join), "join");
  probe_record(11, stream, ctx);
  emb_forward_joined = true;
}

void FFModel::issue_embedding_update_on_side_stream() const {
  if (use_workers()) {
    const FFModel* self = this;
    side_worker->post([self](ffh_ctx* wc) {
      self->check(self->api->ffh_stream_wait_event(wc, self->side_stream, self->ev_grad_ready), "event");
      self->embedding_group_update(self->side_stream, wc);
      self->check(self->api->ffh_event_record(wc, self->ev_update_done, self->side_stream), "event");
    });
  } else {
    check(api->ffh_stream_wait_event(ctx, side_stream, ev_grad_ready), "event");
    probe_record(2, side_stream, ctx);
    embedding_group_update(side_stream);
    probe_record(3, side_stream, ctx);
    check(api->ffh_event_record(ctx, ev_update_done, side_stream), "event");
  }
}

void FFModel::order_input_writes_behind_update() const {
  if (embeddings.empty() || !config.overlap_embedding || !fused_embedding_update()) return;
  if (side_worker) side_worker->drain();
  check(api->ffh_stream_wait_event(ctx, stream, ev_update_done), "inputs behind the table update");
}

void FFModel::zero_gradients() {
  if (replaying_trace >= 0) return;
  if (need_zero_act_grads) check(api->ffh_zero(ctx, act_grad_slab, act_grad_bytes, stream), "zero_gradients");
  if (!mlp_grads_clean) check(api->ffh_zero(ctx, mlp_grads, mlp_count * 4, stream), "zero_gradients");
  if (exchange && gsend && need_zero_gsend) {
    size_t n = 0;
    for (int64_t c : fwd_recv_counts) n += (size_t)c;
    check(api->ffh_zero(ctx, gsend, n * 4, stream), "zero_gradients");
  }
  if (!fused_embedding_update())
    for (Embedding* e : embeddings)
      if (e->held_here(rank) && !e->replicated)
        check(api->ffh_zero(ctx, e->weights[0].impl->grad, e->weights[0].impl->bytes + (e->row_sharded ? (size_t)e->out_channels * 4 : 0), stream), "zero_gradients");
}

void FFModel::compute_metrics() {
  if (replaying_trace >= 0) return;
  const Tensor& fin = layers.back()->outputs[0];
  check(api->ffh_metrics_update(ctx, (const float*)fin.impl->ptr, (const float*)label_tensor.impl->ptr, d_perf,
                                local_rows(fin, this), fin.adim[0], metrics_flags, stream), "compute_metrics");
}

void FFModel::backward(int _seq_length) {
  if (replaying_trace >= 0) return;
  seq_length = _seq_length;
  if (config.computationMode != COMP_MODE_TRAINING) die("backward() in inference mode");
  const Tensor& fin = layers.back()->outputs[0];
  const bool bce = loss_type == LOSS_BINARY_CROSSENTROPY;
  const float scale = (bce || loss_type == LOSS_MEAN_SQUARED_ERROR_AVG_REDUCE) ? 1.0f / (float)fin.adim[fin.numDim - 1] : 1.0f;
  if (fin.impl->grad_ld != fin.adim[0] || fin.impl->ld != fin.adim[0]) die("final layer output must be contiguous");
  dw_forked = false;
  opt_next_done = false;
  int first = (int)layers.size() - 1;
  emb_update_pending = false;
  mlp_grads_clean = false;
  Linear* last = (config.fuse_loss && !config.profiling) ? dynamic_cast<Linear*>(layers.back()) : nullptr;
  int rc = FFH_ERR_UNSUPPORTED;
  if (last) {
    const Tensor& x = last->inputs[0];
    const int flags = (last->dx_overwrite ? FFH_LINEAR_DX_OVERWRITE : 0) | (last->dx_mask_by_x ? FFH_LINEAR_DX_MASK_BY_X : 0);
    if (bce)
      rc = api->ctr->ffh_linear_bwd_bce(ctx, (const float*)x.impl->ptr, x.impl->ld, last->discard_input_grad ? nullptr : x.impl->grad, x.impl->grad_ld,
                                        (const float*)fin.impl->ptr, fin.impl->ld, fin.impl->grad, fin.impl->grad_ld,
                                        (const float*)last->weights[0].impl->ptr, last->weights[0].impl->grad,
                                        last->use_bias ? last->weights[1].impl->grad : nullptr, last->in_channels, last->out_channels,
                                        local_rows(fin, this), (int)last->activation, flags, (const float*)label_tensor.impl->ptr, scale, d_perf,
                                        d_bce_sum, metrics_flags, stream);
    else
    rc = api->ffh_linear_bwd_mse(ctx, (const float*)x.impl->ptr, x.impl->ld, last->discard_input_grad ? nullptr : x.impl->grad, x.impl->grad_ld,
                                 (const float*)fin.impl->ptr, fin.impl->ld, fin.impl->grad, fin.impl->grad_ld,
                                 (const float*)last->weights[0].impl->ptr, last->weights[0].impl->grad,
                                 last->use_bias ? last->weights[1].impl->grad : nullptr, last->in_channels, last->out_channels,
                                 local_rows(fin, this), (int)last->activation, flags, (const float*)label_tensor.impl->ptr, scale, d_perf,
                                 metrics_flags, stream);
    if (rc == FFH_OK) n_fused_loss_calls++;
    if (rc == FFH_OK) first--;
    else if (rc != FFH_ERR_UNSUPPORTED) check(rc, "loss + last layer backward");
  }
  if (rc != FFH_OK && bce)
    check(api->ctr->ffh_bce_bwd_metrics(ctx, fin.impl->grad, (const float*)fin.impl->ptr, (const float*)label_tensor.impl->ptr, d_perf, d_bce_sum,
                                        local_rows(fin, this), fin.adim[0], scale, metrics_flags, stream), "metrics + loss backward (bce)");
  else if (rc != FFH_OK)
    check(api->ffh_mse_bwd_metrics(ctx, fin.impl->grad, (const float*)fin.impl->ptr, (const float*)label_tensor.impl->ptr, d_perf,
                                   local_rows(fin, this), fin.adim[0], scale, metrics_flags, stream), "metrics + loss backward");
  grad_ready_attached = false;
  z_free_recorded = false;
  auto mark_z_free = [&](int l) {
    if (l == z_reader_layer && dw_forked && !dw_worker && capturing_trace < 0) {
      check(api->ffh_event_record(ctx, ev_z_free, dw_stream), "z free");
      z_free_recorded = true;
    }
  };
  bwd_alltoall_issued = false;
  for (GradBucket& b : grad_buckets) b.issued = b.inline_issued = false;
  const int dw_chunks = big_dw_chunks_now();
  auto chunked_big_backward = [&](Linear* up, int l) {
    ffh_event ev = layer_events[l];
    check(api->ffh_event_record(ctx, ev, stream), "event");
    check(api->ffh_stream_wait_event(ctx, dw_stream, ev), "event");
    up->backward_part(*this, 1);
    const int per = up->out_channels / dw_chunks;
    for (size_t k = 0; k < grad_buckets.size(); k++) {
      GradBucket& b = grad_buckets[k];
      if (b.chunk_layer != l) continue;
      up->backward_dw_rows(*this, b.chunk_index * per, per);
      if (!buckets_held()) issue_one_bucket(k, false);
    }
    up->db_from_upper = false;
  };
  for (int l = first; l >= 0; l--) {
    if (bucketed_now()) issue_grad_buckets(l);
    if (l == grad_attach_layer) {
      check(api->ffh_event_record_with_next_linear_bwd(ctx, ev_grad_ready), "attach event");
      grad_ready_attached = true;
    }
    Linear* up = layers[l]->op_type == OP_LINEAR ? static_cast<Linear*>(layers[l]) : nullptr;
    if (up && up->dx_map && !use_workers()) {
      const bool attach = l == scatter_attach_layer;
      check(api->ffh_linear_bwd_set_dx_scatter(ctx, up->dx_map, up->in_channels, attach ? ev_grad_ready : nullptr), "dx scatter");
      if (dw_chunks > 1 && l == big_dw_layer) { chunked_big_backward(up, l); mark_z_free(l); }
      else { up->backward(*this); mark_z_free(l); }
      if (api->ffh_linear_dx_scatter_used(ctx)) {
        up->dx_map_concat->bwd_done = true;
        if (attach) grad_ready_attached = true;
      }
      continue;
    }
    if (config.profiling) {
      if (layers[l]->op_type == OP_EMBEDDING && static_cast<Embedding*>(layers[l])->table_index != (int)embeddings.size() - 1) continue;
      profiled(layers[l], false, [&] {
        layers[l]->backward(*this);
        if (layers[l]->op_type == OP_EMBEDDING && fused_embedding_update()) embedding_group_update(stream);
      });
      continue;
    }
    if (up && !up->chain_bwd.empty() && mlp_chain_usable(local_rows(up->outputs[0], this), false)) {
      const int n = (int)up->chain_bwd.size();
      const int crc = run_chain_bwd(up);
      if (crc == FFH_OK) {
        if (grad_attach_layer > l - n && grad_attach_layer < l && !grad_ready_attached) {
          check(api->ffh_event_record(ctx, ev_grad_ready, stream), "event");
          grad_ready_attached = true;
        }
        for (int k = 0; k < n; k++) mark_z_free(l - k);
        l -= n - 1;
        continue;
      }
      if (crc != FFH_ERR_UNSUPPORTED) check(crc, up->name);
      up->chain_bwd.clear();
    }
    if (up && up->pair_lower && !use_workers() && l != grad_attach_layer && l >= 1 && layers[l - 1] == up->pair_lower) {
      const int prc = up->backward_pair(*this);
      if (prc == FFH_OK) { l--; continue; }
      if (prc != FFH_ERR_UNSUPPORTED) check(prc, up->name);
      up->pair_lower = nullptr;
    }
    if (up && dw_chunks > 1 && l == big_dw_layer) { chunked_big_backward(up, l); mark_z_free(l); continue; }
    layers[l]->backward(*this);
    mark_z_free(l);
  }
  if (emb_update_pending) {
    issue_embedding_update_on_side_stream();
    emb_update_pending = false;
  }
  if (bucketed_now()) { bwd_alltoall_issued = true; issue_grad_buckets(-1); }
}

void FFModel::update() {
  n_update_calls++;
  if (replaying_trace >= 0) return;
  optimizer->next();
  opt_next_done = true;
  SGDOptimizer* sgd = dynamic_cast<SGDOptimizer*>(optimizer);
  AdamOptimizer* adam = dynamic_cast<AdamOptimizer*>(optimizer);
  AdagradOptimizer* adagrad = dynamic_cast<AdagradOptimizer*>(optimizer);
  if (!sgd && !adam && !adagrad) die("update(): unknown optimizer");
  if (side_worker) side_worker->drain();
  if (dw_forked && !dw_worker && !api->ffh_second_stream_used(ctx, 1) && !dw_stream_used_directly) { dw_forked = false; dw1_used = false; }
  dw_stream_used_directly = false;
  if (dw_forked) {
    if (dw_worker) { dw_worker->drain(); dw1_used = true; }
    if (dw1_used) {
      check(api->ffh_event_record(ctx, ev_dw_done, dw_stream), "join dw");
      check(api->ffh_stream_wait_event(ctx, stream, ev_dw_done), "join dw");
    }
    if (config.overlap_embedding && !embeddings.empty() && !use_workers()) {
      if (z_free_recorded) check(api->ffh_stream_wait_event(ctx, side_stream, ev_z_free), "join dw (embedding stream)");
      else {
        if (dw1_used) check(api->ffh_stream_wait_event(ctx, side_stream, ev_dw_done), "join dw (embedding stream)");
      }
    }
    dw1_used = false;
    dw_forked = false;
  }
  if (exchange && mlp_count) {
    bool any_issued = false;
    for (const GradBucket& b : grad_buckets) any_issued = any_issued || b.issued;
    if (any_issued) {
      for (const GradBucket& b : grad_buckets) if (!b.issued) die("update(): a gradient bucket was not issued");
      probe_record(12, stream, ctx);
      for (const GradBucket& b : grad_buckets) if (!b.inline_issued) check(api->ffh_stream_wait_event(ctx, stream, b.done), "join all-reduce bucket");
      probe_record(13, stream, ctx);
      probe_record(8, stream, ctx);
      for (auto& r : grad_rest)
// ... 327 lines not shown
```

include/ff_hip_fold.h:

```cpp
#ifndef FF_HIP_FOLD_H_
#define FF_HIP_FOLD_H_

#include "ff_hip.h"

#ifdef __cplusplus
extern "C" {
#endif

#define FFH_FOLD_ABI_VERSION 1

#define FFH_FOLD_KTILE      16
#define FFH_FOLD_NTILE      64
#define FFH_FOLD_MAX_GROUPS 64
#define FFH_FOLD_MAX_SEGS   32

typedef struct ffh_fold_group {
  const float* e;
  int64_t      lde;
  int64_t      col0;
  float*       p;
  int64_t      rows;
} ffh_fold_group;

typedef struct ffh_fold_seg { int32_t k0, len; } ffh_fold_seg;

int ffh_fold_abi_version(void);

int ffh_fold_product(ffh_ctx* ctx, const ffh_fold_group* groups, int ngroups, const float* w, int64_t ldw, int d, int out_dim, ffh_stream s);

int ffh_fold_gather_add(ffh_ctx* ctx, const ffh_emb_table* tables, int ntables, int in_dim, int out_dim, int64_t batch, int aggr,
                        float* S, int64_t ldS, ffh_stream s);

int ffh_fold_linear_fwd(ffh_ctx* ctx, const float* x, int64_t ldx, float* y, int64_t ldy, const float* w, const float* bias,
                        int in_dim, int out_dim, int64_t batch, int activation, const ffh_fold_seg* keep, int nkeep,
                        const float* addend, int64_t ldadd, ffh_stream s);

int ffh_fold_linear_fwd_plan(ffh_ctx* ctx, const float* x, int64_t ldx, const float* y, int64_t ldy, const float* w, const float* bias,
                             int in_dim, int out_dim, int64_t batch, const ffh_fold_seg* keep, int nkeep, const float* addend, int64_t ldadd);

#ifdef __cplusplus
}
#endif

#define FFH_FOLD_API_LIST(X) \
  X(ffh_fold_abi_version) X(ffh_fold_product) X(ffh_fold_gather_add) X(ffh_fold_linear_fwd) X(ffh_fold_linear_fwd_plan)

#endif
```

Before: 4.493 million samples/s.

## Fold small-table weight gradient via per-row segment sums and product

Measured after the change: 4.766 million samples/s, median of 6. 6.1% higher.

```diff
diff --git a/dlrm_flexflow_amd/capi.py b/dlrm_flexflow_amd/capi.py
--- a/dlrm_flexflow_amd/capi.py
+++ b/dlrm_flexflow_amd/capi.py
@@ -794,6 +794,10 @@
     "ffh_fold_gather_add": (I, [P, C.POINTER(EmbTable), I, I, I, L, I, P, L, P]),
     "ffh_fold_linear_fwd": (I, [P, P, L, P, L, P, P, I, I, L, I, C.POINTER(FoldSeg), I, P, L, P]),
     "ffh_fold_linear_fwd_plan": (I, [P, P, L, P, L, P, P, I, I, L, C.POINTER(FoldSeg), I, P, L]),
+    "ffh_fold_segment_sum": (I, [P, C.POINTER(EmbTable), I, I, I, L, P]),
+    "ffh_fold_dw_product": (I, [P, C.POINTER(FoldGroup), I, P, L, I, I, P]),
+    "ffh_fold_linear_bwd_dw": (I, [P, P, L, P, L, P, P, I, I, L, C.POINTER(C.c_int32), I, P]),
+    "ffh_fold_linear_bwd_dw_plan": (I, [P, P, L, P, L, P, P, I, I, L, C.POINTER(C.c_int32), I]),
 }
 
 
diff --git a/dlrm_flexflow_amd/csrc/fold.hip b/dlrm_flexflow_amd/csrc/fold.hip
--- a/dlrm_flexflow_amd/csrc/fold.hip
+++ b/dlrm_flexflow_amd/csrc/fold.hip
@@ -117,7 +117,101 @@
   }
 }
 
+constexpr int FOLD_DW_EP_LD = 68;
+struct FoldDwGroup { const float* g; const float* e; int64_t lde; int64_t col0; int rows; int tile0; };
+struct FoldDwArgs {
+  FoldDwGroup grp[FFH_FOLD_MAX_GROUPS];
+  float* dw; int64_t lddw;
+  int ngroups, out, d, ntiles;
+};
+static_assert(sizeof(FoldDwArgs) <= 4096, "kernel arguments");
+
+__global__ __launch_bounds__(256) void fold_dw_product_kernel(const FoldDwArgs g) {
+  __shared__ __attribute__((aligned(16))) float ep_all[4][16 * FOLD_DW_EP_LD];
+  ffh_kernel_prio();
+  const int lane = threadIdx.x & 63;
+  const int wave = __builtin_amdgcn_readfirstlane((int)(threadIdx.x >> 6));
+  const int c = lane & 15, q = lane >> 4;
+  const int wt = (int)blockIdx.x * 4 + wave;
+  if (wt >= g.ntiles) return;
+  int gi = 0;
+  while (gi + 1 < g.ngroups && g.grp[gi + 1].tile0 <= wt) gi++;
+  const FoldDwGroup G = g.grp[gi];
+  const int ot = g.out / 64, dt = g.d / 64, local = wt - G.tile0;
+  const int chunk = local / (ot * dt), rem = local - chunk * (ot * dt);
+  const int o0 = (rem / dt) * 64, d0 = (rem % dt) * 64;
+  const int rb = chunk * FFH_FOLD_DW_CHUNK;
+  const int re = rb + FFH_FOLD_DW_CHUNK < G.rows ? rb + FFH_FOLD_DW_CHUNK : G.rows;
+  const float* gp = G.g + o0 + 4 * c;
+  const float* epn = G.e + d0 + 4 * c;
+  f32x4 acc[4][4];
+#pragma unroll
+  for (int tm = 0; tm < 4; tm++)
+#pragma unroll
+    for (int tn = 0; tn < 4; tn++) acc[tm][tn] = f32x4{0.f, 0.f, 0.f, 0.f};
+  f32x4 a[4], b[4], an[4], bn[4];
+  auto load16 = [&](int k, f32x4* av, f32x4* bv) {
+#pragma unroll
+    for (int u = 0; u < 4; u++) {
+      const int r = k + 4 * u + q;
+      const int rc = r < re ? r : re - 1;
+      av[u] = *reinterpret_cast<const f32x4*>(gp + (int64_t)rc * g.out);
+      bv[u] = *reinterpret_cast<const f32x4*>(epn + (int64_t)rc * G.lde);
+      if (r >= re) av[u] = f32x4{0.f, 0.f, 0.f, 0.f};
+    }
+  };
+  load16(rb, a, b);
+  for (int k = rb; k < re; k += 16) {
+    if (k + 16 < re) load16(k + 16, an, bn);
+#pragma unroll
+    for (int u = 0; u < 4; u++)
+#pragma unroll
+      for (int tm = 0; tm < 4; tm++)
+#pragma unroll
+        for (int tn = 0; tn < 4; tn++) acc[tm][tn] = __builtin_amdgcn_mfma_f32_16x16x4f32(a[u][tm], b[u][tn], acc[tm][tn], 0, 0, 0);
+#pragma unroll
+    for (int u = 0; u < 4; u++) { a[u] = an[u]; b[u] = bn[u]; }
+  }
+  float* const ep = ep_all[wave];
+  float* crow = g.dw + (int64_t)o0 * g.lddw + G.col0 + d0 + lane;
+#pragma unroll
+  for (int p = 0; p < 4; p++) {
+    if (q == p) {
+#pragma unroll
+      for (int tm = 0; tm < 4; tm++)
+#pragma unroll
+        for (int i = 0; i < 4; i++)
+          *reinterpret_cast<f32x4*>(ep + (4 * i + tm) * FOLD_DW_EP_LD + 4 * c) = f32x4{acc[tm][0][i], acc[tm][1][i], acc[tm][2][i], acc[tm][3][i]};
+    }
+    __builtin_amdgcn_wave_barrier();
+#pragma unroll
+    for (int r = 0; r < 16; r++) atomicAdd(crow + (int64_t)(16 * p + r) * g.lddw, ep[r * FOLD_DW_EP_LD + lane]);
+    __builtin_amdgcn_wave_barrier();
+  }
+}
+
 inline bool al16(const void* p) { return ((uintptr_t)p & 15) == 0; }
+
+int fold_dw_check(ffh_ctx* c, const float* x, int64_t ldx, const float* dy, int64_t lddy, const float* dw, int in, int out, int64_t batch,
+                  const int32_t* kept, int nkept) {
+  FFH_REQUIRE(c, in > 0 && out > 0 && batch >= 0 && ldx >= in && lddy >= out, "fold_linear_bwd_dw: bad dims");
+  FFH_REQUIRE(c, batch == 0 || (x && dy && dw), "fold_linear_bwd_dw: null pointer");
+  FFH_REQUIRE(c, batch < (1LL << 31), "fold_linear_bwd_dw: batch too large");
+  FFH_REQUIRE(c, nkept >= 1 && kept, "fold_linear_bwd_dw: bad tile list");
+  for (int i = 0; i < nkept; i++)
+    FFH_REQUIRE(c, kept[i] >= 0 && ((int64_t)kept[i] + 1) * FFH_FOLD_DW_NTILE <= in && (i == 0 || kept[i] > kept[i - 1]), "fold_linear_bwd_dw: tiles must ascend inside [0, in_dim)");
+  return FFH_OK;
+}
+GemmArgs fold_dw_gemm(const float* x, int64_t ldx, const float* dy, int64_t lddy, float* dw, float* db, int in, int out, int64_t batch) {
+  GemmArgs g{};
+  g.A = dy; g.sAm = 1; g.sAk = lddy;
+  g.B = x; g.sBn = 1; g.sBk = ldx;
+  g.C = dw; g.ldc = in;
+  g.M = out; g.N = in; g.K = (int)batch;
+  g.epi = EPI_ATOMIC; g.act = FFH_AC_MODE_NONE;
+  g.db = db;
+  return g;
+}
 
 int fold_fwd_check(ffh_ctx* c, const float* x, int64_t ldx, const float* y, int64_t ldy, const float* w, int in, int out, int64_t batch,
                    const ffh_fold_seg* keep, int nkeep, const float* addend, int64_t ldadd) {
@@ -249,4 +343,65 @@
   return FFH_OK;
 }
 
-}
+int ffh_fold_segment_sum(ffh_ctx* c, const ffh_emb_table* tables, int ntables, int in_dim, int width, int64_t batch, ffh_stream s) {
+  FFH_REQUIRE(c, tables && ntables >= 1 && in_dim >= 1 && width > 0 && batch >= 0, "fold_segment_sum: bad arguments");
+  if (ntables > FFH_MAX_TABLES || batch * in_dim >= (1LL << 31)) return ffh_fail(c, FFH_ERR_UNSUPPORTED, "fold_segment_sum: at most 64 tables, batch * in_dim < 2^31");
+  for (int t = 0; t < ntables; t++)
+    FFH_REQUIRE(c, tables[t].weight && tables[t].num_entries >= 1 && (batch == 0 || (tables[t].idx && tables[t].io && tables[t].ld >= width)), "fold_segment_sum: bad table");
+  if (batch > 0 && (!c->ws || c->ws_bytes < ffh_embedding_bwd_workspace_bytes(ntables, in_dim, width, batch) || ((uintptr_t)c->ws & 15)))
+    return ffh_fail(c, FFH_ERR_WORKSPACE, "fold_segment_sum: workspace too small (ffh_embedding_bwd_workspace_bytes) or not 16-byte aligned");
+  for (int t = 0; t < ntables;) {
+    char* p0 = (char*)tables[t].weight;
+    size_t bytes = 0;
+    for (; t < ntables && (char*)tables[t].weight == p0 + bytes; t++) bytes += (size_t)tables[t].num_entries * (size_t)width * 4;
+    const int rc = ffh_zero(c, p0, bytes, s);
+    if (rc != FFH_OK) return rc;
+  }
+  if (batch == 0) return FFH_OK;
+  return ffh_embedding_bwd_sgd_fused_multi(c, tables, ntables, in_dim, width, batch, FFH_AGGR_MODE_SUM, -1.0f, s);
+}
+
+int ffh_fold_dw_product(ffh_ctx* c, const ffh_fold_group* groups, int ngroups, float* dw, int64_t lddw, int d, int out, ffh_stream s) {
+  FFH_REQUIRE(c, groups && dw && ngroups >= 1 && d > 0 && out > 0 && lddw >= d, "fold_dw_product: bad arguments");
+  if (ngroups > FFH_FOLD_MAX_GROUPS || d % 64 || out % FFH_FOLD_NTILE) return ffh_fail(c, FFH_ERR_UNSUPPORTED, "fold_dw_product: d and out_dim multiples of 64, at most 64 tables");
+  FoldDwArgs a{};
+  int64_t tiles = 0;
+  for (int i = 0; i < ngroups; i++) {
+    const ffh_fold_group& gr = groups[i];
+    FFH_REQUIRE(c, gr.e && gr.p && gr.rows >= 1 && gr.rows < (1LL << 31) && gr.lde >= d && gr.col0 >= 0 && gr.col0 + d <= lddw, "fold_dw_product: bad group");
+    if (!al16(gr.e) || !al16(gr.p) || gr.lde % 4) return ffh_fail(c, FFH_ERR_UNSUPPORTED, "fold_dw_product: group not aligned");
+    a.grp[i] = FoldDwGroup{gr.p, gr.e, gr.lde, gr.col0, (int)gr.rows, (int)tiles};
+    tiles += ((gr.rows + FFH_FOLD_DW_CHUNK - 1) / FFH_FOLD_DW_CHUNK) * (out / 64) * (d / 64);
+    FFH_REQUIRE(c, tiles < (1LL << 30), "fold_dw_product: too many rows");
+  }
+  a.dw = dw; a.lddw = lddw; a.ngroups = ngroups; a.out = out; a.d = d; a.ntiles = (int)tiles;
+  hipLaunchKernelGGL(fold_dw_product_kernel, dim3((unsigned)((tiles + 3) / 4)), dim3(256), 0, as_stream(s), a);
+  FFH_LAUNCH_CHECK(c, "fold_dw_product_kernel");
+  return FFH_OK;
+}
+
+int ffh_fold_linear_bwd_dw_plan(ffh_ctx* c, const float* x, int64_t ldx, const float* dy, int64_t lddy, const float* dw, const float* db, int in, int out,
+                                int64_t batch, const int32_t* kept, int nkept) {
+  const int rc = fold_dw_check(c, x, ldx, dy, lddy, dw, in, out, batch, kept, nkept);
+  if (rc != FFH_OK) return rc;
+  if (batch == 0 || c->math_mode != FFH_MATH_DEFAULT) return 0;
+  const GemmArgs g = fold_dw_gemm(x, ldx, dy, lddy, const_cast<float*>(dw), const_cast<float*>(db), in, out, batch);
+  if (!gemm_sk_serves(c, g, SK_FORM_DW)) return 0;
+  return launch_gemm_sk_kept(c, g, kept, nkept, true, nullptr, "") == 1 ? 1 : 0;
+}
+
+int ffh_fold_linear_bwd_dw(ffh_ctx* c, const float* x, int64_t ldx, const float* dy, int64_t lddy, float* dw, float* db, int in, int out, int64_t batch,
+                           const int32_t* kept, int nkept, ffh_stream s) {
+  const int rc = fold_dw_check(c, x, ldx, dy, lddy, dw, in, out, batch, kept, nkept);
+  if (rc != FFH_OK) return rc;
+  ffh_route_clear(c);
+  if (batch == 0 || c->math_mode != FFH_MATH_DEFAULT) return ffh_fail(c, FFH_ERR_UNSUPPORTED, "fold_linear_bwd_dw: empty batch / math mode not served");
+  const GemmArgs g = fold_dw_gemm(x, ldx, dy, lddy, dw, db, in, out, batch);
+  if (!gemm_sk_serves(c, g, SK_FORM_DW)) return ffh_fail(c, FFH_ERR_UNSUPPORTED, "fold_linear_bwd_dw: the layer's weight gradient does not run the stream-K form");
+  const int r = launch_gemm_sk_kept(c, g, kept, nkept, false, s, "fold_linear_bwd_dw gemm");
+  if (r < 0) return r;
+  if (r == 0) return ffh_fail(c, FFH_ERR_UNSUPPORTED, "fold_linear_bwd_dw: too few kept tiles for the stream-K form, deterministic mode, or a bias gradient without tile 0");
+  return FFH_OK;
+}
+
+}
diff --git a/dlrm_flexflow_amd/csrc/linear_gemm.h b/dlrm_flexflow_amd/csrc/linear_gemm.h
--- a/dlrm_flexflow_amd/csrc/linear_gemm.h
+++ b/dlrm_flexflow_amd/csrc/linear_gemm.h
@@ -86,5 +86,6 @@
 int launch_gemm_sk(ffh_ctx* c, const GemmArgs& g, int form, ffh_stream s, const char* name);
 int launch_gemm_sk_fold(ffh_ctx* c, const GemmArgs& g, const unsigned long long keep[2], int nk_kept, const float* addend, int64_t ldadd, bool dry,
                         ffh_stream s, const char* name);
+int launch_gemm_sk_kept(ffh_ctx* c, const GemmArgs& g, const int* tiles, int nkept, bool dry, ffh_stream s, const char* name);
 
 }
diff --git a/dlrm_flexflow_amd/csrc/linear_sk.hip b/dlrm_flexflow_amd/csrc/linear_sk.hip
--- a/dlrm_flexflow_amd/csrc/linear_sk.hip
+++ b/dlrm_flexflow_amd/csrc/linear_sk.hip
@@ -41,6 +41,11 @@
   int64_t            ldadd;
 };
 
+struct SkArgsKept : SkArgs {
+  unsigned       nkept;
+  unsigned short tile[128];
+};
+
 template <int... I, class F>
 __device__ __forceinline__ void sk_static_for_impl(std::integer_sequence<int, I...>, F&& f) { (f(std::integral_constant<int, I>{}), ...); }
 template <int N_, class F>
@@ -52,8 +57,9 @@
 constexpr int SK_EP_ROWS = 16;
 constexpr int SK_EP_WAVE = SK_EP_ROWS * SK_EP_LD * 4;
 
-template <bool AKR, bool BKR, int EPI, bool DB = false, bool SPLIT = false, int TMW = 4, bool FOLD = false>
-__global__ __launch_bounds__(256, 1) void gemm_sk_kernel(const std::conditional_t<FOLD, SkArgsFold, SkArgs> g) {
+template <bool AKR, bool BKR, int EPI, bool DB = false, bool SPLIT = false, int TMW = 4, bool FOLD = false, bool KEPT = false>
+__global__ __launch_bounds__(256, 1) void gemm_sk_kernel(const std::conditional_t<KEPT, SkArgsKept, std::conditional_t<FOLD, SkArgsFold, SkArgs>> g) {
+  static_assert(!KEPT || (EPI == SK_EPI_DW_ATOMIC && AKR && BKR && !FOLD), "kept column tiles: the weight-gradient form");
   static_assert(!FOLD || (EPI == SK_EPI_FWD && !SPLIT && !DB && TMW == 4), "kept k-tiles + addend: the whole-tile forward form");
   static_assert(!DB || (EPI == SK_EPI_DW_ATOMIC && AKR), "the bias gradient rides on the weight-gradient form");
   static_assert(!SPLIT || EPI != SK_EPI_DW_ATOMIC, "the weight gradient meets by atomics");
@@ -87,7 +93,9 @@
   const __amdgpu_buffer_rsrc_t rsA = __builtin_amdgcn_make_buffer_rsrc(const_cast<float*>(g.A), 0, g.a_bytes, 0x00020000);
   const __amdgpu_buffer_rsrc_t rsB = __builtin_amdgcn_make_buffer_rsrc(const_cast<float*>(g.B), 0, g.b_bytes, 0x00020000);
 
-  const unsigned nbx = (unsigned)(g.N / SK_BN), nby = (unsigned)(g.M / BM), ntiles = nbx * nby;
+  unsigned nbx = (unsigned)(g.N / SK_BN);
+  if constexpr (KEPT) nbx = g.nkept;
+  const unsigned nby = (unsigned)(g.M / BM), ntiles = nbx * nby;
   unsigned nk = (unsigned)(g.K / SK_BK);
   if constexpr (FOLD) nk = g.nk_kept;
   auto first_kept = [&]() -> unsigned {
@@ -129,7 +137,9 @@
     else lin = c.seq * G + wperm;
     if (lin >= ntiles) lin = ntiles - 1;
     const unsigned by = lin / nbx, bx = lin - by * nbx;
-    c.m0 = by * BM; c.n0 = bx * SK_BN;
+    c.m0 = by * BM;
+    if constexpr (KEPT) c.n0 = (unsigned)g.tile[bx] * SK_BN;
+    else c.n0 = bx * SK_BN;
     c.kp = FOLD ? first_kept() : c.kt;
     c.offA = (AKR ? c.m0 * 4u : (unsigned)(c.m0 * g.lda * 4)) + c.kp * kadvA;
     c.offB = (BKR ? c.n0 * 4u : (unsigned)(c.n0 * g.ldb * 4)) + c.kp * kadvB;
@@ -557,4 +567,45 @@
   return 1;
 }
 
-}
+int launch_gemm_sk_kept(ffh_ctx* c, const GemmArgs& g, const int* tiles, int nkept, bool dry, ffh_stream s, const char* name) {
+  if (g.N % SK_BN || g.N / SK_BN > 128 || nkept < 1 || nkept > g.N / SK_BN) return 0;
+  for (int i = 0; i < nkept; i++)
+    if (tiles[i] < 0 || tiles[i] >= g.N / SK_BN || (i > 0 && tiles[i] <= tiles[i - 1])) return 0;
+  if (g.db && tiles[0] != 0) return 0;
+  GemmArgs gk = g;
+  gk.N = nkept * SK_BN;
+  SkPlan p{};
+  if (!sk_plan(c, gk, SK_FORM_DW, p)) return 0;
+  const int64_t b_bytes = ((int64_t)(g.K - 1) * p.ldb + g.N) * 4;
+  if (b_bytes >= (1LL << 32)) return 0;
+  if (dry) return 1;
+  SkArgsKept a{};
+  a.A = g.A; a.B = g.B; a.C = g.C; a.db = g.db;
+  a.lda = p.lda; a.ldb = p.ldb; a.ldc = g.ldc;
+  a.M = g.M; a.N = g.N; a.K = g.K; a.act = g.act;
+  a.a_bytes = (unsigned)p.a_bytes; a.b_bytes = (unsigned)b_bytes;
+  a.nkept = (unsigned)nkept;
+  for (int i = 0; i < nkept; i++) a.tile[i] = (unsigned short)tiles[i];
+  constexpr int LDSB = 2 * SK_LDS_KR + 4 * SK_EP_WAVE;
+#define FFH_SK_KEPT_LAUNCH(DBV)                                                                                  \
+  {                                                                                                              \
+    auto kern = gemm_sk_kernel<true, true, SK_EPI_DW_ATOMIC, DBV, false, 4, false, true>;                        \
+    static std::atomic<signed char> ok[64];       \
+    const int dev = c->device & 63;                                                                              \
+    if (ok[dev].load(std::memory_order_acquire) == 0) ok[dev].store(sk_set_lds(kern, LDSB) ? 1 : -1, std::memory_order_release); \
+    if (ok[dev].load(std::memory_order_acquire) < 0) return 0;                                                   \
+    hipLaunchKernelGGL(kern, dim3((unsigned)p.G), dim3(256), LDSB, as_stream(s), a);                             \
+  }
+  if (g.db) FFH_SK_KEPT_LAUNCH(true)
+  else FFH_SK_KEPT_LAUNCH(false)
+#undef FFH_SK_KEPT_LAUNCH
+  {
+    const hipError_t e = hipGetLastError();
+    if (e == hipErrorInvalidValue || e == hipErrorInvalidConfiguration || e == hipErrorLaunchOutOfResources || e == hipErrorSharedObjectInitFailed) return 0;
+    if (e != hipSuccess) return ffh_fail_hip(c, e, name);
+  }
+  { char tok[96]; snprintf(tok, sizeof tok, "%s|sk_128x128x64|kept=%d/%d%s|wgs=%d", name, nkept, g.N / SK_BN, g.db ? "|db" : "", p.G); ffh_route_add(c, tok); }
+  return 1;
+}
+
+}
diff --git a/dlrm_flexflow_amd/host/ffmodel.h b/dlrm_flexflow_amd/host/ffmodel.h
--- a/dlrm_flexflow_amd/host/ffmodel.h
+++ b/dlrm_flexflow_amd/host/ffmodel.h
@@ -113,6 +113,7 @@
   int  trace_mode;
   bool fold_small_tables;
   int64_t fold_max_rows;
+  bool fold_dw;
   bool mlp_chain;
   int64_t mlp_chain_max_batch;
   int64_t mlp_chain_fwd_max_batch;
@@ -634,11 +635,22 @@
     std::vector<ffh_fold_seg> keep;
     float* P = nullptr;
     float* S = nullptr;
+    std::vector<Embedding*> dw_tables;
+    std::vector<ffh_emb_table> dw_sum;
+    std::vector<ffh_fold_group> dw_groups;
+    std::vector<int32_t> dw_kept;
+    float* G = nullptr;
+    ffh_ctx* sum_ctx = nullptr;
+    void* sum_ws = nullptr;
   } fold;
+  ffh_event ev_fold_e_read = nullptr;
+  mutable bool fold_e_read_recorded = false;
+  void fold_weight_gradient(const Linear* li, float* dbp, ffh_stream dws) const;
   ffh_event ev_fold_w = nullptr;
   ffh_event ev_fold_done = nullptr;
   mutable bool fold_w_recorded = false, fold_on_side = false;
   void plan_fold();
+  void plan_fold_dw(FoldRoute& r);
   void fold_products_and_sum(ffh_stream s, ffh_ctx* cx) const;
   void fold_linear_forward(const Linear* li) const;
   int z_reader_layer;
diff --git a/dlrm_flexflow_amd/host/ffmodel_c.cc b/dlrm_flexflow_amd/host/ffmodel_c.cc
--- a/dlrm_flexflow_amd/host/ffmodel_c.cc
+++ b/dlrm_flexflow_amd/host/ffmodel_c.cc
@@ -176,6 +176,7 @@
   if (n == "lr_route") return M(m)->lr_route;
   if (n == "graph_replays") return M(m)->n_graph_replays;
   if (n == "folded_tables") return (int64_t)M(m)->fold.tables.size();
+  if (n == "folded_dw_tables") return (int64_t)M(m)->fold.dw_tables.size();
   if (n == "tensor_op_exact_backward_layers") {
     int64_t k = 0;
     for (Op* op : M(m)->layers) if (op->op_type == OP_LINEAR && static_cast<Linear*>(op)->bwd_exact) k++;
diff --git a/dlrm_flexflow_amd/host/model.cc b/dlrm_flexflow_amd/host/model.cc
--- a/dlrm_flexflow_amd/host/model.cc
+++ b/dlrm_flexflow_amd/host/model.cc
@@ -368,7 +368,9 @@
   api->ffh_event_destroy(ctx, ev_z_free);
   if (ev_fold_w) api->ffh_event_destroy(ctx, ev_fold_w);
   if (ev_fold_done) api->ffh_event_destroy(ctx, ev_fold_done);
-  for (void* p : {(void*)fold.P, (void*)fold.S}) if (p) api->ffh_free(ctx, p);
+  if (ev_fold_e_read) api->ffh_event_destroy(ctx, ev_fold_e_read);
+  for (void* p : {(void*)fold.P, (void*)fold.S, (void*)fold.G, fold.sum_ws}) if (p) api->ffh_free(ctx, p);
+  if (fold.sum_ctx) api->ffh_ctx_destroy(fold.sum_ctx);
   for (auto& kv : trace_tune) for (ffh_event& e : kv.second.ev) if (e) { api->ffh_event_destroy(ctx, e); e = nullptr; }
   for (ffh_event& e : probe_ev) if (e) { api->ffh_event_destroy(ctx, e); e = nullptr; }
   api->ffh_stream_destroy(ctx, stream); api->ffh_stream_destroy(ctx, side_stream); api->ffh_stream_destroy(ctx, dw_stream); api->ffh_stream_destroy(ctx, ar_stream);
@@ -592,6 +594,21 @@
     return;
   }
   ffh_stream dws = ff.dw_stream;
+  if (part == 0 && ff.fold.layer == this && !ff.fold.dw_tables.empty()) {
+    if (fork) {
+      ffh_event ev = ff.layer_events[layer_index];
+      ff.check(ff.api->ffh_event_record(ff.ctx, ev, ff.stream), "event");
+      ff.check(ff.api->ffh_stream_wait_event(ff.ctx, dws, ev), "event");
+    }
+    if (dx) {
+      ff.check(ff.api->ffh_linear_bwd_ex(ff.ctx, xp, ldx, dx, lddx, yp, ldy, dyp, lddy, wp, dwp, dbp, in_padded, out_channels, b, (int)activation,
+                                         flags | FFH_LINEAR_ONLY_DX, ff.stream, nullptr), name);
+      image_dx();
+    }
+    ff.fold_weight_gradient(this, dbp, fork ? dws : ff.stream);
+    if (fork) { ff.dw_forked = true; ff.dw1_used = true; ff.dw_stream_used_directly = true; }
+    return;
+  }
   ff.check(ff.api->ffh_linear_bwd_ex(ff.ctx, xp, ldx, dx, lddx, yp, ldy, dyp, lddy, wp, dwp, dbp, in_padded, out_channels, b, (int)activation,
                                      flags, ff.stream, fork ? dws : nullptr), name);
   image_dx();
diff --git a/dlrm_flexflow_amd/host/model_allocate.cc b/dlrm_flexflow_amd/host/model_allocate.cc
--- a/dlrm_flexflow_amd/host/model_allocate.cc
+++ b/dlrm_flexflow_amd/host/model_allocate.cc
@@ -925,6 +925,7 @@
       col += in.adim[0];
     }
     r.layer = li;
+    plan_fold_dw(r);
     fold = r;
     if (!ev_fold_w) check((config.timing_events ? api->ffh_event_create : api->ffh_event_create_sync)(ctx, &ev_fold_w), "event create");
     if (!ev_fold_done) check((config.timing_events ? api->ffh_event_create : api->ffh_event_create_sync)(ctx, &ev_fold_done), "event create");
@@ -932,6 +933,56 @@
   }
 }
 
+void FFModel::plan_fold_dw(FoldRoute& r) {
+  Linear* li = r.layer;
+  if (!config.fold_dw || config.deterministic || config.profiling || dw_worker || side_worker) return;
+  if (!(li->dy_premasked || li->activation == AC_MODE_NONE) || li->pair_lower || li->bwd_exact || li->dx_image || li->dx_map) return;
+  const int64_t rows = local_rows(li->outputs[0], this);
+  if (!li->chain_bwd.empty() && mlp_chain_usable(rows, false)) return;
+  if (li->in_padded % FFH_FOLD_DW_NTILE || li->weights[0].impl->ld != li->in_padded) return;
+  const int out = li->out_channels, ntile = li->in_padded / FFH_FOLD_DW_NTILE;
+  std::vector<char> folded(ntile, 0);
+  std::vector<size_t> pick;
+  int64_t grows = 0;
+  for (size_t k = 0; k < r.tables.size(); k++) {
+    const int64_t col0 = r.groups[k].col0, d = r.tables[k]->out_channels;
+    if (col0 % FFH_FOLD_DW_NTILE || d % FFH_FOLD_DW_NTILE) continue;
+    for (int64_t t = col0 / FFH_FOLD_DW_NTILE; t < (col0 + d) / FFH_FOLD_DW_NTILE; t++) folded[t] = 1;
+    pick.push_back(k);
+    grows += r.tables[k]->num_entries;
+  }
+  if (pick.empty()) return;
+  for (int t = 0; t < ntile; t++) if (!folded[t]) r.dw_kept.push_back(t);
+  const Tensor &x = li->inputs[0], &y = li->outputs[0];
+  const int plan = r.dw_kept.empty() ? 0 : api->fold->ffh_fold_linear_bwd_dw_plan(ctx, (const float*)x.impl->ptr, x.impl->ld, y.impl->grad, y.impl->grad_ld, li->weights[0].impl->grad,
+                                                                                  li->use_bias ? li->weights[1].impl->grad : nullptr, li->in_padded, out, rows,
+                                                                                  r.dw_kept.data(), (int)r.dw_kept.size());
+  if (plan != 1) { r.dw_kept.clear(); return; }
+  const Embedding* e0 = r.tables[pick[0]];
+  const int L = (int)e0->inputs[0].adim[0];
+  r.G = (float*)dmalloc((size_t)grows * out * 4);
+  const size_t ws_bytes = api->ffh_embedding_bwd_workspace_bytes((int)pick.size(), L, out, local_batch) + 256;
+  r.sum_ws = dmalloc(ws_bytes);
+  if (api->ffh_ctx_create(&r.sum_ctx, config.device) != FFH_OK || !r.sum_ctx) die("fold: ffh_ctx_create(device %d) failed", config.device);
+  check(api->ffh_ctx_set_workspace(r.sum_ctx, r.sum_ws, ws_bytes), "set workspace");
+  int64_t grow = 0;
+  for (size_t k : pick) {
+    Embedding* e = r.tables[k];
+    float* g = r.G + (size_t)grow * out;
+    r.dw_tables.push_back(e);
+    r.dw_groups.push_back(ffh_fold_group{(const float*)e->weights[0].impl->ptr, (int64_t)e->out_channels, r.groups[k].col0, g, (int64_t)e->num_entries});
+    ffh_emb_table t;
+    t.idx = (const int64_t*)e->inputs[0].impl->ptr;
+    t.weight = g;
+    t.num_entries = e->num_entries;
+    t.io = y.impl->grad;
+    t.ld = y.impl->grad_ld;
+    r.dw_sum.push_back(t);
+    grow += e->num_entries;
+  }
+  if (!ev_fold_e_read) check((config.timing_events ? api->ffh_event_create : api->ffh_event_create_sync)(ctx, &ev_fold_e_read), "event create");
+}
+
 void FFModel::init_layers() {
   if (!compiled) die("init_layers() before compile()");
   for (Op* op : layers) op->init(*this);
diff --git a/dlrm_flexflow_amd/host/model_flags.cc b/dlrm_flexflow_amd/host/model_flags.cc
--- a/dlrm_flexflow_amd/host/model_flags.cc
+++ b/dlrm_flexflow_amd/host/model_flags.cc
@@ -37,6 +37,7 @@
   mlp_chain = true;
   fold_small_tables = true;
   fold_max_rows = 7420;
+  fold_dw = true;
   trace_mode = -1;
   bucket_allreduce = -1;
   allreduce_bucket_floats = 1 << 20;
@@ -147,6 +148,7 @@
     if (is("--no-fused-pair")) { fuse_pair = false; continue; }
     if (is("--no-mlp-chain")) { mlp_chain = false; continue; }
     if (is("--no-fold-small-tables")) { fold_small_tables = false; continue; }
+    if (is("--no-fold-dw")) { fold_dw = false; continue; }
     if (is("--fold-max-rows")) { fold_max_rows = atoll(next()); continue; }
     if (is("--always-replay")) { trace_mode = 1; continue; }
     if (is("--adaptive-replay")) { trace_mode = 0; continue; }
diff --git a/dlrm_flexflow_amd/host/model_step.cc b/dlrm_flexflow_amd/host/model_step.cc
--- a/dlrm_flexflow_amd/host/model_step.cc
+++ b/dlrm_flexflow_amd/host/model_step.cc
@@ -120,6 +120,20 @@
                                        fold.S, li->out_channels, s), "fold_gather_add");
 }
 
+void FFModel::fold_weight_gradient(const Linear* li, float* dbp, ffh_stream dws) const {
+  const Tensor &x = li->inputs[0], &y = li->outputs[0];
+  const Embedding* e0 = fold.dw_tables[0];
+  const int64_t b = local_rows(y, this);
+  const int out = li->out_channels, ng = (int)fold.dw_groups.size();
+  if (api->fold->ffh_fold_segment_sum(fold.sum_ctx, fold.dw_sum.data(), ng, e0->inputs[0].adim[0], out, b, dws) != FFH_OK)
+    die("%s: fold_segment_sum failed: %s", li->name, api->ffh_last_error_string(fold.sum_ctx));
+  check(api->fold->ffh_fold_dw_product(ctx, fold.dw_groups.data(), ng, li->weights[0].impl->grad, li->in_padded, e0->out_channels, out, dws), "fold_dw_product");
+  check(api->ffh_event_record(ctx, ev_fold_e_read, dws), "fold: table rows read");
+  fold_e_read_recorded = true;
+  check(api->fold->ffh_fold_linear_bwd_dw(ctx, (const float*)x.impl->ptr, x.impl->ld, y.impl->grad, y.impl->grad_ld, li->weights[0].impl->grad, dbp, li->in_padded, out, b,
+                                          fold.dw_kept.data(), (int)fold.dw_kept.size(), dws), li->name);
+}
+
 void FFModel::fold_linear_forward(const Linear* li) const {
   if (fold_on_side) check(api->ffh_stream_wait_event(ctx, stream, ev_fold_done), "fold: sum ready");
   else fold_products_and_sum(stream, ctx);
@@ -148,6 +162,7 @@
     });
   } else {
     check(api->ffh_stream_wait_event(ctx, side_stream, ev_grad_ready), "event");
+    if (fold_e_read_recorded) check(api->ffh_stream_wait_event(ctx, side_stream, ev_fold_e_read), "fold: table rows read");
     probe_record(2, side_stream, ctx);
     embedding_group_update(side_stream);
     probe_record(3, side_stream, ctx);
@@ -192,6 +207,7 @@
   const float scale = (bce || loss_type == LOSS_MEAN_SQUARED_ERROR_AVG_REDUCE) ? 1.0f / (float)fin.adim[fin.numDim - 1] : 1.0f;
   if (fin.impl->grad_ld != fin.adim[0] || fin.impl->ld != fin.adim[0]) die("final layer output must be contiguous");
   dw_forked = false;
+  fold_e_read_recorded = false;
   opt_next_done = false;
   int first = (int)layers.size() - 1;
   emb_update_pending = false;
diff --git a/include/ff_hip_fold.h b/include/ff_hip_fold.h
--- a/include/ff_hip_fold.h
+++ b/include/ff_hip_fold.h
@@ -7,12 +7,14 @@
 extern "C" {
 #endif
 
-#define FFH_FOLD_ABI_VERSION 1
+#define FFH_FOLD_ABI_VERSION 2
 
 #define FFH_FOLD_KTILE      16
 #define FFH_FOLD_NTILE      64
 #define FFH_FOLD_MAX_GROUPS 64
 #define FFH_FOLD_MAX_SEGS   32
+#define FFH_FOLD_DW_NTILE   128
+#define FFH_FOLD_DW_CHUNK   256
 
 typedef struct ffh_fold_group {
   const float* e;
@@ -38,11 +40,23 @@
 int ffh_fold_linear_fwd_plan(ffh_ctx* ctx, const float* x, int64_t ldx, const float* y, int64_t ldy, const float* w, const float* bias,
                              int in_dim, int out_dim, int64_t batch, const ffh_fold_seg* keep, int nkeep, const float* addend, int64_t ldadd);
 
+
+int ffh_fold_segment_sum(ffh_ctx* ctx, const ffh_emb_table* tables, int ntables, int in_dim, int width, int64_t batch, ffh_stream s);
+
+int ffh_fold_dw_product(ffh_ctx* ctx, const ffh_fold_group* groups, int ngroups, float* dw, int64_t lddw, int d, int out_dim, ffh_stream s);
+
+int ffh_fold_linear_bwd_dw(ffh_ctx* ctx, const float* x, int64_t ldx, const float* dy, int64_t lddy, float* dw, float* db, int in_dim, int out_dim,
+                           int64_t batch, const int32_t* kept, int nkept, ffh_stream s);
+
+int ffh_fold_linear_bwd_dw_plan(ffh_ctx* ctx, const float* x, int64_t ldx, const float* dy, int64_t lddy, const float* dw, const float* db, int in_dim,
+                                int out_dim, int64_t batch, const int32_t* kept, int nkept);
+
 #ifdef __cplusplus
 }
 #endif
 
 #define FFH_FOLD_API_LIST(X) \
-  X(ffh_fold_abi_version) X(ffh_fold_product) X(ffh_fold_gather_add) X(ffh_fold_linear_fwd) X(ffh_fold_linear_fwd_plan)
+  X(ffh_fold_abi_version) X(ffh_fold_product) X(ffh_fold_gather_add) X(ffh_fold_linear_fwd) X(ffh_fold_linear_fwd_plan) \
+  X(ffh_fold_segment_sum) X(ffh_fold_dw_product) X(ffh_fold_linear_bwd_dw) X(ffh_fold_linear_bwd_dw_plan)
 
 #endif
```
